# chlhnu/DOT-SOCP

Measured on AMD Instinct MI355X. Metric: ADMM iters/sec on NxNxT dot2d staggered grid at 1/2/4/8 MI355X, higher is better.
Workload: dtype f64

## Files before the change

### dot-socp_amd/capi.py

```python
import ctypes
import os

import numpy as np

_HERE = os.path.dirname(os.path.abspath(__file__))
LIB_PATH = os.path.join(_HERE, "lib", "libdotsocp.so")

i64 = ctypes.c_longlong
dbl = ctypes.c_double
vp = ctypes.c_void_p


class DotsocpError(RuntimeError):
    def __init__(self, code, msg):
        super().__init__(f"libdotsocp error {code}: {msg}")
        self.code = code


class Problem(ctypes.Structure):
    _fields_ = [("dim", ctypes.c_int), ("weighted", ctypes.c_int),
                ("ny", i64), ("nx", i64), ("nt", i64),
                ("D", dbl), ("E", dbl), ("cScale", dbl), ("dScale", dbl),
                ("normc", dbl), ("normd", dbl)]


class Opts(ctypes.Structure):
    _fields_ = [("tau", dbl), ("sigma", dbl), ("tol", dbl), ("maxit", i64),
                ("ifCheckStepByStep", ctypes.c_int), ("checkPrimDualFeas", ctypes.c_int),
                ("scaling", ctypes.c_int), ("time_limit", dbl)]


class Result(ctypes.Structure):
    _fields_ = [("sigma", dbl), ("sigma_internal", dbl), ("cScale", dbl), ("dScale", dbl),
                ("times", dbl * 7), ("iters", i64), ("hist_len", i64), ("stopped", ctypes.c_int),
                ("time_extra", dbl)]


class AccOpts(ctypes.Structure):
    _fields_ = [("restart", i64), ("rho", dbl), ("theta", dbl)]


REPORT_BINS = 49
REPORT_RHO_FLOOR = 1e-8


class Report(ctypes.Structure):
    _fields_ = [("n_nodes", i64), ("n_cells", i64), ("mass_err", dbl), ("neg_err", dbl),
                ("rho_min", dbl), ("rho_neg", i64), ("rho_hist", i64 * REPORT_BINS),
                ("fq_max", dbl), ("fq_pos", i64), ("fq_hist", i64 * REPORT_BINS),
                ("cost", dbl), ("nonfinite", i64)]


class AdvectOpts(ctypes.Structure):
    _fields_ = [("n", i64), ("nsub", ctypes.c_int), ("direction", ctypes.c_int), ("rho_floor", dbl)]


class PushOpts(ctypes.Structure):
    _fields_ = [("n", i64), ("nsub", ctypes.c_int), ("direction", ctypes.c_int), ("rho_floor", dbl), ("nf", i64)]


class MapReport(ctypes.Structure):
    _fields_ = [("n", i64), ("n_clamped", i64), ("n_still", i64), ("mass", dbl),
                ("cost_map", dbl), ("cost_length", dbl), ("cost_action", dbl), ("disp_mean", dbl), ("len_mean", dbl),
                ("disp_max", dbl), ("len_max", dbl), ("detour_max", dbl),
                ("detour_hist", i64 * REPORT_BINS), ("detour_over", i64)]


class RenderOpts(ctypes.Structure):
    _fields_ = [("mode", ctypes.c_int), ("channels", ctypes.c_int), ("nf", i64), ("nlevels", ctypes.c_int),
                ("barrier_index", ctypes.c_int), ("vmax", dbl), ("skip_y", i64), ("skip_x", i64), ("mask_frac", dbl)]


class RenderInfo(ctypes.Structure):
    _fields_ = [("vmax", dbl), ("rho_min", dbl), ("nonfinite", i64), ("masked", i64), ("my", i64), ("mx", i64)]


RENDER_LINEAR, RENDER_INVERTED, RENDER_LEVELS = 0, 1, 2
METHOD_INPALM, METHOD_PALM, METHOD_ACCADMM = 0, 1, 2


F_PHI, F_Q, F_ALPHA, F_Z, F_BETA, F_C, F_WEIGHT = range(7)

SYMBOLS = {
    "dotsocp_last_error": (ctypes.c_char_p, []),
    "dotsocp_version": (ctypes.c_char_p, []),
    "dotsocp_device_count": (ctypes.c_int, []),
    "dotsocp_proj_soc": (ctypes.c_int, [vp, vp, i64, i64]),
    "dotsocp_bfd": (ctypes.c_int, [vp, vp, i64, i64, i64, dbl, dbl]),
    "dotsocp_bfd_conj": (ctypes.c_int, [vp, vp, i64, i64, i64, dbl]),
    "dotsocp_bfd1d": (ctypes.c_int, [vp, vp, i64, i64, dbl, dbl]),
    "dotsocp_bfd_conj1d": (ctypes.c_int, [vp, vp, i64, i64, dbl]),
    "dotsocp_oper_poisson": (ctypes.c_int, [vp, vp, i64, i64, i64, dbl]),
    "dotsocp_dctn": (ctypes.c_int, [vp, i64, i64, i64, ctypes.c_int]),
    "dotsocp_proj_soc_dev": (ctypes.c_int, [vp, vp, i64, i64, vp]),
    "dotsocp_bfd_dev": (ctypes.c_int, [vp, vp, i64, i64, i64, dbl, dbl, vp]),
    "dotsocp_bfd_conj_dev": (ctypes.c_int, [vp, vp, i64, i64, i64, dbl, vp]),
    "dotsocp_create": (vp, [ctypes.POINTER(Problem), ctypes.c_int, ctypes.c_int]),
    "dotsocp_create_multi": (vp, [ctypes.POINTER(Problem), ctypes.c_int, ctypes.c_int]),
    "dotsocp_destroy": (None, [vp]),
    "dotsocp_rccl_unique_id": (ctypes.c_int, [vp]),
    "dotsocp_attach_rccl": (ctypes.c_int, [vp, vp, ctypes.c_int, ctypes.c_int]),
    "dotsocp_slab_range": (ctypes.c_int, [i64, ctypes.c_int, ctypes.c_int, ctypes.POINTER(i64), ctypes.POINTER(i64)]),
    "dotsocp_field_len": (i64, [ctypes.POINTER(Problem), ctypes.c_int]),
    "dotsocp_dct_algorithm": (ctypes.c_int, [i64]),
    "dotsocp_dct_levels": (ctypes.c_int, [i64, ctypes.c_int]),
    "dotsocp_cdft_levels": (ctypes.c_int, [i64]),
    "dotsocp_tsolve_tri_safe": (ctypes.c_int, [i64, i64, i64]),
    "dotsocp_cone_writes_beta": (ctypes.c_int, [i64, dbl, i64, ctypes.c_int, ctypes.c_int, ctypes.c_int, dbl, dbl]),
    "dotsocp_rescale_due": (ctypes.c_int, [i64, ctypes.c_int, dbl, dbl]),
    "dotsocp_qcone_form": (ctypes.c_int, [i64, dbl, i64, ctypes.c_int, ctypes.c_int, ctypes.c_int, ctypes.c_int, dbl, dbl]),
    "dotsocp_release_cache": (i64, []),
    "dotsocp_upload": (ctypes.c_int, [vp, ctypes.c_int, vp]),
    "dotsocp_upload_layers": (ctypes.c_int, [vp, ctypes.c_int, vp, i64, i64]),
    "dotsocp_download": (ctypes.c_int, [vp, ctypes.c_int, vp]),
    "dotsocp_begin": (ctypes.c_int, [vp, ctypes.POINTER(Opts)]),
    "dotsocp_begin_method": (ctypes.c_int, [vp, ctypes.POINTER(Opts), ctypes.c_int, ctypes.POINTER(AccOpts)]),
    "dotsocp_run": (ctypes.c_int, [vp, i64, ctypes.POINTER(i64)]),
    "dotsocp_recover_outputs": (ctypes.c_int, [vp, vp, vp, vp, vp, vp, vp, vp, vp]),
    "dotsocp_report_edges": (ctypes.c_int, [vp]),
    "dotsocp_solution_report": (ctypes.c_int, [vp, vp, vp, ctypes.POINTER(Report), vp, vp]),
    "dotsocp_recover_velocity": (ctypes.c_int, [vp, vp, vp, dbl, vp, vp]),
    "dotsocp_advect_particles": (ctypes.c_int, [vp, vp, vp, ctypes.POINTER(AdvectOpts), vp, vp, vp, vp, ctypes.POINTER(i64)]),
    "dotsocp_push_mass": (ctypes.c_int, [vp, vp, vp, ctypes.POINTER(PushOpts), vp, vp, vp, vp, vp, ctypes.POINTER(i64),
                                         ctypes.POINTER(dbl), vp]),
    "dotsocp_map_report": (ctypes.c_int, [vp, vp, vp, ctypes.POINTER(AdvectOpts), vp, vp, vp, ctypes.POINTER(MapReport),
                                          vp, vp, vp]),
    "dotsocp_render_evolution": (ctypes.c_int, [vp, vp, vp, ctypes.POINTER(RenderOpts), vp, vp, vp, vp, vp, vp, vp,
                                                ctypes.POINTER(RenderInfo)]),
    "dotsocp_jump_next_level": (ctypes.c_int, [vp, vp]),
    "dotsocp_finish": (ctypes.c_int, [vp, ctypes.POINTER(Result)]),
    "dotsocp_get_history": (ctypes.c_int, [vp, vp, vp, vp, vp]),
    "dotsocp_set_profiling": (ctypes.c_int, [vp, ctypes.c_int]),
    "dotsocp_kernel_time": (ctypes.c_int, [vp, ctypes.c_char_p, ctypes.POINTER(dbl), ctypes.POINTER(i64)]),
    "dotsocp_canary_check": (ctypes.c_int, []),
    "dotsocp_poisson_phi": (ctypes.c_int, [vp]),
    "dotsocp_synchronize": (ctypes.c_int, [vp]),
    "dotsocp_weights_create": (vp, [ctypes.c_int, i64, i64, i64, ctypes.c_int]),
    "dotsocp_weights_destroy": (None, [vp]),
    "dotsocp_weights_len": (i64, [i64, i64, i64, ctypes.c_int, ctypes.c_int]),
    "dotsocp_weights_set": (ctypes.c_int, [vp, vp]),
    "dotsocp_weights_set_space": (ctypes.c_int, [vp, vp, vp]),
    "dotsocp_weights_restrict": (ctypes.c_int, [vp, ctypes.c_int]),
    "dotsocp_weights_log10_mean": (ctypes.c_int, [vp, ctypes.c_int, ctypes.POINTER(dbl)]),
    "dotsocp_weights_download": (ctypes.c_int, [vp, ctypes.c_int, vp]),
    "dotsocp_upload_weight_from": (ctypes.c_int, [vp, vp, ctypes.c_int]),
}

_lib = None


def _share_torchs_hip_runtime():
    import importlib.util
    import sys
    if "torch" in sys.modules or os.environ.get("DOTSOCP_SYSTEM_HIP"):
        return
    try:
        spec = importlib.util.find_spec("torch")
    except (ImportError, ValueError):
        return
    if not spec or not spec.submodule_search_locations:
        return
    for name in ("libamdhip64.so", "libamdhip64.so.7"):
        path = os.path.join(list(spec.submodule_search_locations)[0], "lib", name)
        if os.path.exists(path):
            try:
                ctypes.CDLL(path, mode=ctypes.RTLD_GLOBAL)
            except OSError:
                pass
            return


def lib():
    global _lib
    if _lib is None:
        _share_torchs_hip_runtime()
        if not os.path.exists(LIB_PATH):
            raise ImportError(
                f"{LIB_PATH} is missing: build the HIP extension first "
                "(python -c 'import __graft_entry__ as g; g.build()'); there is no CPU fallback")
        L = ctypes.CDLL(LIB_PATH)
        for name, (res, args) in SYMBOLS.items():
            f = getattr(L, name)
            f.restype = res
            f.argtypes = args
        _lib = L
    return _lib


def check(code):
    if code != 0:
        raise DotsocpError(code, lib().dotsocp_last_error().decode())


def fptr(a):
    if not isinstance(a, np.ndarray) or a.dtype != np.float64 or not (a.flags.f_contiguous or a.flags.c_contiguous):
        raise ValueError("expected a contiguous float64 numpy array")
    return a.ctypes.data


def slab_range(nt, world, rank):
    t0, t1 = i64(), i64()
    check(lib().dotsocp_slab_range(nt, world, rank, ctypes.byref(t0), ctypes.byref(t1)))
    return t0.value, t1.value


def rccl_unique_id():
    buf = (ctypes.c_ubyte * 128)()
    check(lib().dotsocp_rccl_unique_id(buf))
    return bytes(buf)


DCT_ALGORITHMS = ("none", "fft", "pfa", "rader", "bluestein", "dense")


def dct_algorithm(n):
    return DCT_ALGORITHMS[lib().dotsocp_dct_algorithm(int(n))]


def dct_levels(n, axis):
    return int(lib().dotsocp_dct_levels(int(n), int(axis)))


def cdft_levels(n):
    return int(lib().dotsocp_cdft_levels(int(n)))
```

### dot-socp_amd/csrc/capi.hip

```cpp
#include <cstring>
#include <new>

#include "comm.h"
#include "solver.h"
#include "weights.h"

using namespace dotsocp;

namespace dotsocp {
extern thread_local std::string g_last_error;
int dotsocp_slab_range_impl(i64 nt, int world, int rank, i64 *t0, i64 *t1);
}

struct dotsocp_ctx {
    Solver s;
};

struct dotsocp_weights {
    Weights w;
};

static int require_device() {
    int n = 0;
    if (hipGetDeviceCount(&n) != hipSuccess || n <= 0) {
// ... 119 lines not shown
    Grid g;
    DS_CHECK(make_grid(g, nt, 1, nx));
    DS_ARG(z && q, "NULL pointer");
    DS_CHECK(require_device());
    DevBuf dz, dq;
    DS_CHECK(dz.alloc(10 * g.Nz));
    DS_CHECK(dq.alloc(g.NqAlloc));
    DS_HIP(hipMemset(dz.p, 0, sizeof(double) * 10 * g.Nz));
    for (int j = 0; j < 6; ++j)
        DS_HIP(hipMemcpy(dz.p + k1dCols[j] * g.Nz, z + j * g.Nz, sizeof(double) * g.Nz, hipMemcpyHostToDevice));
    DS_CHECK(launch_bfd_conj(g, dq.p, dz.p, scale, nullptr));
    DS_HIP(hipDeviceSynchronize());
    DS_HIP(hipMemcpy(q, dq.p, sizeof(double) * g.NqAlloc, hipMemcpyDeviceToHost));
    return 0;
}

static int dctn_dev(double *a, double *b, i64 ny, i64 nx, i64 nt, int inverse, DctPlan *py, DctPlan *px, DctPlan *pt) {
    if (!inverse) {
        DS_CHECK(launch_dct_axis(py, a, b, ny, nx, nt, 0, 0, nullptr));
        DS_CHECK(launch_dct_axis(px, b, a, ny, nx, nt, 1, 0, nullptr));
        DS_CHECK(launch_dct_axis(pt, a, b, ny, nx, nt, 2, 0, nullptr));
    } else {
        DS_CHECK(launch_dct_axis(pt, a, b, ny, nx, nt, 2, 1, nullptr));
        DS_CHECK(launch_dct_axis(px, b, a, ny, nx, nt, 1, 1, nullptr));
        DS_CHECK(launch_dct_axis(py, a, b, ny, nx, nt, 0, 1, nullptr));
    }
    return 0;
}

struct Plans {
    DctPlan *py = nullptr, *px = nullptr, *pt = nullptr;
    ~Plans() { dct_plan_destroy(py); dct_plan_destroy(px); dct_plan_destroy(pt); }
    int make(i64 ny, i64 nx, i64 nt) {
        DS_CHECK(dct_length_check(ny)); DS_CHECK(dct_length_check(nx)); DS_CHECK(dct_length_check(nt));
        py = dct_plan_create(ny); px = dct_plan_create(nx); pt = dct_plan_create(nt);
        if (!py || !px || !pt) { set_error("DCT plan allocation failed"); return DOTSOCP_EHIP; }
        return 0;
    }
};

int dotsocp_dctn(double *a, dotsocp_i64 ny, dotsocp_i64 nx, dotsocp_i64 nt, int inverse) {
    DS_ARG(a && ny >= 1 && nx >= 1 && nt >= 1, "bad array");
    DS_CHECK(dct_length_check(ny)); DS_CHECK(dct_length_check(nx)); DS_CHECK(dct_length_check(nt));
    DS_CHECK(require_device());
    const i64 n = ny * nx * nt;
    DevBuf da, db;
    Plans pl;
    DS_CHECK(da.alloc(n));
    DS_CHECK(db.alloc(n));
    DS_CHECK(pl.make(ny, nx, nt));
    DS_HIP(hipMemcpy(da.p, a, sizeof(double) * n, hipMemcpyHostToDevice));
    DS_CHECK(dctn_dev(da.p, db.p, ny, nx, nt, inverse, pl.py, pl.px, pl.pt));
    DS_HIP(hipDeviceSynchronize());
    DS_HIP(hipMemcpy(a, db.p, sizeof(double) * n, hipMemcpyDeviceToHost));
    return 0;
}

int dotsocp_oper_poisson(double *res, const double *rhs, dotsocp_i64 ny, dotsocp_i64 nx, dotsocp_i64 nt,
                         double kernelScale) {
    DS_ARG(res && rhs && ny >= 1 && nx >= 1 && nt >= 1, "bad array");
    DS_CHECK(dct_length_check(ny)); DS_CHECK(dct_length_check(nx)); DS_CHECK(dct_length_check(nt));
    DS_CHECK(require_device());
    const i64 n = ny * nx * nt;
    DevBuf da, db, cy, cx, ct;
    Plans pl;
    DS_CHECK(da.alloc(n));
    DS_CHECK(db.alloc(n));
    DS_CHECK(pl.make(ny, nx, nt));
    const double pi = 3.14159265358979323846;
    auto table = [&](DevBuf &d, i64 m) -> int {
        std::vector<double> t((size_t)m);
        for (i64 k = 0; k < m; ++k) t[k] = (2.0 * (double)(m - 1) * (double)(m - 1)) * (1.0 - cos(pi * (double)k / (double)m));
        DS_CHECK(d.alloc(m));
        DS_HIP(hipMemcpy(d.p, t.data(), sizeof(double) * m, hipMemcpyHostToDevice));
        return 0;
    };
    DS_CHECK(table(cy, ny));
    DS_CHECK(table(cx, nx));
    DS_CHECK(table(ct, nt));
    DS_HIP(hipMemcpy(da.p, rhs, sizeof(double) * n, hipMemcpyHostToDevice));
    Grid g;
    g.set(ny, nx, nt, 0, nt);
    DS_CHECK(launch_dct_axis(pl.py, da.p, db.p, ny, nx, nt, 0, 0, nullptr));
    DS_CHECK(launch_dct_axis(pl.px, db.p, da.p, ny, nx, nt, 1, 0, nullptr));
    DS_CHECK(launch_poisson_t_single(pl.pt, g, kernelScale, cy.p, cx.p, ct.p, da.p, db.p, 0, nullptr, tsolve_tri_allowed()));
    DS_CHECK(launch_dct_axis(pl.px, da.p, db.p, ny, nx, nt, 1, 1, nullptr));
    DS_CHECK(launch_dct_axis(pl.py, db.p, da.p, ny, nx, nt, 0, 1, nullptr));
    DS_HIP(hipDeviceSynchronize());
    DS_HIP(hipMemcpy(res, da.p, sizeof(double) * n, hipMemcpyDeviceToHost));
    return 0;
}

dotsocp_ctx *dotsocp_create(const dotsocp_problem *prob, int device, int nslabs) {
    dotsocp_ctx *c = new (std::nothrow) dotsocp_ctx();
    if (!c) { set_error("out of host memory"); return nullptr; }
    if (c->s.init(prob, device, nslabs) != 0) {
        delete c;
        return nullptr;
    }
    return c;
}

dotsocp_ctx *dotsocp_create_multi(const dotsocp_problem *prob, int first_device, int ngpu) {
    dotsocp_ctx *c = new (std::nothrow) dotsocp_ctx();
    if (!c) { set_error("out of host memory"); return nullptr; }
    if (c->s.init(prob, first_device, ngpu, true) != 0) {
        delete c;
        return nullptr;
    }
    return c;
}

void dotsocp_destroy(dotsocp_ctx *ctx) { delete ctx; }

int dotsocp_slab_range(dotsocp_i64 nt, int world, int rank, dotsocp_i64 *t0, dotsocp_i64 *t1) {
    DS_ARG(t0 && t1 && world >= 1 && rank >= 0 && rank < world && nt >= 2 * world, "bad slab request");
    return dotsocp_slab_range_impl(nt, world, rank, t0, t1);
}

int dotsocp_rccl_unique_id(unsigned char id[128]) {
    DS_ARG(id != nullptr, "id is NULL");
    Rccl &api = rccl_api();
    DS_CHECK(api.load());
    ncclUniqueId uid;
    static_assert(sizeof(uid) == 128, "ncclUniqueId is expected to be 128 bytes");
    DS_NCCL(api.GetUniqueId(&uid));
    memcpy(id, &uid, sizeof uid);
    return 0;
}

int dotsocp_attach_rccl(dotsocp_ctx *ctx, const unsigned char id[128], int rank, int world) {
    if (!ctx) { set_error("ctx is NULL"); return DOTSOCP_EINVAL; }
    return ctx->s.attach_rccl(id, rank, world);
}

#define CTX_OR_FAIL()                                      \
    do {                                                   \
        if (!ctx) { set_error("ctx is NULL"); return DOTSOCP_EINVAL; } \
        (void)hipGetLastError();    \
    } while (0)

int dotsocp_dct_algorithm(dotsocp_i64 n) { return dct_choose_algorithm(n); }
int dotsocp_dct_levels(dotsocp_i64 n, int axis) { return dct_levels(n, axis); }
int dotsocp_cdft_levels(dotsocp_i64 n) { return cdft_levels(n); }
int dotsocp_tsolve_tri_safe(dotsocp_i64 ny, dotsocp_i64 nx, dotsocp_i64 nt) { return tsolve_tri_safe(ny, nx, nt) ? 1 : 0; }

int dotsocp_cone_writes_beta(dotsocp_i64 it, double last_sigma_it, dotsocp_i64 maxit, int check_step_by_step,
                             int last_of_run, int rescale, double maxFeas, double relGap) {
    return cone_writes_beta(it, last_sigma_it, maxit, check_step_by_step != 0, last_of_run != 0, rescale, maxFeas, relGap) ? 1 : 0;
}
int dotsocp_rescale_due(dotsocp_i64 it, int rescale, double maxFeas, double relGap) {
    return rescale_due(it, rescale, maxFeas, relGap) ? 1 : 0;
}
int dotsocp_qcone_form(dotsocp_i64 it, double last_sigma_it, dotsocp_i64 maxit, int check_step_by_step, int last_of_run,
                       int next_last_of_run, int rescale, double maxFeas, double relGap) {
    return qcone_form(it, last_sigma_it, maxit, check_step_by_step != 0, last_of_run != 0, next_last_of_run != 0, rescale,
                      maxFeas, relGap);
}

dotsocp_i64 dotsocp_field_len(const dotsocp_problem *p, int field) {
    if (!p || (p->dim != 1 && p->dim != 2) || p->nt < 2 || p->nx < 1 || (p->dim == 2 && p->ny < 1)) return -1;
    const i64 ny = p->dim == 1 ? p->nx : p->ny, nx = p->dim == 1 ? 1 : p->nx, nt = p->nt;
    const i64 Nphi = ny * nx * nt, Nz = ny * nx * (nt - 1);
    const i64 Nq = Nz + ny * (nx - 1) * nt + (ny - 1) * nx * nt;
    switch (field) {
        case DOTSOCP_F_PHI: case DOTSOCP_F_C: return Nphi;
        case DOTSOCP_F_Q: case DOTSOCP_F_ALPHA: case DOTSOCP_F_WEIGHT: return Nq;
        case DOTSOCP_F_Z: case DOTSOCP_F_BETA: return Nz * (p->dim == 1 ? 6 : 10);
        default: return -1;
    }
}

int dotsocp_upload(dotsocp_ctx *ctx, int field, const double *host) { CTX_OR_FAIL(); return ctx->s.upload(field, host); }
dotsocp_i64 dotsocp_release_cache(void) { return (dotsocp_i64)device_cache_release(); }

int dotsocp_upload_layers(dotsocp_ctx *ctx, int field, const double *host, dotsocp_i64 t0, dotsocp_i64 n) {
    CTX_OR_FAIL();
    return ctx->s.upload_layers(field, host, t0, n);
}
int dotsocp_download(dotsocp_ctx *ctx, int field, double *host) { CTX_OR_FAIL(); return ctx->s.download(field, host); }
int dotsocp_begin(dotsocp_ctx *ctx, const dotsocp_opts *opts) { CTX_OR_FAIL(); return ctx->s.begin(opts); }
int dotsocp_begin_method(dotsocp_ctx *ctx, const dotsocp_opts *opts, int method, const dotsocp_acc_opts *acc) {
    CTX_OR_FAIL();
    return ctx->s.begin_method(opts, method, acc);
}
int dotsocp_recover_outputs(dotsocp_ctx *ctx, const double *rho0, const double *rho1, double *rho, double *Ex,
                            double *Ey, double *q0, double *bx, double *by) {
    CTX_OR_FAIL();
    if (ctx->s.prob.dim == 1)
        return ctx->s.recover_outputs(rho0, rho1, rho, nullptr, Ex, q0, nullptr, bx);
    return ctx->s.recover_outputs(rho0, rho1, rho, Ex, Ey, q0, bx, by);
}

int dotsocp_report_edges(double edges[DOTSOCP_REPORT_BINS + 1]) {
    if (!edges) { set_error("invalid argument: report_edges() needs an array of %d doubles", DOTSOCP_REPORT_BINS + 1); return DOTSOCP_EINVAL; }
    report_edges_host(edges);
    return 0;
}

int dotsocp_solution_report(dotsocp_ctx *ctx, const double *rho0, const double *rho1, dotsocp_report *rep, double *layer_mass,
                            double *layer_neg) {
    CTX_OR_FAIL();
    return ctx->s.solution_report(rho0, rho1, rep, layer_mass, layer_neg);
}

int dotsocp_recover_velocity(dotsocp_ctx *ctx, const double *rho0, const double *rho1, double rho_floor, double *vx, double *vy) {
    CTX_OR_FAIL();
    if (ctx->s.prob.dim == 1)
        return ctx->s.recover_velocity(rho0, rho1, rho_floor, nullptr, vx);
    return ctx->s.recover_velocity(rho0, rho1, rho_floor, vx, vy);
}

int dotsocp_advect_particles(dotsocp_ctx *ctx, const double *rho0, const double *rho1, const dotsocp_advect_opts *o, double *x,
                             double *y, double *traj_x, double *traj_y, dotsocp_i64 *n_clamped) {
    CTX_OR_FAIL();
    if (ctx->s.prob.dim == 1)
        return ctx->s.advect_particles(rho0, rho1, o, nullptr, x, nullptr, traj_x, n_clamped);
    return ctx->s.advect_particles(rho0, rho1, o, x, y, traj_x, traj_y, n_clamped);
}

int dotsocp_push_mass(dotsocp_ctx *ctx, const double *rho0, const double *rho1, const dotsocp_push_opts *o, double *x, double *y,
                      const double *mass, const dotsocp_i64 *frame_nodes, double *frames, dotsocp_i64 *n_clamped, double *unit,
                      double *l1) {
    CTX_OR_FAIL();
    if (ctx->s.prob.dim == 1)
        return ctx->s.push_mass(rho0, rho1, o, nullptr, x, mass, frame_nodes, frames, n_clamped, unit, l1);
    return ctx->s.push_mass(rho0, rho1, o, x, y, mass, frame_nodes, frames, n_clamped, unit, l1);
}

int dotsocp_map_report(dotsocp_ctx *ctx, const double *rho0, const double *rho1, const dotsocp_advect_opts *o, double *x, double *y,
                       const double *mass, dotsocp_map_report_t *rep, double *disp, double *len, double *action) {
    CTX_OR_FAIL();
    if (ctx->s.prob.dim == 1)
        return ctx->s.map_report(rho0, rho1, o, nullptr, x, mass, rep, disp, len, action);
    return ctx->s.map_report(rho0, rho1, o, x, y, mass, rep, disp, len, action);
}

int dotsocp_render_evolution(dotsocp_ctx *ctx, const double *rho0, const double *rho1, const dotsocp_render_opts *opts,
                             const dotsocp_i64 *frame_nodes, const double *levels, const unsigned char *lut,
                             const unsigned char *barrier, unsigned char *image, double *mvx, double *mvy,
                             dotsocp_render_info *info) {
    CTX_OR_FAIL();
    if (ctx->s.prob.dim != 1 || !opts)
        return ctx->s.render_evolution(rho0, rho1, opts, frame_nodes, levels, lut, barrier, image, mvx, mvy, info);
    dotsocp_render_opts o = *opts;
    if (o.skip_y >= 1 && o.skip_x >= 1) { o.skip_y = o.skip_x; o.skip_x = 1; }
    dotsocp_render_info got{};
    const int rc = ctx->s.render_evolution(rho0, rho1, &o, frame_nodes, levels, lut, barrier, image, nullptr, mvx, &got);
    if (rc == 0 && info) {
        *info = got;
        info->mx = got.my;
        info->my = got.my > 0 ? 1 : 0;
    }
    return rc;
}

int dotsocp_jump_next_level(dotsocp_ctx *coarse, dotsocp_ctx *fine) {
    if (!coarse || !fine) { set_error("context is NULL"); return DOTSOCP_EINVAL; }
    return fine->s.jump_from(coarse->s);
}

int dotsocp_run(dotsocp_ctx *ctx, dotsocp_i64 n_iters, dotsocp_i64 *done) { CTX_OR_FAIL(); return ctx->s.run(n_iters, done); }
int dotsocp_finish(dotsocp_ctx *ctx, dotsocp_result *res) { CTX_OR_FAIL(); return ctx->s.finish(res); }

int dotsocp_get_history(dotsocp_ctx *ctx, double *kkt, double *time, double *iter, double *pdGap) {
    CTX_OR_FAIL();
    const Solver &s = ctx->s;
    const size_t n = s.hist_iter.size();
    for (size_t i = 0; i < n; ++i) {
        if (kkt) for (int j = 0; j < 7; ++j) kkt[j * n + i] = s.hist_kkt[i * 7 + j];
        if (time) time[i] = s.hist_time[i];
        if (iter) iter[i] = s.hist_iter[i];
        if (pdGap) pdGap[i] = s.hist_gap[i];
    }
    return 0;
}

int dotsocp_set_profiling(dotsocp_ctx *ctx, int on) {
    CTX_OR_FAIL();
    ctx->s.profiling = on != 0;
    return 0;
}

int dotsocp_kernel_time(dotsocp_ctx *ctx, const char *name, double *avg_ms, dotsocp_i64 *launches) {
    CTX_OR_FAIL();
    DS_ARG(name != nullptr, "name is NULL");
    static const char *names[PH_COUNT] = {"rhs", "poisson", "cone_proj", "qstep", "beta", "kkt",
                                          "cone_fused_a", "cone_fused_b", "materialise", "comm",
                                          "interp", "acc_cone", "acc_gather", "qstep_first", "transpose", "cone_carry", "qcone",
                                          "velocity_layer", "advect", "deposit", "frame_l1", "advect_path", "map_final"};
    for (int i = 0; i < PH_COUNT; ++i)
        if (strcmp(name, names[i]) == 0) {
            const i64 n = ctx->s.phase_launches[i];
            if (avg_ms) *avg_ms = n ? ctx->s.phase_ms[i] / (double)n : 0.0;
            if (launches) *launches = n;
            return 0;
        }
    set_error("unknown kernel family '%s'", name);
    return DOTSOCP_EINVAL;
}

int dotsocp_canary_check(void) {
    std::string rep;
    const int bad = canary_check(&rep);
    if (bad) set_error("canary: %d device buffer(s) written out of bounds: %s", bad, rep.c_str());
    return bad;
}

#define WEIGHTS_OR_FAIL()                                  \
    do {                                                   \
        if (!w) { set_error("weight pyramid is NULL"); return DOTSOCP_EINVAL; } \
        (void)hipGetLastError();                           \
    } while (0)

dotsocp_weights *dotsocp_weights_create(int device, dotsocp_i64 ny, dotsocp_i64 nx, dotsocp_i64 nt, int levels) {
    dotsocp_weights *w = new (std::nothrow) dotsocp_weights();
    if (!w) { set_error("out of host memory"); return nullptr; }
    if (w->w.init(device, ny, nx, nt, levels) != 0) {
        delete w;
        return nullptr;
    }
    return w;
}

void dotsocp_weights_destroy(dotsocp_weights *w) { delete w; }

dotsocp_i64 dotsocp_weights_len(dotsocp_i64 ny, dotsocp_i64 nx, dotsocp_i64 nt, int levels, int level) {
    return weights_level_len(ny, nx, nt, levels, level);
}

int dotsocp_weights_set(dotsocp_weights *w, const double *weight) { WEIGHTS_OR_FAIL(); return w->w.set(weight); }
int dotsocp_weights_set_space(dotsocp_weights *w, const double *weightX, const double *weightY) {
    WEIGHTS_OR_FAIL();
    return w->w.set_space(weightX, weightY);
}
int dotsocp_weights_restrict(dotsocp_weights *w, int log_mean) { WEIGHTS_OR_FAIL(); return w->w.restrict_all(log_mean); }
int dotsocp_weights_log10_mean(dotsocp_weights *w, int level, double *mean) { WEIGHTS_OR_FAIL(); return w->w.log10_mean(level, mean); }
int dotsocp_weights_download(dotsocp_weights *w, int level, double *host) { WEIGHTS_OR_FAIL(); return w->w.download(level, host); }

int dotsocp_upload_weight_from(dotsocp_ctx *ctx, dotsocp_weights *w, int level) {
    CTX_OR_FAIL();
    WEIGHTS_OR_FAIL();
    const Weights::Level *L = nullptr;
    DS_CHECK(w->w.level_for_upload(level, &L));
    return ctx->s.upload_weight_from(L->w, w->w.device, L->ny, L->nx, L->nt);
}

int dotsocp_poisson_phi(dotsocp_ctx *ctx) { CTX_OR_FAIL(); return ctx->s.poisson_phi(); }

int dotsocp_synchronize(dotsocp_ctx *ctx) {
    CTX_OR_FAIL();
    ctx->s.cur_dev = -1;
    return ctx->s.sync_all();
}

}
```

### dot-socp_amd/csrc/fused.hip

```cpp
#include "device_utils.h"
#include "gather_tile.h"
#include "kernels.h"

#include <cstdlib>

namespace dotsocp {

template <int MODE, int XB, bool NT = false, bool GIN = false, bool GOUT = false>
__global__ void __launch_bounds__(64 * XB) k_cone_fused(Grid g, LoopCoef c, FusedArgs a) {
    static_assert(MODE == 1 || !(GIN || GOUT), "the gamma form exists between two MODE_B passes only");
    constexpr bool DUAL = (MODE >= 5);
    constexpr bool UPD = (MODE != 0 && MODE != 6);
    constexpr bool PROJ = (MODE < 2 || MODE >= 5);
    __shared__ double2 xch[2][XB][64];
    __shared__ double2 xchp[DUAL ? 2 : 1][DUAL ? XB : 1][DUAL ? 64 : 1];
    const int lane = threadIdx.x, xl = threadIdx.y;
    const BlockId blk = block_id(a.xcd != 0);
    const i64 y = (i64)blk.x * 64 + lane;
    const i64 x = (i64)blk.y * XB + xl;
    const bool inb = (y < g.ny) && (x < g.nx);
    const i64 yc = inb ? y : 0, xc = inb ? x : 0;
    const i64 t0 = ((i64)blk.z + a.z0) * a.TC;
    const i64 t1 = (t0 + a.TC < g.ncl) ? t0 + a.TC : g.ncl;
    const bool lastChunk = (t1 == g.ncl);
    constexpr bool GATHER = (PROJ || MODE == 4);
    const bool carried = GATHER && !DUAL && t0 > 0 && a.carry_in != nullptr;
    const i64 tstart = (GATHER && t0 > 0 && !carried) ? t0 - 1 : t0;
    const i64 nxblk = gridDim.y, nyblk = gridDim.x;

    EdgeQuad cur = load_edges(g, a.q, yc, xc, tstart, c.sf), curo, cur3;
    if (UPD && !GIN) curo = load_edges(g, a.q_old, yc, xc, tstart, c.sf);
    if (MODE == 5) cur3 = load_edges(g, a.q3, yc, xc, tstart, c.sf);
    GatherCarry gc, gcp;
    if (carried) {
        const i64 ci = yc + g.py * xc;
        gc.p3 = a.carry_in[ci]; gc.p4 = a.carry_in[g.plane + ci];
        gc.p7 = a.carry_in[2 * g.plane + ci]; gc.p8 = a.carry_in[3 * g.plane + ci];
    }
    const i64 tstop = (GATHER && lastChunk) ? t1 + 1 : t1;
    for (i64 tl = tstart; tl < tstop; ++tl) {
        const bool hasCell = tl < g.ncl;
        const bool own = tl >= t0;
        double w[10], wp[10];
        if (hasCell) {
            const i64 i = yc + g.py * (xc + g.nx * tl);
            const EdgeQuad nxt = load_edges(g, a.q, yc, xc, tl + 1, c.sf);
            double b[10], v[10];
#pragma unroll
            for (int j = 0; j < 10; ++j) b[j] = ld_stream<NT>(a.beta_in + j * g.Nc + i);
            if (!GIN) apply_scale_ops(b, a.bops);
            build_z2(v, a.q[i], cur, nxt, c.s, c.dF);
            if constexpr (GIN) {
#pragma unroll
                for (int j = 0; j < 10; ++j) b[j] = mult_finish(b[j], v[j], c.tau);
                if (!GOUT && own && inb) {
#pragma unroll
                    for (int j = 0; j < 10; ++j) st_stream<NT>(a.beta_out + j * g.Nc + i, b[j]);
                }
            } else if constexpr (UPD) {
                const EdgeQuad nxto = load_edges(g, a.q_old, yc, xc, tl + 1, c.sf);
                double zo[10];
                build_z2(zo, a.q_old[i], curo, nxto, c.s, c.dF);
#pragma unroll
                for (int j = 0; j < 10; ++j) zo[j] = zo[j] - b[j];
                proj_row<10>(zo);
#pragma unroll
                for (int j = 0; j < 10; ++j) b[j] = mult_finish(mult_carry(b[j], zo[j], c.tau), v[j], c.tau);
                if (own && inb) {
                    if (MODE != 3 && !GOUT) {
#pragma unroll
                        for (int j = 0; j < 10; ++j) st_stream<NT>(a.beta_out + j * g.Nc + i, b[j]);
                    }
                    if (MODE == 2 || MODE == 3) {
#pragma unroll
                        for (int j = 0; j < 10; ++j) st_stream<NT>(a.z_out + j * g.Nc + i, zo[j]);
                    }
                }
                curo = nxto;
                if (MODE == 4) {
#pragma unroll
                    for (int j = 0; j < 10; ++j) w[j] = zo[j] + b[j];
                    if (own && inb) a.q2[i] = c.s * (w[9] - w[0]);
                }
            }
            cur = nxt;
            if (PROJ) {
                if (MODE == 5) {
                    const EdgeQuad nxt3 = load_edges(g, a.q3, yc, xc, tl + 1, c.sf);
                    build_z2(v, a.q3[i], cur3, nxt3, c.s, c.dF);
                    cur3 = nxt3;
                }
#pragma unroll
                for (int j = 0; j < 10; ++j) v[j] = v[j] - b[j];
                proj_row<10>(v);
                if (GOUT && own && inb) {
#pragma unroll
                    for (int j = 0; j < 10; ++j) st_stream<NT>(a.beta_out + j * g.Nc + i, mult_carry(b[j], v[j], c.tau));
                }
#pragma unroll
                for (int j = 0; j < 10; ++j) w[j] = v[j] + b[j];
                if (own && inb) a.q2[i] = c.s * (w[9] - w[0]);
                if (DUAL) {
#pragma unroll
                    for (int j = 0; j < 10; ++j) wp[j] = w[j] + c.tau * v[j];
                    if (own && inb) a.p2[i] = c.s * (wp[9] - wp[0]);
                }
            }
        } else {
#pragma unroll
            for (int j = 0; j < 10; ++j) w[j] = 0.0;
            if (DUAL) {
#pragma unroll
                for (int j = 0; j < 10; ++j) wp[j] = 0.0;
            }
        }
        if constexpr (GATHER && !DUAL)
            gather_emit<XB>(g, c.sf, xch, gc, w, tl, own && inb, x, y, xl, lane, nxblk, nyblk, blk.y, blk.x,
                            a.q2, a.sx, a.sy);
        if constexpr (DUAL) {
            gather_post<XB>(xch, gc, w, xl, lane);
            gather_post<XB>(xchp, gcp, wp, xl, lane);
            __syncthreads();
            gather_finish<XB>(g, c.sf, xch, gc, w, tl, own && inb, x, y, xl, lane, nxblk, nyblk, blk.y, blk.x,
                              a.q2, a.sx, a.sy);
            gather_finish<XB>(g, c.sf, xchp, gcp, wp, tl, own && inb, x, y, xl, lane, nxblk, nyblk, blk.y, blk.x,
                              a.p2, a.sxp, a.syp);
        }
    }
    if (GATHER && !DUAL && !lastChunk && a.carry_out != nullptr && inb) {
        const i64 ci = y + g.py * x;
        a.carry_out[ci] = gc.p3; a.carry_out[g.plane + ci] = gc.p4;
        a.carry_out[2 * g.plane + ci] = gc.p7; a.carry_out[3 * g.plane + ci] = gc.p8;
    }
}

bool stream_nt_enabled() {
    const char *e = getenv("DOTSOCP_NT");
    return !(e && atoi(e) == 0);
}

bool tile_xcd_remap(const Grid &g) {
    return (g.py % 16) != 0;
}

bool cone_split_enabled() { return true; }

int fused_geometry(const Grid &g, FusedGeom &fg) {
    fg.XB = 4;
    fg.nyblk = (g.ny + 63) / 64;
    fg.nxblk = (g.nx + fg.XB - 1) / fg.XB;
    const i64 tiles = fg.nyblk * fg.nxblk;
    const i64 target = 2048;
    i64 chunks = (target + tiles - 1) / tiles;
    if (chunks < 1) chunks = 1;
    if (!(g.first && g.last) && cone_split_enabled() && chunks < 2 && g.ncl >= 12) chunks = 2;
    i64 TC = (g.ncl + chunks - 1) / chunks;
    if (TC < 8) TC = 8;
    if (TC > g.ncl) TC = g.ncl;
    if (TC < 1) TC = 1;
    fg.TC = TC;
    fg.chunks = (g.ncl + TC - 1) / TC;
    fg.sx_len = (g.ncl + 1) * fg.nxblk * g.ny;
    fg.sy_len = (g.ncl + 1) * g.nx * fg.nyblk;
    return 0;
}

int launch_cone_fused(int mode, const Grid &g, const LoopCoef &c, const FusedGeom &fg, FusedArgs a,
                      hipStream_t st, i64 z0, i64 zcount, int flavour) {
    if (g.Nz <= 0) return 0;
    if (zcount < 0) zcount = fg.chunks - z0;
    if (z0 < 0 || zcount <= 0 || z0 + zcount > fg.chunks) return 0;
    a.TC = fg.TC;
    a.z0 = (int)z0;
    a.xcd = tile_xcd_remap(g) ? 1 : 0;
    dim3 grid((unsigned)fg.nyblk, (unsigned)fg.nxblk, (unsigned)zcount);
    dim3 blk(64, 4);
    const bool nt = stream_nt_enabled();
#define CONE_MODE(M)                                                                     \
    case M:                                                                              \
        if (nt) DS_KLAUNCH((k_cone_fused<M, 4, true>), grid, blk, 0, st, g, c, a);       \
        else DS_KLAUNCH((k_cone_fused<M, 4>), grid, blk, 0, st, g, c, a);                \
        break;
    if (flavour != 0) {
        if (mode != 1 || (flavour & ~(CONE_GIN | CONE_GOUT))) { set_error("bad fused flavour"); return DOTSOCP_EINVAL; }
        if ((flavour & CONE_GIN) && !a.bops.empty()) { set_error("internal: gamma with a pending scaling"); return DOTSOCP_ESTATE; }
#define CONE_FLAV(GI, GO)                                                                          \
        if (nt) DS_KLAUNCH((k_cone_fused<1, 4, true, GI, GO>), grid, blk, 0, st, g, c, a);         \
        else DS_KLAUNCH((k_cone_fused<1, 4, false, GI, GO>), grid, blk, 0, st, g, c, a);
        if (flavour == CONE_GOUT) { CONE_FLAV(false, true) }
        else if (flavour == CONE_GIN) { CONE_FLAV(true, false) }
        else { CONE_FLAV(true, true) }
#undef CONE_FLAV
        DS_HIP(hipGetLastError());
        return 0;
    }
    switch (mode) {
        CONE_MODE(0) CONE_MODE(1) CONE_MODE(2) CONE_MODE(3) CONE_MODE(4) CONE_MODE(5) CONE_MODE(6)
#undef CONE_MODE
        default: set_error("bad fused mode"); return DOTSOCP_EINVAL;
    }
    DS_HIP(hipGetLastError());
    return 0;
}

}
```

### dot-socp_amd/csrc/kernels.h

```cpp
#pragma once
#include "common.h"
#include "defer.h"
#include "particle_block.h"

namespace dotsocp {

struct LoopCoef {
    double s;
    double sf;
    double dF;
    double at, ax, ay;
    double tau;
    double c1, c2;
    double dinv1, dinv2;
};

enum {
    S_Q2 = 0, S_Z2, S_APHI2, S_ALPHA2, S_BETA2, S_FBBETA2, S_PRIM1, S_PRIM2, S_DUAL1, S_DUAL2,
    S_COMPLEM, S_DOTCOMP, S_RHO2, S_RHOFQ2, S_MRHOB, S_M2, S_RHOB2, S_QALPHA, S_CPHI, S_PHI2,
    S_COUNT
};

struct KktCoef {
    double sigma;
    double kappa;
    double dsD;
    double dsE;
};

struct ScaleOps {
    int n;
    double mul, div;
    double mul2, div2;
    bool empty() const { return n == 0; }
    void clear() { n = 0; }
    bool push(double m, double d) {
        if (n >= 2) return false;
        if (n == 0) { mul = m; div = d; } else { mul2 = m; div2 = d; }
        n += 1;
        return true;
    }
};

int launch_proj_soc(double *out, const double *in, i64 M, i64 K, hipStream_t st);
int launch_bfd(const Grid &g, double *z, const double *q, double s, double dF, hipStream_t st);
int launch_bfd_conj(const Grid &g, double *q, const double *w, double s, hipStream_t st, const double *tail_bx = nullptr,
                    const double *tail_by = nullptr);
int launch_cone_proj(const Grid &g, const LoopCoef &c, const double *q, const double *beta, double *z,
                     hipStream_t st);
int launch_beta_update(const Grid &g, const LoopCoef &c, const double *q, const double *z, double *beta,
                       hipStream_t st);
int launch_gather_tail(const Grid &g, const double *z, const double *beta, double *tail_bx, double *tail_by,
                       hipStream_t st);

struct FusedGeom {
    int XB;
    i64 nyblk, nxblk;
    i64 TC, chunks;
    i64 sx_len, sy_len;
};
struct FusedArgs {
    const double *q_old;
    const double *q;
    const double *beta_in;
    double *beta_out;
    double *z_out;
    double *q2;
    double *sx, *sy;
    const double *q3;
    double *p2, *sxp, *syp;
    i64 TC;
    ScaleOps bops;
    int xcd;
    int z0;
    const double *carry_in;
    double *carry_out;
};
bool tile_xcd_remap(const Grid &g);
int fused_geometry(const Grid &g, FusedGeom &fg);
enum { CONE_GIN = 1, CONE_GOUT = 2 };
int launch_cone_fused(int mode, const Grid &g, const LoopCoef &c, const FusedGeom &fg, FusedArgs a,
                      hipStream_t st, i64 z0 = 0, i64 zcount = -1, int flavour = 0);
bool cone_split_enabled();

struct KktWork;
struct AccArgs {
    const double *q;
    const double *z_in, *beta_in;
    const double *z0, *beta0;
    double *z0_out, *beta0_out;
    double bdiv;
    KktCoef kk;
    const double *alpha_p, *weight;
    double *partials;
    int nostore;
    double *z_out, *beta_out;
    double *q2, *sx, *sy;
    i64 TC;
    double c1, c2, om_rho, rho;
};
struct AccCoef {
    double c1, c2, om_rho, rho;
    double om_c1, c1c2;
};
int launch_acc_cone(int mode, const Grid &g, const LoopCoef &c, const FusedGeom &fg, AccArgs a, hipStream_t st);
int launch_acc_cone_kkt(const Grid &g, const LoopCoef &c, const FusedGeom &fg, AccArgs a, const KktWork &w, hipStream_t st);
int launch_acc_restart(double *x, const double *xp, double *anchor, i64 n, const AccCoef &k, double div, hipStream_t st);
int launch_acc_interp(double *x, const double *xp, double *aux, i64 n, const AccCoef &k, int mode, int write_aux,
                      hipStream_t st);

int launch_prolong_phi(const Grid &gf, const Grid &gc, const double *phic, double *phif, double sc_in, double sc_out,
                       hipStream_t st, i64 tc0 = 0);
int launch_prolong_beta(const Grid &gf, const Grid &gc, const double *betac, double *betaf, double *neg, double sc_in0,
                        double sc_in1, double sc_out, hipStream_t st, i64 tc0 = 0, i64 Nzc = -1);
int launch_scale_div(double *x, const double *w, i64 n, double sc, hipStream_t st);
int launch_fill(double *x, i64 n, double v, hipStream_t st);
int launch_outputs(const Grid &g, const double *q, const double *alpha, const double *weight, const double *rho0,
                   const double *rho1, const double *a_prev, double sig, double cD, double dD, int which, double *out,
                   hipStream_t st);
int launch_out_tail(const Grid &g, const double *alpha, const double *weight, double sig, double cD, double *out,
                    hipStream_t st);

int launch_velocity_layer(const Grid &g, const double *alpha, const double *weight, const double *rho0, const double *rho1,
                          const double *a_prev, double sig, double cD, bool dim1, i64 tl, double floor, double *vX, double *vY,
                          hipStream_t st);
int launch_advect_seed(bool dim1, i64 n, double *px, double *py, unsigned int *flag, hipStream_t st);
int launch_advect(bool dim1, i64 ny, i64 nx, i64 py, const double *vX0, const double *vY0, const double *vX1,
                  const double *vY1, i64 n, int nsub, int dir, double dt, double *px, double *py_, unsigned int *flag,
                  hipStream_t st, double *sq = nullptr, double *len = nullptr);
int launch_advect_count(const unsigned int *flag, i64 n, unsigned long long *count, hipStream_t st);
int launch_deposit(bool dim1, i64 ny, i64 nx, i64 py, i64 n, const double *px, const double *py_, const i64 *units,
                   unsigned long long *cnt, hipStream_t st);
int launch_frame_l1(const Grid &g, const double *alpha, const double *weight, const double *rho0, const double *rho1,
                    const double *a_prev, double sig, double cD, i64 tl, double unit, double *frame, double *partials,
                    double *sum, hipStream_t st);
i64 map_blocks(i64 n);
int launch_map_final(bool dim1, i64 n, const double *px, const double *py_, const double *sq, const double *len, const double *sx,
                     const double *sy, const double *mass, const double *edges, double steps, double *disp, double *action,
                     double *partials, double *sums, unsigned long long *counts, hipStream_t st);

enum { RC_RHO_HIST = 0, RC_FQ_HIST = DOTSOCP_REPORT_BINS, RC_RHO_NEG = 2 * DOTSOCP_REPORT_BINS, RC_FQ_POS, RC_NONFINITE,
       RC_RHO_MIN, RC_FQ_MAX, RC_COUNT };
void report_edges_host(double edges[DOTSOCP_REPORT_BINS + 1]);
double report_key_decode(unsigned long long key, bool inverted, double none);
i64 report_tiles(const Grid &g);
int launch_report_rows(const double *partials, i64 tiles, i64 rows, double *sums, hipStream_t st);
int launch_report(const Grid &g, const double *q, const double *alpha, const double *weight, const double *rho0,
                  const double *rho1, const double *a_prev, double sig, double cD, double dD, bool dim1, const double *edges,
                  double *partials, double *sums, unsigned long long *counts, hipStream_t st);

enum { RR_MAX = 0, RR_MIN, RR_NONFINITE, RR_MASKED, RR_COUNT };
#define RND_LEVELS 255
int launch_rho_range(const Grid &g, const double *alpha, const double *weight, const double *rho0, const double *rho1,
                     const double *a_prev, double sig, double cD, const unsigned char *barrier, unsigned long long *counts,
                     hipStream_t st);
int launch_render(const Grid &g, const double *alpha, const double *weight, const double *rho0, const double *rho1,
                  const double *a_prev, double sig, double cD, i64 tl, int mode, int channels, const unsigned char *barrier,
                  const double *levels, int nlevels, const unsigned char *lut, int barrier_index, double vmax,
                  unsigned char *image, hipStream_t st);
int launch_movement(const Grid &g, const double *alpha, const double *weight, const double *rho0, const double *rho1,
                    const double *a_prev, double sig, double cD, i64 tl, i64 skip_y, i64 skip_x, i64 my, i64 mx, double thr,
                    double *mvX, double *mvY, hipStream_t st);

struct QStepExtra {
    ScaleOps aops;
    double *partials, *resid;
    double kappa, dsD;
    double *u0_tail;
    int c_ends;
};
int launch_qstep_rhs(const Grid &g, const LoopCoef &c, const FusedGeom &fg, const double *phi, const double *q2,
                     const double *sx, const double *sy, const double *weight, const double *tail_bx,
                     const double *tail_by, const double *cvec, double *q_out, const double *alpha_in, double *alpha_out,
                     double *rhs, hipStream_t st, i64 z0 = 0, i64 zcount = -1, i64 zstride = 1,
                     const QStepExtra *ex = nullptr);
i64 qstep_rhs_blocks(const Grid &g, const FusedGeom &fg);
struct QConeArgs {
    const double *phi, *q2v, *sx, *sy, *cvec, *alpha_in, *gamma_in;
    double *alpha_out, *rhs, *q_out, *beta_out, *q2_out, *sx_out, *sy_out;
    i64 TC;
    int ap_on;
    double ap_mul, ap_div;
    int c_ends;
};
int launch_qcone(const Grid &g, const LoopCoef &c, const FusedGeom &fg, QConeArgs a, bool gout, hipStream_t st);
i64 qcone_chunk_len(const Grid &g);
i64 qstep_rhs_chunks(const Grid &g, const FusedGeom &fg, i64 *TC = nullptr);
int launch_qstep_rhs_acc(int var, const Grid &g, const LoopCoef &c, const FusedGeom &fg, const double *phi,
                         const double *q2, const double *sx, const double *sy, const double *weight, const double *cvec,
                         double *q_raw, const double *alpha_in, double *alpha_out, double *rhs, double *q_state,
                         const double *q_anchor, const double *alpha_anchor, const AccCoef &k, hipStream_t st,
                         const double *tail_bx = nullptr, const double *tail_by = nullptr, double *u0_tail = nullptr);
int launch_qstep_palm_first(const Grid &g, const LoopCoef &c, const FusedGeom &fg, const double *phi, const double *q2,
                            const double *sx, const double *sy, const double *cvec, double *q_out, const double *alpha,
                            double *rhs, hipStream_t st, const double *tail_bx = nullptr, const double *tail_by = nullptr,
                            const double *qk = nullptr);

int launch_qstep_fused(const Grid &g, const LoopCoef &c, const FusedGeom &fg, const double *phi,
                       const double *q2, const double *sx, const double *sy, const double *weight,
                       const double *tail_bx, const double *tail_by, double *q_out, double *alpha,
                       hipStream_t st);
int launch_rhs_sigma_fix(const Grid &g, double *rhs, const double *r, double *cvec, double factor, hipStream_t st,
                         bool c_ends = false);
int launch_c_interior_test(const Grid &g, const double *cvec, int *flag, hipStream_t st);
int launch_rhs_fixup(const Grid &g, const LoopCoef &c, const double *u0_prev, double *rhs, hipStream_t st);
int launch_grad(const Grid &g, const LoopCoef &c, const double *phi, double *out, hipStream_t st);
int launch_tail_finalize(const Grid &g, const LoopCoef &c, const FusedGeom &fg, const double *q2, const double *sx,
                         const double *sy, double *tail_bx, double *tail_by, hipStream_t st);
int launch_kkt_tail(const Grid &g, const double *alpha, const double *beta, const double *weight, double *a0,
                    double *a0w, double *bt_bx, double *bt_by, hipStream_t st);
int launch_rhs(const Grid &g, const LoopCoef &c, const double *q, const double *alpha, const double *cvec,
               const double *weight, const double *u0_prev, double *rhs, hipStream_t st, bool c_ends = false);
int launch_qstep(const Grid &g, const LoopCoef &c, const double *phi, const double *z, const double *beta,
                 const double *weight, const double *tail_bx, const double *tail_by, double *q,
                 double *alpha, hipStream_t st);
int launch_u0_tail(const Grid &g, const double *q, const double *alpha, const double *weight, double *out,
                   hipStream_t st);
int launch_scale(double *x, i64 n, double mul, double div, hipStream_t st);
#define DS_MAX_WORLD 64
struct PencilCuts {
    int world;
    i64 cut[DS_MAX_WORLD + 1];
};
int launch_pencil_pack(bool pack, const PencilCuts &pc, i64 plane, i64 ntl, double *slab, double *stage, hipStream_t st);

#define TRI_EXTRA 256
int launch_tri_local(const Grid &g, i64 nt, double kscale, const double *cy, const double *cx, const PencilCuts &pc,
                     const double *r, double *send, hipStream_t st);
int launch_tri_reduced(const Grid &g, i64 nt, double kscale, const double *cy, const double *cx, const PencilCuts &pc,
                       int rank, i64 l0, i64 nl, const i64 *slab_n, const double *recv, double *back, double *zero_work,
                       hipStream_t st, const double *own_recv = nullptr, double *own_back = nullptr);
int launch_tri_final(const Grid &g, i64 nt, double kscale, const double *cy, const double *cx, const PencilCuts &pc,
                     const double *back, double *x, hipStream_t st);
bool tsolve_tri_supported(i64 nt);
bool tsolve_tri_preferred(i64 nt, bool pow2, i64 plane);
bool tsolve_tri_safe(i64 ny, i64 nx, i64 nt);
int launch_tsolve_tri(const Grid &g, i64 nt, double kscale, const double *cy, const double *cx, double *x, hipStream_t st);
int device_cus();
struct GatherMsgs {
    const double *src[DS_MAX_WORLD];
    double *dst[DS_MAX_WORLD];
    i64 count[DS_MAX_WORLD];
    int n;
};
int launch_gather_msgs(const GatherMsgs &m, hipStream_t st);

#define KKT_SLICES 64
struct KktWork {
    double *partials;
    i64 maxBlocks;
    double *sums;
};
struct KktHalo {
    const double *a0_prev, *a0w_prev, *btail_bx, *btail_by;
};
i64 kkt_partials_needed(const Grid &g);
int launch_kkt(const Grid &g, const LoopCoef &c, const KktCoef &k, const double *phi, const double *q,
               const double *alpha, const double *z, const double *beta, const double *cvec,
               const double *weight, const KktHalo &halo, const KktWork &w, int parts, hipStream_t st,
               bool layer0 = false, double *resid = nullptr);
int launch_kkt_nodual(const Grid &g, const LoopCoef &c, const KktCoef &k, const double *phi, const double *q,
                      const double *alpha, const double *cvec, const double *weight, const KktWork &w, hipStream_t st);
int launch_kkt_bnd_dual(const Grid &g, const LoopCoef &c, const KktCoef &k, const FusedGeom &fg, const double *q,
                        const double *alpha, const double *weight, const double *q2, const double *sx, const double *sy,
                        const KktWork &w, hipStream_t st);
int launch_kkt_cells_update(const Grid &g, const LoopCoef &c, const KktCoef &k, const FusedGeom &fg, FusedArgs a,
                            const double *phi, const double *alpha, const double *weight, const KktWork &w,
                            hipStream_t st, bool edges = false, const double *q_new = nullptr);
int launch_norms(const Grid &g, const LoopCoef &c, const KktCoef &k, const FusedGeom &fg, FusedArgs a, const double *phi,
                 const double *alpha, const double *weight, const KktWork &w, hipStream_t st);
double *kkt_qstep_partials(const Grid &g, const KktWork &w);
int launch_kkt_final(const Grid &g, const KktWork &w, hipStream_t st);

enum { DCT_ALG_NONE = 0, DCT_ALG_FFT = 1, DCT_ALG_PFA = 2, DCT_ALG_RADER = 3, DCT_ALG_BLUESTEIN = 4, DCT_ALG_DENSE = 5 };
int dct_choose_algorithm(i64 n);
struct DctPlan;
int dct_levels(i64 n, int axis);
int dct_length_check(i64 n);
int cdft_levels(i64 n);
DctPlan *dct_plan_create(i64 n);
void dct_plan_destroy(DctPlan *p);
int launch_dct_axis(const DctPlan *p, const double *src, double *dst, i64 n0, i64 n1, i64 n2, int axis,
                    int inverse, hipStream_t st, i64 pitch0 = 0);
bool dct_plan_is_pow2(const DctPlan *p);
bool dct_plan_has_tsolve(const DctPlan *p);
int launch_dct_t_solve(const DctPlan *p, const double *src, double *dst, i64 ny, i64 nplane, i64 line0, i64 nl,
                       i64 nt, double kscale, const double *cy, const double *cx, const double *ct, hipStream_t st,
                       i64 pitch0 = 0);
int launch_spectral_divide_pencil(double *data, i64 ny, i64 line0, i64 nl, i64 nt, double kscale, const double *cy,
                                  const double *cx, const double *ct, hipStream_t st);
int launch_spectral_divide(double *data, i64 ny, i64 nt, i64 x0, i64 nxl, double kscale, const double *cy,
                           const double *cx, const double *ct, hipStream_t st, i64 pitch0 = 0);
bool tsolve_tri_allowed();
int launch_poisson_t_single(const DctPlan *pt, const Grid &g, double kscale, const double *cy, const double *cx,
                            const double *ct, double *p, double *p2, i64 pitch0, hipStream_t st, bool allow_tri);

}
```

### dot-socp_amd/csrc/kkt.hip

```cpp
#include "device_utils.h"
#include "gather_tile.h"
#include "kernels.h"

#include <cstdlib>

namespace dotsocp {

struct WBeta {
    const double *b;
    i64 Nz;
    __device__ __forceinline__ double operator()(int j, i64 cell) const { return b[j * Nz + cell]; }
};

template <bool WEIGHTED, int PART, bool NODUAL = false>
__global__ void __launch_bounds__(TILE_Y *TILE_X) k_kkt(Grid g, LoopCoef c, KktCoef k, i64 chunk,
                                                         const double *__restrict__ phi, const double *__restrict__ q,
                                                         const double *__restrict__ alpha, const double *__restrict__ z,
                                                         const double *__restrict__ beta,
                                                         const double *__restrict__ cvec,
                                                         const double *__restrict__ weight,
                                                         KktHalo halo, double *__restrict__ partials,
                                                         double *__restrict__ resid) {
    const i64 y = (i64)blockIdx.x * TILE_Y + threadIdx.x;
    const i64 x = (i64)blockIdx.y * TILE_X + threadIdx.y;
// ... 2 lines not shown
    const i64 tend = (tbeg + chunk < g.ntl) ? tbeg + chunk : g.ntl;
    double S[S_COUNT];
#pragma unroll
    for (int i = 0; i < S_COUNT; ++i) S[i] = 0.0;
    WBeta WB{beta, g.Nc};
    auto wgt = [&](i64 idx) { return WEIGHTED ? weight[idx] : 1.0; };
    auto rhoT_at = [&](i64 yy, i64 xx, i64 tl) -> double {
        if (tl >= g.ncl) return 0.0;
        if (tl < 0) {
            if (g.first) return 0.0;
            return k.kappa * halo.a0w_prev[yy + g.py * xx];
        }
        const i64 cidx = yy + g.py * (xx + g.nx * tl);
        return k.kappa * (wgt(cidx) * alpha[cidx]);
    };
    auto rho_node = [&](i64 yy, i64 xx, i64 tl) { return (rhoT_at(yy, xx, tl - 1) + rhoT_at(yy, xx, tl)) / 2.0; };
    auto edge_sums = [&](i64 idx, double tmp, double q2b) {
        const double w = wgt(idx);
        const double qv = q[idx], av = alpha[idx];
        const double wq = w * qv, wa = w * av;
        S[S_Q2] += qv * qv;
        S[S_ALPHA2] += av * av;
        S[S_APHI2] += tmp * tmp;
        const double r1 = tmp - wq;
        S[S_PRIM1] += r1 * r1;
        if (!NODUAL) {
            S[S_FBBETA2] += q2b * q2b;
            const double r2 = q2b + wa;
            S[S_DUAL2] += r2 * r2;
        }
        S[S_QALPHA] += wq * av;
    };
    if (inb) {
        for (i64 tl = tbeg; tl < tend; ++tl) {
            const i64 node = y + g.py * (x + g.nx * tl);
            const i64 bxo = g.offBx + g.bxLayer * tl, byo = g.offBy + g.byLayer * tl;
            if (PART & 1) {
                double r = 0.0;
                if (tl >= 1)
                    r += c.at * alpha[node - g.plane];
                else if (!g.first)
                    r += c.at * halo.a0_prev[y + g.py * x];
                if (tl < g.ncl) r += (-c.at) * alpha[node];
                if (x >= 1) r += c.ax * alpha[bxo + y + g.py * (x - 1)];
                if (x <= g.nx - 2) r += (-c.ax) * alpha[bxo + y + g.py * x];
                if (y >= 1) r += c.ay * alpha[byo + (y - 1) + g.pyb * x];
                if (y <= g.ny - 2) r += (-c.ay) * alpha[byo + y + g.pyb * x];
                const double cv = cvec[node], pv = phi[node];
                r = r - cv;
                if (resid) resid[node] = (tl == 0 && !g.first) ? r - c.at * halo.a0_prev[y + g.py * x] : r;
                S[S_DUAL1] += r * r;
                S[S_CPHI] += cv * pv;
                S[S_PHI2] += pv * pv;
            }
            if ((PART & 2) && tl < g.ncl) {
                const EdgeQuad ea = load_edges(g, q, y, x, tl, c.sf);
                const EdgeQuad eb = load_edges(g, q, y, x, tl + 1, c.sf);
                const double q0 = q[node];
                double z2[10], zz[10], p[10];
                build_z2(z2, q0, ea, eb, c.s, c.dF);
                double zs = 0.0, bs = 0.0, rs = 0.0;
#pragma unroll
                for (int j = 0; j < 10; ++j) {
                    const double zv = z[j * g.Nc + node], bv = beta[j * g.Nc + node];
                    zz[j] = zv;
                    p[j] = zv - k.sigma * bv;
                    zs += zv * zv;
                    bs += bv * bv;
                    const double d = zv - z2[j];
                    rs += d * d;
                }
                proj_row<10>(p);
                double cs = 0.0;
#pragma unroll
                for (int j = 0; j < 10; ++j) {
                    const double d = zz[j] - p[j];
                    cs += d * d;
                }
                S[S_Z2] += zs;
                S[S_BETA2] += bs;
                S[S_PRIM2] += rs;
                S[S_COMPLEM] += cs;
                const double rhoT = rhoT_at(y, x, tl);
                double sq = 0.0;
#pragma unroll
                for (int j = 1; j < 9; ++j) {
                    const double e = k.dsE * z2[j];
                    sq += e * e;
                }
                double rhoFq = rhoT + k.dsD * q0 + sq / 4.0;
                rhoFq = (rhoFq < 0.0) ? 0.0 : rhoFq;
                const double dd = rhoT - rhoFq;
                S[S_DOTCOMP] += dd * dd;
                S[S_RHO2] += rhoT * rhoT;
                S[S_RHOFQ2] += rhoFq * rhoFq;
                double tmp = (-c.at) * phi[node];
                tmp += c.at * phi[node + g.plane];
                edge_sums(node, tmp, c.s * (WB(9, node) - WB(0, node)));
            }
            if ((PART & 16) && tl < g.ncl) {
                double tmp = (-c.at) * phi[node];
                tmp += c.at * phi[node + g.plane];
                edge_sums(node, tmp, 0.0);
            }
            if ((PART & 4) && x < g.nx - 1) {
                const i64 idx = bxo + y + g.py * x;
                double tmp = (-c.ax) * phi[node];
                tmp += c.ax * phi[node + g.py];
                const double q2b = NODUAL ? 0.0 : c.sf * gather_bx(g, WB, y, x, tl, halo.btail_bx);
                edge_sums(idx, tmp, q2b);
                const double rm = (rho_node(y, x, tl) + rho_node(y, x + 1, tl)) / 2.0;
                const double rb = k.dsD * (rm * q[idx]);
                const double m = k.kappa * (wgt(idx) * alpha[idx]);
                const double d = m - rb;
                S[S_MRHOB] += d * d;
                S[S_M2] += m * m;
                S[S_RHOB2] += rb * rb;
            }
            if ((PART & 8) && y < g.ny - 1) {
                const i64 idx = byo + y + g.pyb * x;
                double tmp = (-c.ay) * phi[node];
                tmp += c.ay * phi[node + 1];
                const double q2b = NODUAL ? 0.0 : c.sf * gather_by(g, WB, y, x, tl, halo.btail_by);
                edge_sums(idx, tmp, q2b);
                const double rm = (rho_node(y, x, tl) + rho_node(y + 1, x, tl)) / 2.0;
                const double rb = k.dsD * (rm * q[idx]);
                const double m = k.kappa * (wgt(idx) * alpha[idx]);
                const double d = m - rb;
                S[S_MRHOB] += d * d;
                S[S_M2] += m * m;
                S[S_RHOB2] += rb * rb;
            }
        }
    }
    __shared__ double red[TILE_X][S_COUNT];
    const int lane = threadIdx.x;
#pragma unroll
    for (int i = 0; i < S_COUNT; ++i) {
        double v = S[i];
#pragma unroll
        for (int off = 32; off >= 1; off >>= 1) v += __shfl_down(v, off, 64);
        if (lane == 0) red[threadIdx.y][i] = v;
    }
    __syncthreads();
    if (threadIdx.y == 0 && lane < S_COUNT) {
        double v = red[0][lane];
#pragma unroll
        for (int wv = 1; wv < TILE_X; ++wv) v += red[wv][lane];
        const i64 b = blockIdx.x + (i64)gridDim.x * (blockIdx.y + (i64)gridDim.y * blockIdx.z);
        partials[b * S_COUNT + lane] = v;
    }
}

template <bool WEIGHTED, bool EDGES, bool NORMS = false, bool NT = false>
__global__ void __launch_bounds__(TILE_Y *TILE_X) k_kkt_cells(Grid g, LoopCoef c, KktCoef k, FusedArgs a,
                                                               const double *__restrict__ phi,
                                                               const double *__restrict__ alpha,
                                                               const double *__restrict__ weight,
                                                               double *__restrict__ partials) {
    __shared__ double2 xch[EDGES ? 2 : 1][EDGES ? TILE_X : 1][EDGES ? 64 : 1];
    const int lane = threadIdx.x, xl = threadIdx.y;
    const i64 y = (i64)blockIdx.x * TILE_Y + lane;
    const i64 x = (i64)blockIdx.y * TILE_X + xl;
    const bool inb = (y < g.ny) && (x < g.nx);
    const i64 yc = inb ? y : 0, xc = inb ? x : 0;
    const i64 t0 = (i64)blockIdx.z * a.TC;
    const i64 t1 = (t0 + a.TC < g.ncl) ? t0 + a.TC : g.ncl;
    const bool lastChunk = (t1 == g.ncl);
    const i64 tstart = (EDGES && t0 > 0) ? t0 - 1 : t0;
    const i64 tstop = (EDGES && lastChunk) ? t1 + 1 : t1;
    const i64 nxblk = gridDim.y, nyblk = gridDim.x;
    double S[S_COUNT];
#pragma unroll
    for (int i = 0; i < S_COUNT; ++i) S[i] = 0.0;
    auto wgt = [&](i64 idx) { return WEIGHTED ? weight[idx] : 1.0; };
    double p3 = 0.0, p4 = 0.0, p7 = 0.0, p8 = 0.0;
    int par = 0;
    if (inb || EDGES) {
        EdgeQuad cur = load_edges(g, a.q, yc, xc, tstart, c.sf);
        EdgeQuad curo = load_edges(g, a.q_old, yc, xc, tstart, c.sf);
        for (i64 tl = tstart; tl < tstop; ++tl) {
            const bool hasCell = tl < g.ncl;
            const bool own = (tl >= t0) && inb;
            double b[10];
            if (hasCell) {
                const i64 i = yc + g.py * (xc + g.nx * tl);
                const EdgeQuad nxt = load_edges(g, a.q, yc, xc, tl + 1, c.sf);
                const EdgeQuad nxto = load_edges(g, a.q_old, yc, xc, tl + 1, c.sf);
                const double q0 = a.q[i];
                double v[10], zo[10];
#pragma unroll
                for (int j = 0; j < 10; ++j) b[j] = ld_stream<NT>(a.beta_in + j * g.Nc + i);
                apply_scale_ops(b, a.bops);
                build_z2(v, q0, cur, nxt, c.s, c.dF);
                build_z2(zo, a.q_old[i], curo, nxto, c.s, c.dF);
#pragma unroll
                for (int j = 0; j < 10; ++j) zo[j] = zo[j] - b[j];
                proj_row<10>(zo);
                double zs = 0.0, bs = 0.0, rs = 0.0;
#pragma unroll
                for (int j = 0; j < 10; ++j) {
                    const double r = zo[j] - v[j];
                    b[j] = mult_finish(mult_carry(b[j], zo[j], c.tau), v[j], c.tau);
                    zs += zo[j] * zo[j];
                    bs += b[j] * b[j];
                    rs += r * r;
                }
                cur = nxt;
                curo = nxto;
                if (own && NORMS) {
                    S[S_Z2] += zs;
                    S[S_BETA2] += bs;
                }
                if (own && !NORMS) {
#pragma unroll
                    for (int j = 0; j < 10; ++j) st_stream<NT>(a.beta_out + j * g.Nc + i, b[j]);
                    auto xj = [&](int j) { return zo[j] - k.sigma * b[j]; };
                    const double n = sqrt(soc_norm2(xj, 10)), x0 = xj(0);
                    double cf = (x0 / n + 1.0) * 0.5;
                    cf = (cf > 1.0) ? 1.0 : cf;
                    cf = (cf < 0.0) ? 0.0 : cf;
                    const double p0 = (cf >= 1.0) ? x0 : cf * n;
                    double cs = (zo[0] - p0) * (zo[0] - p0);
#pragma unroll
                    for (int j = 1; j < 10; ++j) {
                        const double d = zo[j] - cf * xj(j);
                        cs += d * d;
                    }
                    S[S_Z2] += zs;
                    S[S_BETA2] += bs;
                    S[S_PRIM2] += rs;
                    S[S_COMPLEM] += cs;
                    const double w = wgt(i);
                    const double av = alpha[i];
                    const double rhoT = k.kappa * (w * av);
                    double sq = 0.0;
#pragma unroll
                    for (int j = 1; j < 9; ++j) {
                        const double e = k.dsE * v[j];
                        sq += e * e;
                    }
                    double rhoFq = rhoT + k.dsD * q0 + sq / 4.0;
                    rhoFq = (rhoFq < 0.0) ? 0.0 : rhoFq;
                    const double dd = rhoT - rhoFq;
                    S[S_DOTCOMP] += dd * dd;
                    S[S_RHO2] += rhoT * rhoT;
                    S[S_RHOFQ2] += rhoFq * rhoFq;
                    const double q2b = c.s * (b[9] - b[0]);
                    const double wa = w * av;
                    S[S_FBBETA2] += q2b * q2b;
                    const double r2 = q2b + wa;
                    S[S_DUAL2] += r2 * r2;
                    if (!EDGES) {
                        double tmp = (-c.at) * phi[i];
                        tmp += c.at * phi[i + g.plane];
                        const double wq = w * q0;
                        S[S_Q2] += q0 * q0;
                        S[S_ALPHA2] += av * av;
                        S[S_APHI2] += tmp * tmp;
                        const double r1 = tmp - wq;
                        S[S_PRIM1] += r1 * r1;
                        S[S_QALPHA] += wq * av;
                    }
                }
            } else {
#pragma unroll
                for (int j = 0; j < 10; ++j) b[j] = 0.0;
            }
            if (EDGES) {
                auto dual = [&](i64 e, double acc) {
                    const double gb = c.sf * acc;
                    S[S_FBBETA2] += gb * gb;
                    const double r2 = gb + wgt(e) * alpha[e];
                    S[S_DUAL2] += r2 * r2;
                };
                xch[par][xl][lane] = make_double2(b[1], p3);
                __syncthreads();
                const bool sumLayer = (tl < g.ntl) && !(tl == 0 && !g.first);
                if (own) {
                    if (x < g.nx - 1) {
                        const i64 e = g.offBx + g.bxLayer * tl + y + g.py * x;
                        if (xl < TILE_X - 1) {
                            if (sumLayer) {
                            const double2 r = xch[par][xl + 1][lane];
                            double acc = r.x + b[2];
                            acc += r.y;
                            acc += p4;
                            dual(e, acc);
                            }
                        } else {
                            a.q2[e] = b[2] + p4;
                        }
                    }
                    if (xl == 0 && x > 0) a.sx[(tl * nxblk + blockIdx.y) * g.ny + y] = b[1] + p3;
                }
                const double u5 = __shfl_down(b[5], 1, 64), u7 = __shfl_down(p7, 1, 64);
                if (own) {
                    if (y < g.ny - 1) {
                        const i64 e = g.offBy + g.byLayer * tl + y + g.pyb * x;
                        if (lane < 63) {
                            if (sumLayer) {
                                double acc = u5 + b[6];
                                acc += u7;
                                acc += p8;
                                dual(e, acc);
                            }
                        } else {
                            a.q2[e] = b[6] + p8;
                        }
                    }
                    if (lane == 0 && y > 0) a.sy[(tl * g.nx + x) * nyblk + blockIdx.x] = b[5] + p7;
                }
                p3 = b[3]; p4 = b[4]; p7 = b[7]; p8 = b[8];
                par ^= 1;
            }
        }
    }
    __shared__ double red[TILE_X][S_COUNT];
#pragma unroll
    for (int i = 0; i < S_COUNT; ++i) {
        double v = S[i];
#pragma unroll
        for (int off = 32; off >= 1; off >>= 1) v += __shfl_down(v, off, 64);
        if (lane == 0) red[threadIdx.y][i] = v;
    }
    __syncthreads();
    if (threadIdx.y == 0 && lane < S_COUNT) {
        double v = red[0][lane];
#pragma unroll
        for (int wv = 1; wv < TILE_X; ++wv) v += red[wv][lane];
        const i64 bb = blockIdx.x + (i64)gridDim.x * (blockIdx.y + (i64)gridDim.y * blockIdx.z);
        partials[bb * S_COUNT + lane] = v;
    }
}

__global__ void __launch_bounds__(256) k_sumsq(const double *__restrict__ x, i64 n, int slot, double *__restrict__ partials) {
    double v = 0.0;
    for (i64 i = (i64)blockIdx.x * 256 + threadIdx.x; i < n; i += (i64)gridDim.x * 256) v += x[i] * x[i];
    __shared__ double red[4];
#pragma unroll
    for (int off = 32; off >= 1; off >>= 1) v += __shfl_down(v, off, 64);
    if ((threadIdx.x & 63) == 0) red[threadIdx.x >> 6] = v;
    __syncthreads();
    if (threadIdx.x < S_COUNT)
        partials[(i64)blockIdx.x * S_COUNT + threadIdx.x] = ((int)threadIdx.x == slot) ? ((red[0] + red[1]) + red[2]) + red[3] : 0.0;
}

#define BND_TC 8
// ... 46 lines not shown
            const double gb = c.sf * (q2[e] + sy[(tl * g.nx + x) * fg.nyblk + (y / 64 + 1)]);
            sF += gb * gb;
            const double r2 = gb + wgt(e) * alpha[e];
            sD += r2 * r2;
        }
    }
    }
    __shared__ double red[4][4];
    double v4[4] = {sM, sR, sF, sD};
    const int lane = threadIdx.x & 63, wv = threadIdx.x >> 6;
#pragma unroll
    for (int i = 0; i < 4; ++i) {
        double v = v4[i];
#pragma unroll
        for (int off = 32; off >= 1; off >>= 1) v += __shfl_down(v, off, 64);
        if (lane == 0) red[wv][i] = v;
    }
    __syncthreads();
    if (threadIdx.x < S_COUNT) {
        const int s = threadIdx.x;
        const int i = (s == S_MRHOB) ? 0 : (s == S_RHOB2) ? 1 : (s == S_FBBETA2) ? 2 : (s == S_DUAL2) ? 3 : -1;
        double v = 0.0;
        if (i >= 0) v = ((red[0][i] + red[1][i]) + red[2][i]) + red[3][i];
        const i64 bb = blockIdx.x + (i64)gridDim.x * (blockIdx.y + (i64)gridDim.y * blockIdx.z);
        partials[bb * S_COUNT + s] = v;
    }
}

__global__ void __launch_bounds__(256) k_kkt_final(const double *__restrict__ partials, i64 nblocks,
                                                    double *__restrict__ sums) {
    const int s = blockIdx.x;
    const i64 per = (nblocks + gridDim.y - 1) / gridDim.y;
    const i64 b0 = (i64)blockIdx.y * per, b1 = (b0 + per < nblocks) ? b0 + per : nblocks;
    double v = 0.0;
    for (i64 b = b0 + threadIdx.x; b < b1; b += 256) v += partials[b * S_COUNT + s];
    __shared__ double red[256];
    red[threadIdx.x] = v;
    __syncthreads();
    for (int off = 128; off >= 1; off >>= 1) {
        if ((int)threadIdx.x < off) red[threadIdx.x] += red[threadIdx.x + off];
        __syncthreads();
    }
    if (threadIdx.x == 0) sums[(i64)blockIdx.y * S_COUNT + s] = red[0];
}

__global__ void __launch_bounds__(64) k_kkt_final2(const double *__restrict__ slices, int nslices, double *__restrict__ sums) {
    const int s = threadIdx.x;
    if (s >= S_COUNT) return;
    double v = 0.0;
    for (int j = 0; j < nslices; ++j) v += slices[(i64)j * S_COUNT + s];
    sums[s] = v;
}

static void kkt_geometry(const Grid &g, dim3 &grid, i64 &chunk) {
    const i64 tiles = ((g.ny + TILE_Y - 1) / TILE_Y) * ((g.nx + TILE_X - 1) / TILE_X);
    i64 chunks = (4096 + tiles - 1) / tiles;
    if (chunks < 1) chunks = 1;
    if (chunks > g.ntl) chunks = g.ntl;
    chunk = (g.ntl + chunks - 1) / chunks;
    chunks = (g.ntl + chunk - 1) / chunk;
    grid = dim3((unsigned)((g.ny + TILE_Y - 1) / TILE_Y), (unsigned)((g.nx + TILE_X - 1) / TILE_X), (unsigned)chunks);
}

static i64 bnd_blocks(const Grid &g, const FusedGeom &fg, int dir) {
    const i64 tch = (g.ntl + BND_TC - 1) / BND_TC;
    if (dir == 0) return ((g.ny + 255) / 256) * fg.nxblk * tch;
    return ((g.nx + 255) / 256) * fg.nyblk * tch;
}

static i64 kkt_region_blocks(const Grid &g) {
    dim3 grid;
    i64 chunk;
    kkt_geometry(g, grid, chunk);
    FusedGeom fg;
    fused_geometry(g, fg);
    i64 m = (i64)grid.x * grid.y * grid.z;
    const i64 cand[] = {fg.nyblk * fg.nxblk * fg.chunks, qstep_rhs_blocks(g, fg), bnd_blocks(g, fg, 0), bnd_blocks(g, fg, 1)};
    for (i64 v : cand) m = v > m ? v : m;
    return m;
}

#define KKT_REGIONS 8
i64 kkt_partials_needed(const Grid &g) { return KKT_REGIONS * kkt_region_blocks(g); }

int launch_kkt(const Grid &g, const LoopCoef &c, const KktCoef &k, const double *phi, const double *q,
               const double *alpha, const double *z, const double *beta, const double *cvec, const double *weight,
               const KktHalo &halo, const KktWork &w, int parts, hipStream_t st, bool layer0, double *resid) {
    dim3 grid;
    i64 chunk;
    kkt_geometry(g, grid, chunk);
    const i64 region = kkt_region_blocks(g);
    if (KKT_REGIONS * region > w.maxBlocks) {
        set_error("kkt workspace too small");
        return DOTSOCP_EINVAL;
    }
    const int base = layer0 ? 4 : 0;
    if (layer0) { chunk = 1; grid.z = 1; }
    const dim3 blk(TILE_Y, TILE_X);
#define KKT_PART(W, P, slot)                                                                                     \
    if (parts & P)                                                                                               \
    DS_KLAUNCH((k_kkt<W, P>), grid, blk, 0, st, g, c, k, chunk, phi, q, alpha, z, beta, cvec, weight, halo, \
                       w.partials + ((layer0 && (slot) > 0 ? (slot) - 1 : (slot)) + base) * region * S_COUNT,    \
                       (P == 1) ? resid : nullptr)
    if (weight) { KKT_PART(true, 1, 0); KKT_PART(true, 2, 1); KKT_PART(true, 4, 2); KKT_PART(true, 8, 3); }
    else { KKT_PART(false, 1, 0); KKT_PART(false, 2, 1); KKT_PART(false, 4, 2); KKT_PART(false, 8, 3); }
#undef KKT_PART
    DS_HIP(hipGetLastError());
    return 0;
}

int launch_kkt_nodual(const Grid &g, const LoopCoef &c, const KktCoef &k, const double *phi, const double *q,
                      const double *alpha, const double *cvec, const double *weight, const KktWork &w, hipStream_t st) {
    dim3 grid;
    i64 chunk;
    kkt_geometry(g, grid, chunk);
    const i64 region = kkt_region_blocks(g);
    if (KKT_REGIONS * region > w.maxBlocks) {
        set_error("kkt workspace too small");
        return DOTSOCP_EINVAL;
    }
    const dim3 blk(TILE_Y, TILE_X);
    const KktHalo halo{nullptr, nullptr, nullptr, nullptr};
    const double *none = nullptr;
#define KKT_ND(W, P, reg)                                                                                                 \
    DS_KLAUNCH((k_kkt<W, P, true>), grid, blk, 0, st, g, c, k, chunk, phi, q, alpha, none, none, cvec, weight, halo, \
               w.partials + (i64)(reg) * region * S_COUNT, (double *)nullptr)
    if (weight) { KKT_ND(true, 1, 0); KKT_ND(true, 16, 4); KKT_ND(true, 4, 5); KKT_ND(true, 8, 6); }
    else { KKT_ND(false, 1, 0); KKT_ND(false, 16, 4); KKT_ND(false, 4, 5); KKT_ND(false, 8, 6); }
#undef KKT_ND
    DS_HIP(hipGetLastError());
    return 0;
}

int launch_kkt_bnd_dual(const Grid &g, const LoopCoef &c, const KktCoef &k, const FusedGeom &fg, const double *q,
                        const double *alpha, const double *weight, const double *q2, const double *sx, const double *sy,
                        const KktWork &w, hipStream_t st) {
    const i64 region = kkt_region_blocks(g);
    for (int dir = 0; dir < 2; ++dir) {
        const i64 len = dir == 0 ? g.ny : g.nx, lines = dir == 0 ? fg.nxblk : fg.nyblk;
        if (len <= 0 || lines <= 0) continue;
        dim3 gb((unsigned)((len + 255) / 256), (unsigned)lines, (unsigned)((g.ntl + BND_TC - 1) / BND_TC));
        double *pb = w.partials + (2 + dir) * region * S_COUNT;
#define BND(W, D) DS_KLAUNCH((k_kkt_bnd<W, D, true>), gb, dim3(256), 0, st, g, c, k, fg, q, alpha, weight, q2, sx, sy, pb)
        if (weight) { if (dir == 0) BND(true, 0); else BND(true, 1); }
        else { if (dir == 0) BND(false, 0); else BND(false, 1); }
#undef BND
        DS_HIP(hipGetLastError());
    }
    return 0;
}

int launch_kkt_cells_update(const Grid &g, const LoopCoef &c, const KktCoef &k, const FusedGeom &fg, FusedArgs a,
                            const double *phi, const double *alpha, const double *weight, const KktWork &w,
                            hipStream_t st, bool edges, const double *q_new) {
    if (g.Nz <= 0) return 0;
    const i64 region = kkt_region_blocks(g);
    a.TC = fg.TC;
    dim3 grid((unsigned)fg.nyblk, (unsigned)fg.nxblk, (unsigned)fg.chunks);
    double *part = w.partials + 1 * region * S_COUNT;
    const dim3 blk(TILE_Y, TILE_X);
    if (!edges) {
        if (weight) DS_KLAUNCH((k_kkt_cells<true, false>), grid, blk, 0, st, g, c, k, a, phi, alpha, weight, part);
        else DS_KLAUNCH((k_kkt_cells<false, false>), grid, blk, 0, st, g, c, k, a, phi, alpha, weight, part);
        DS_HIP(hipGetLastError());
        return 0;
    }
    const bool nt = stream_nt_enabled();
    if (weight) {
        if (nt) DS_KLAUNCH((k_kkt_cells<true, true, false, true>), grid, blk, 0, st, g, c, k, a, phi, alpha, weight, part);
        else DS_KLAUNCH((k_kkt_cells<true, true>), grid, blk, 0, st, g, c, k, a, phi, alpha, weight, part);
    } else {
        if (nt) DS_KLAUNCH((k_kkt_cells<false, true, false, true>), grid, blk, 0, st, g, c, k, a, phi, alpha, weight, part);
        else DS_KLAUNCH((k_kkt_cells<false, true>), grid, blk, 0, st, g, c, k, a, phi, alpha, weight, part);
    }
    DS_HIP(hipGetLastError());
    for (int dir = 0; dir < 2; ++dir) {
        const i64 len = dir == 0 ? g.ny : g.nx, lines = dir == 0 ? fg.nxblk : fg.nyblk;
        if (len <= 0 || lines <= 0) continue;
        dim3 gb((unsigned)((len + 255) / 256), (unsigned)lines, (unsigned)((g.ntl + BND_TC - 1) / BND_TC));
        double *pb = w.partials + (2 + dir) * region * S_COUNT;
#define BND(W, D) DS_KLAUNCH((k_kkt_bnd<W, D>), gb, dim3(256), 0, st, g, c, k, fg, q_new, alpha, weight, a.q2, a.sx, a.sy, pb)
        if (weight) { if (dir == 0) BND(true, 0); else BND(true, 1); }
        else { if (dir == 0) BND(false, 0); else BND(false, 1); }
#undef BND
        DS_HIP(hipGetLastError());
    }
    return 0;
}

int launch_norms(const Grid &g, const LoopCoef &c, const KktCoef &k, const FusedGeom &fg, FusedArgs a, const double *phi,
                 const double *alpha, const double *weight, const KktWork &w, hipStream_t st) {
    const i64 region = kkt_region_blocks(g);
    a.TC = fg.TC;
    if (g.Nz > 0) {
        dim3 grid((unsigned)fg.nyblk, (unsigned)fg.nxblk, (unsigned)fg.chunks);
        double *part = w.partials + 1 * region * S_COUNT;
        if (weight) DS_KLAUNCH((k_kkt_cells<true, false, true>), grid, dim3(TILE_Y, TILE_X), 0, st, g, c, k, a, phi, alpha, weight, part);
        else DS_KLAUNCH((k_kkt_cells<false, false, true>), grid, dim3(TILE_Y, TILE_X), 0, st, g, c, k, a, phi, alpha, weight, part);
    }
    struct R { const double *x; i64 n; int slot, reg; };
    const R rs[] = {{phi, g.Nphi, S_PHI2, 0},
                    {a.q, g.Nz, S_Q2, 2}, {a.q + g.offBx, g.bxLayer * g.ntl, S_Q2, 3}, {a.q + g.offBy, g.byLayer * g.ntl, S_Q2, 4},
                    {alpha, g.Nz, S_ALPHA2, 5}, {alpha + g.offBx, g.bxLayer * g.ntl, S_ALPHA2, 6},
                    {alpha + g.offBy, g.byLayer * g.ntl, S_ALPHA2, 7}};
    for (const R &r : rs) {
        if (r.n <= 0) continue;
        i64 blocks = (r.n + 256 * 64 - 1) / (256 * 64);
        if (blocks > region) blocks = region;
        double *part = w.partials + r.reg * region * S_COUNT;
        DS_KLAUNCH(k_sumsq, dim3((unsigned)blocks), dim3(256), 0, st, r.x, r.n, r.slot, part);
    }
    DS_HIP(hipGetLastError());
    return 0;
}

double *kkt_qstep_partials(const Grid &g, const KktWork &w) {
    (void)g;
    return w.partials;
}

int launch_kkt_final(const Grid &g, const KktWork &w, hipStream_t st) {
    DS_KLAUNCH(k_kkt_final, dim3(S_COUNT, KKT_SLICES), dim3(256), 0, st, w.partials,
                       KKT_REGIONS * kkt_region_blocks(g), w.sums + S_COUNT);
    DS_KLAUNCH(k_kkt_final2, dim3(1), dim3(64), 0, st, w.sums + S_COUNT, KKT_SLICES, w.sums);
    DS_HIP(hipGetLastError());
    return 0;
}

}
```

### dot-socp_amd/csrc/qstep_march.hip

```cpp
#include "device_utils.h"
#include "gather_tile.h"
#include "kernels.h"
#include "qstep_tile.h"

#include <cstdlib>

namespace dotsocp {


struct QRhsArgs {
    const double *phi, *q2v, *sx, *sy, *weight, *tail_bx, *tail_by, *cvec, *alpha_in;
    double *q_out, *alpha_out, *rhs;
    double *u0_tail;
    i64 TC, z0, zstride;
    double *q_state;
    const double *q_anchor, *alpha_anchor;
    double c1, c2, om_rho, rho;
    APend ap;
    int xcd;
    const double *qk;
    double *partials, *resid;
    double kappa, dsD;
    int c_ends;
};
// ... 114 lines not shown
            if (KKT && !lay0) {
                const double abx_m = from_left(t, xcha[par], o.aL, 0.0);
                const double aby_m = from_below(t, aby_s, o.aB);
                double ra = adjoint_sum(g, c, t, tl, a0prev, o.a0n, abx_m, o.aXn, aby_m, o.aYn);
                ra = ra - in.cv;
                a.resid[in.node] = ra;
                S[Q_DUAL1] += ra * ra;
                S[Q_CPHI] += in.cv * p0;
                S[Q_PHI2] += p0 * p0;
                if (x < g.nx - 1 && xl < QTX - 1) {
                    const double rm = (rhoN + xchr[par][xl + 1][lane]) / 2.0;
                    const double rb = a.dsD * (rm * o.qXn);
                    const double d = mbx - rb;
                    S[Q_MRHOB] += d * d;
                    S[Q_RHOB2] += rb * rb;
                }
                if (y < g.ny - 1 && lane < TILE_Y - 1) {
                    const double rm = (rhoN + rhoU) / 2.0;
                    const double rb = a.dsD * (rm * o.qYn);
                    const double d = mby - rb;
                    S[Q_MRHOB] += d * d;
                    S[Q_RHOB2] += rb * rb;
                }
            }
        }
        u0prev = o.u0;
        if (KKT) {
            a0prev = o.a0n;
            rhoTprev = rhoT;
        }
        p0 = o.pT;
        par ^= 1;
    }
    if (KKT) {
        __shared__ double red[QTX][Q_COUNT];
        static const int slot[Q_COUNT] = {S_Q2, S_ALPHA2, S_APHI2, S_PRIM1, S_QALPHA, S_CPHI, S_PHI2, S_DUAL1, S_MRHOB, S_M2, S_RHOB2};
#pragma unroll
        for (int i = 0; i < Q_COUNT; ++i) {
            double v = S[i];
#pragma unroll
            for (int off = 32; off >= 1; off >>= 1) v += __shfl_down(v, off, 64);
            if (lane == 0) red[xl][i] = v;
        }
        __syncthreads();
        if (xl == 0 && lane < S_COUNT) {
            double v = 0.0;
#pragma unroll
            for (int i = 0; i < Q_COUNT; ++i)
                if (slot[i] == lane) {
                    v = red[0][i];
#pragma unroll
                    for (int wv = 1; wv < QTX; ++wv) v += red[wv][i];
                }
            const i64 b = blk.x + (i64)gridDim.x * (blk.y + (i64)gridDim.y * ((i64)blk.z * a.zstride + a.z0));
            a.partials[b * S_COUNT + lane] = v;
        }
    }
}

static int launch_qstep_rhs_var(int var, const Grid &g, const LoopCoef &c, const FusedGeom &fg, QRhsArgs a, hipStream_t st,
                                i64 z0 = 0, i64 zcount = -1, i64 zstride = 1);

int launch_qstep_rhs(const Grid &g, const LoopCoef &c, const FusedGeom &fg, const double *phi, const double *q2,
                     const double *sx, const double *sy, const double *weight, const double *tail_bx,
                     const double *tail_by, const double *cvec, double *q_out, const double *alpha_in, double *alpha_out,
                     double *rhs, hipStream_t st, i64 z0, i64 zcount, i64 zstride, const QStepExtra *ex) {
    QRhsArgs a{};
    a.phi = phi; a.q2v = q2; a.sx = sx; a.sy = sy; a.weight = weight; a.tail_bx = tail_bx; a.tail_by = tail_by;
    a.cvec = cvec; a.alpha_in = alpha_in; a.q_out = q_out; a.alpha_out = alpha_out; a.rhs = rhs;
    a.ap = APend{0, 1.0, 1.0};
    if (ex) {
        a.ap = APend{ex->aops.n, ex->aops.mul, ex->aops.div};
        a.partials = ex->partials;
        a.resid = ex->resid;
        a.u0_tail = ex->u0_tail;
        a.kappa = ex->kappa;
        a.dsD = ex->dsD;
        a.c_ends = ex->c_ends;
    }
    return launch_qstep_rhs_var(0, g, c, fg, a, st, z0, zcount, zstride);
}

i64 qstep_rhs_blocks(const Grid &g, const FusedGeom &fg) { return fg.nyblk * fg.nxblk * qstep_rhs_chunks(g, fg); }

int launch_qstep_rhs_acc(int var, const Grid &g, const LoopCoef &c, const FusedGeom &fg, const double *phi,
                         const double *q2, const double *sx, const double *sy, const double *weight, const double *cvec,
                         double *q_raw, const double *alpha_in, double *alpha_out, double *rhs, double *q_state,
                         const double *q_anchor, const double *alpha_anchor, const AccCoef &k, hipStream_t st,
                         const double *tail_bx, const double *tail_by, double *u0_tail) {
    QRhsArgs a{};
    a.phi = phi; a.q2v = q2; a.sx = sx; a.sy = sy; a.weight = weight; a.cvec = cvec;
    a.tail_bx = tail_bx; a.tail_by = tail_by; a.u0_tail = u0_tail;
    a.alpha_in = alpha_in; a.q_out = q_raw; a.alpha_out = alpha_out; a.rhs = rhs;
    a.q_state = q_state; a.q_anchor = q_anchor; a.alpha_anchor = alpha_anchor;
    a.c1 = k.c1; a.c2 = k.c2; a.om_rho = k.om_rho; a.rho = k.rho;
    return launch_qstep_rhs_var(var, g, c, fg, a, st);
}

i64 qstep_rhs_chunks(const Grid &g, const FusedGeom &fg, i64 *TCout) {
    const i64 tiles = fg.nyblk * fg.nxblk;
    const i64 target = 32768;
    i64 chunks = (target + tiles - 1) / tiles;
    i64 TC = (g.ntl + chunks - 1) / chunks;
    if (TC < 8) TC = 8;
    if (!(g.first && g.last) && cone_split_enabled() && g.ntl >= 12) {
        const i64 tail = (g.ntl / 4 < 4) ? 4 : g.ntl / 4;
        const i64 body = g.ntl - tail, nb = (body + 7) / 8;
        TC = (body + nb - 1) / nb;
    }
    if (TC > g.ntl) TC = g.ntl;
    if (TC < 1) TC = 1;
    if (TCout) *TCout = TC;
    return (g.ntl + TC - 1) / TC;
}

static int launch_qstep_rhs_var(int var, const Grid &g, const LoopCoef &c, const FusedGeom &fg, QRhsArgs a, hipStream_t st,
                                i64 z0, i64 zcount, i64 zstride) {
    i64 TC = 1;
    const i64 chunks = qstep_rhs_chunks(g, fg, &TC);
    if (zcount < 0) zcount = chunks - z0;
    if (z0 < 0 || zcount <= 0 || zstride < 1 || z0 + (zcount - 1) * zstride >= chunks) return 0;
    a.TC = TC;
    a.z0 = z0;
    a.zstride = zstride;
    a.xcd = 1;
    dim3 grid((unsigned)fg.nyblk, (unsigned)fg.nxblk, (unsigned)zcount);
    dim3 blk(TILE_Y, TILE_X);
    const char *qe = getenv("DOTSOCP_QTX");
    const int qtx_env = qe ? atoi(qe) : 0;
    const int qtx = qtx_env ? qtx_env : ((fg.nyblk * fg.nxblk * zcount >= 8192 && !a.weight) ? 2 * TILE_X : TILE_X);
    if (var == 0 && !a.partials && qtx == 2 * TILE_X) {
        dim3 grid2((unsigned)fg.nyblk, (unsigned)((g.nx + 2 * TILE_X - 1) / (2 * TILE_X)), (unsigned)zcount);
        dim3 blk2(TILE_Y, 2 * TILE_X);
        if (a.weight) DS_KLAUNCH((k_qstep_rhs<true, 0, false, 2 * TILE_X>), grid2, blk2, 0, st, g, c, fg, a);
        else DS_KLAUNCH((k_qstep_rhs<false, 0, false, 2 * TILE_X>), grid2, blk2, 0, st, g, c, fg, a);
        DS_HIP(hipGetLastError());
        return 0;
    }
#define QRHS_LAUNCH(W, V) DS_KLAUNCH((k_qstep_rhs<W, V>), grid, blk, 0, st, g, c, fg, a)
    if (var == 0 && a.partials) {
        if (a.weight) DS_KLAUNCH((k_qstep_rhs<true, 0, true>), grid, blk, 0, st, g, c, fg, a);
        else DS_KLAUNCH((k_qstep_rhs<false, 0, true>), grid, blk, 0, st, g, c, fg, a);
    } else if (a.weight) {
        if (var == 0) QRHS_LAUNCH(true, 0); else if (var == 1) QRHS_LAUNCH(true, 1); else QRHS_LAUNCH(true, 2);
    } else {
        if (var == 0) QRHS_LAUNCH(false, 0); else if (var == 1) QRHS_LAUNCH(false, 1);
        else if (var == 2) QRHS_LAUNCH(false, 2); else QRHS_LAUNCH(false, 3);
    }
#undef QRHS_LAUNCH
    DS_HIP(hipGetLastError());
    return 0;
}

template <bool NT, bool GOUT>
__global__ void __launch_bounds__(TILE_Y *TILE_X, 3) k_qcone(Grid g, LoopCoef c, FusedGeom fg, QConeArgs a) {
    constexpr int XB = TILE_X;
    __shared__ double2 xch[2][XB][TILE_Y];
    __shared__ double ph[2][XB + 2][TILE_Y + 2];
    __shared__ double2 gch[2][XB][64];
    const APend ap{a.ap_on, a.ap_mul, a.ap_div};
    const BlockId blk = block_id(true);
    const QTile<XB> t = q_tile<XB>(g, fg, blk);
    const int lane = t.lane, xl = t.xl;
    const i64 y = t.y, x = t.x;
    const bool inb = t.inb;
    const i64 t0 = (i64)blk.z * a.TC;
    const i64 t1 = (t0 + a.TC < g.ntl) ? t0 + a.TC : g.ntl;
    const i64 tstart = (t0 >= 2) ? t0 - 2 : 0;
    const i64 tstop = (t1 == g.ntl) ? t1 + 1 : t1;
    const i64 nxblk = gridDim.y, nyblk = gridDim.x;
    const QSrc src{a.phi, a.q2v, a.sx, a.sy, nullptr, nullptr, nullptr, a.cvec, a.alpha_in, nullptr, a.c_ends};
    double p0 = 0.0;
    if (inb) {
        const i64 node0 = y + g.py * (x + g.nx * tstart);
        p0 = a.phi[node0];
        store_phi_layer<XB>(ph[0], t, p0, load_phi_halo(g, t, a.phi, node0));
    }
    double u0prev = 0.0;
    double q0c = 0.0;
    EdgeQuad eprev{0.0, 0.0, 0.0, 0.0};
    GatherCarry gc;
    int par = 0;
    __syncthreads();
    for (i64 tl = tstart; tl < tstop; ++tl) {
        const bool own = tl >= t0;
        const bool hasC = (tl > tstart) && (tl - 1 < g.ncl);
        const i64 ci = t.yc + g.py * (t.xc + g.nx * (hasC ? tl - 1 : 0));
        double b[10];
        if (hasC) {
#pragma unroll
            for (int j = 0; j < 10; ++j) b[j] = ld_stream<NT>(a.gamma_in + j * g.Nc + ci);
        }
        EdgeQuad ecur{0.0, 0.0, 0.0, 0.0};
        double q0n = 0.0;
        if (tl < g.ntl) {
            const QLayerIn in = q_layer_load<false, XB>(g, c, fg, t, src, ph[par], tl, false, false);
            const QLayerOut o = q_layer_calc<false, 0, XB>(c, t, in, ap, p0, false, false);
            q0n = o.q0n;
            if (own) {
                if (in.hasCell) {
                    a.alpha_out[in.node] = o.a0n;
                    if (!GOUT) a.q_out[in.node] = o.q0n;
                }
                if (t.hasBx) {
                    a.alpha_out[in.eX] = o.aXn;
                    if (!GOUT) a.q_out[in.eX] = o.qXn;
                }
                if (t.hasBy) {
                    a.alpha_out[in.eY] = o.aYn;
                    if (!GOUT) a.q_out[in.eY] = o.qYn;
                }
            }
            xch[par][xl][lane] = make_double2(o.ubx, o.qXn);
            store_phi_layer<XB>(ph[par ^ 1], t, in.pTl, in.h);
            __syncthreads();
            const double uby_s = __shfl_up(o.uby, 1, 64);
            const double qY_s = __shfl_up(o.qYn, 1, 64);
            if (inb) {
                const double2 r = from_left(t, xch[par], make_double2(o.ubx_l, o.qL),
                                            make_double2(0.0, 0.0));
                const double uby_m = from_below(t, uby_s, o.uby_b), qY_m = from_below(t, qY_s, o.qB);
                if (own) a.rhs[in.node] = adjoint_sum(g, c, t, tl, u0prev, o.u0, r.x, o.ubx, uby_m, o.uby) + in.cv;
                ecur.xm = (x >= 1) ? c.sf * r.y : 0.0;
                ecur.xp = (x <= g.nx - 2) ? c.sf * o.qXn : 0.0;
                ecur.ym = (y >= 1) ? c.sf * qY_m : 0.0;
                ecur.yp = (y <= g.ny - 2) ? c.sf * o.qYn : 0.0;
            }
            u0prev = o.u0;
            p0 = o.pT;
            par ^= 1;
        }
        if (tl > tstart) {
            double w[10];
            if (hasC) {
                double v[10];
                build_z2(v, q0c, eprev, ecur, c.s, c.dF);
#pragma unroll
                for (int j = 0; j < 10; ++j) b[j] = mult_finish(b[j], v[j], c.tau);
                if (!GOUT && own && inb) {
#pragma unroll
                    for (int j = 0; j < 10; ++j) st_stream<NT>(a.beta_out + j * g.Nc + ci, b[j]);
                }
#pragma unroll
                for (int j = 0; j < 10; ++j) v[j] = v[j] - b[j];
                proj_row<10>(v);
                if (GOUT && own && inb) {
#pragma unroll
                    for (int j = 0; j < 10; ++j) st_stream<NT>(a.beta_out + j * g.Nc + ci, mult_carry(b[j], v[j], c.tau));
                }
#pragma unroll
                for (int j = 0; j < 10; ++j) w[j] = v[j] + b[j];
                if (own && inb) a.q2_out[ci] = c.s * (w[9] - w[0]);
            } else {
#pragma unroll
                for (int j = 0; j < 10; ++j) w[j] = 0.0;
            }
            gather_emit<XB>(g, c.sf, gch, gc, w, tl - 1, own && inb, x, y, xl, lane, nxblk, nyblk, blk.y, blk.x, a.q2_out,
                            a.sx_out, a.sy_out);
        }
        eprev = ecur;
        q0c = q0n;
    }
}

i64 qcone_chunk_len(const Grid &g) {
    i64 TC = g.ntl;
    if (const char *e = getenv("DOTSOCP_QCONE_TC")) {
        const i64 n = atoll(e);
        if (n >= 1) TC = n;
    }
    return TC < g.ntl ? TC : g.ntl;
}

int launch_qcone(const Grid &g, const LoopCoef &c, const FusedGeom &fg, QConeArgs a, bool gout, hipStream_t st) {
    if (fg.XB != TILE_X || !(g.first && g.last) || g.ncl < 1) { set_error("internal: k_qcone on a grid it does not serve"); return DOTSOCP_ESTATE; }
    a.TC = qcone_chunk_len(g);
    const i64 chunks = (g.ntl + a.TC - 1) / a.TC;
    dim3 grid((unsigned)fg.nyblk, (unsigned)fg.nxblk, (unsigned)chunks);
    dim3 blk(TILE_Y, TILE_X);
    const bool nt = stream_nt_enabled();
    if (gout) {
        if (nt) DS_KLAUNCH((k_qcone<true, true>), grid, blk, 0, st, g, c, fg, a);
        else DS_KLAUNCH((k_qcone<false, true>), grid, blk, 0, st, g, c, fg, a);
    } else {
        if (nt) DS_KLAUNCH((k_qcone<true, false>), grid, blk, 0, st, g, c, fg, a);
        else DS_KLAUNCH((k_qcone<false, false>), grid, blk, 0, st, g, c, fg, a);
    }
    DS_HIP(hipGetLastError());
    return 0;
}

int launch_qstep_palm_first(const Grid &g, const LoopCoef &c, const FusedGeom &fg, const double *phi, const double *q2,
                            const double *sx, const double *sy, const double *cvec, double *q_out, const double *alpha,
                            double *rhs, hipStream_t st, const double *tail_bx, const double *tail_by, const double *qk) {
    QRhsArgs a{};
    a.phi = phi; a.q2v = q2; a.sx = sx; a.sy = sy; a.cvec = cvec; a.tail_bx = tail_bx; a.tail_by = tail_by;
    a.alpha_in = alpha; a.q_out = q_out; a.rhs = rhs; a.qk = qk;
    return launch_qstep_rhs_var(3, g, c, fg, a, st);
}

}
```

### dot-socp_amd/csrc/solver.h

```cpp
#pragma once
#include <chrono>
#include <functional>
#include <memory>
#include <string>
#include <vector>

#include "hostmem.h"
#include "kernels.h"

namespace dotsocp {

int guarded_malloc(void **p, size_t bytes);
void guarded_free(void *p);
long long device_cache_release();
int canary_check(std::string *report);
bool canary_enabled();
bool stream_stress_enabled();
void stream_stress(hipStream_t st);

template <class T>
inline int dmalloc(T **p, i64 n) {
    *p = nullptr;
    if (n <= 0) n = 1;
    return guarded_malloc((void **)p, sizeof(T) * (size_t)n);
}

inline void dfree(void *p) {
    if (p) guarded_free(p);
}

struct DevRes {
    int dev = 0;
    DctPlan *py = nullptr, *px = nullptr, *pt = nullptr;
    double *cy = nullptr, *cx = nullptr, *ct = nullptr;
};

#define DS_XEV 8
enum SlabEvent { EV_FORK = 0, EV_JOIN, EV_HALO, EV_CJOIN, EV_TRI, EV_MSG, EV_GOT, EV_X0 };
struct Slab {
    int index = 0;
    int dev = 0;
    hipStream_t st = nullptr;
    hipStream_t st_z = nullptr;
    hipEvent_t ev[EV_X0 + DS_XEV] = {nullptr};
    int xev_next = 0;
    DevRes *res = nullptr;
    double *h_sums = nullptr;
    Grid g;
    std::vector<void *> owned;
    template <class T> int alloc(T **p, i64 n) {
        DS_CHECK(dmalloc(p, n));
        owned.push_back(*p);
        return 0;
    }
    int zalloc(double **p, i64 n) {
        DS_CHECK(alloc(p, n));
        DS_HIP(hipMemsetAsync(*p, 0, sizeof(double) * (size_t)(n > 0 ? n : 1), st));
        return 0;
    }
    double *phi = nullptr;
    double *q = nullptr;
    double *alpha = nullptr;
    double *z = nullptr;
    double *beta = nullptr;
    double *c = nullptr;
    bool c_ends = false;
    double *weight = nullptr;
    double *w0 = nullptr, *w1 = nullptr;
    i64 l0 = 0, nl = 0;
    double *pencil = nullptr, *pencil2 = nullptr;
    double *stage = nullptr;
    double *u0_prev = nullptr, *tail_bx = nullptr, *tail_by = nullptr;
    double *a0_prev = nullptr, *a0w_prev = nullptr, *btail_bx = nullptr, *btail_by = nullptr;
    double *send_plane = nullptr, *send_plane2 = nullptr, *send_bx = nullptr, *send_by = nullptr;
    KktWork kw{};
    double *q_old = nullptr, *q2 = nullptr, *beta2 = nullptr, *sx = nullptr, *sy = nullptr;
    double *q3 = nullptr, *p2 = nullptr, *sxp = nullptr, *syp = nullptr;
    double *send_pbx = nullptr, *send_pby = nullptr, *ptail_bx = nullptr, *ptail_by = nullptr;
    double *alpha2 = nullptr;
    double *sx2 = nullptr, *sy2 = nullptr;
    double *tri_send = nullptr, *tri_recv = nullptr, *tri_bsend = nullptr, *tri_brecv = nullptr, *tri_zero = nullptr;
    double *carry = nullptr;
    FusedGeom fg{};
    double *phi_p = nullptr, *alpha_p = nullptr, *z_p = nullptr;
    double *phi_a = nullptr, *q_a = nullptr, *alpha_a = nullptr, *z_a = nullptr, *beta_a = nullptr;
    double *rep_edges = nullptr, *rep_part = nullptr, *rep_sums = nullptr;
    unsigned long long *rep_counts = nullptr;
    double *adv_vel = nullptr;
    i64 adv_have[2] = {-1, -1};
};

#define FOR_SLABS(s) for (auto &s : slabs) if (int rc_use__ = use(s)) return rc_use__; else

int dotsocp_slab_range_impl(i64 nt, int world, int rank, i64 *t0, i64 *t1);
void pencil_range(i64 plane, int world, int j, i64 *l0, i64 *l1);

bool if_adjust_sigma(double iter, double last_iter);

enum Phase { PH_RHS = 0, PH_POISSON, PH_PROJ, PH_QSTEP, PH_BETA, PH_KKT, PH_FUSED_A, PH_FUSED_B, PH_MATERIALISE,
             PH_COMM, PH_INTERP, PH_ACC_CONE, PH_ACC_GATHER, PH_QSTEP0, PH_TRANSPOSE, PH_CONE_CARRY, PH_QCONE, PH_VELOCITY, PH_ADVECT,
             PH_DEPOSIT, PH_FRAME_L1, PH_ADVECT_PATH, PH_MAP_FINAL, PH_COUNT };

bool rescale_due(i64 it, int rescale, double maxFeas, double relGap);
bool cone_writes_beta(i64 it, double lastSigmaIt, i64 maxit, bool checkStepByStep, bool last_of_run, int rescale,
                      double maxFeas, double relGap);

enum { QCONE_NONE = 0, QCONE_STEADY = 1, QCONE_EXIT = 2 };
int qcone_form(i64 it, double lastSigmaIt, i64 maxit, bool checkStepByStep, bool last_of_run, bool next_last_of_run,
               int rescale, double maxFeas, double relGap);

struct Solver {
    dotsocp_problem prob{};
    int device = 0;
    i64 ny = 0, nx = 0, nt = 0;
    hipStream_t stream = nullptr;
    hipStream_t stream_z = nullptr;
    bool multi_device = false;
    int ndev_visible = 1;
    std::vector<DevRes *> devres;
    int cur_dev = -1;
    std::vector<Slab> slabs;
    std::unique_ptr<DeferCtx> defer;
    int world = 1;
    int rank = 0;
    void *nccl = nullptr;
    double *h_sums = nullptr;
    double *d_red = nullptr;
    bool fused = true;
    bool overlap = false;
    bool tri_tsolve = true;
    bool peer_ok = true;
    bool cross_device = false;
    ~Solver();
    int init(const dotsocp_problem *p, int device, int nslabs, bool multi_dev = false);
    int attach_rccl(const unsigned char *id, int rank, int world);
    int use(const Slab &s);
    int use_dev(int d);
    int sync_all();
    DevRes *res_for(int dev);
    i64 column_pad() const;
    i64 row_pitch() const;
    int alloc_slabs(int first, int count);
    int ensure_alloc();
    void free_slabs();
    bool multi() const { return world > 1; }
    bool remote() const { return nccl != nullptr; }

    int xcopy(Slab &from, const double *src, Slab &to, double *dst, i64 count);
    int xcopy2d(Slab &from, const double *src, size_t spitch, Slab &to, double *dst, size_t dpitch, size_t width,
                size_t height);
    bool comm_z = false;
    bool comm_async = false;
    int comm_depth = 0;
    hipStream_t cst(const Slab &s) const { return comm_z ? s.st_z : s.st; }
    int comm_enter();
    int comm_leave();
    int comm_fork();
    int comm_mark(SlabEvent ev);
    int comm_wait(SlabEvent ev);
    int open_groups = 0;
    typedef std::function<double *(Slab &)> Sel;
    int shift(int dir, const Sel &src, const Sel &dst, i64 count);
    int shift_edge_halo(const Sel &base);
    int group_begin();
    int group_end();
    struct Msg { int from, to; const double *src; double *dst; i64 count; };
    std::vector<Msg> msgs;
    int msg_depth = 0;
    bool pull_default(const char *env_var) const;
    bool msg_batching() const;
    int flush_msgs();
    bool halo_pending = false;
    bool u0_fresh = false;
    bool u0_made = false;
    int make_u0_tail();
    int exchange_u0_tail();
    int exchange_q_halo(bool with_u0);
    int ensure_halo();
    int make_tails();
    int send_tails();
    int send_phi_head();
    int ship_tails();
    int transpose(bool forward);
    struct PhiHooks { std::function<int()> fill, behind; };
    int tri_alloc();
    int tri_exchange(bool back);
    int poisson_t_tridiag(const PhiHooks *hooks);

    i64 field_len(int field) const;
    enum { ROWS_DOWN = 0, ROWS_UP = 1, ROWS_FROM_DEV = 2 };
    int copy_rows(double *dev, double *host, i64 rowlen, i64 pitch, i64 nrows, int dir, hipStream_t st, int src_dev = -1);
    int upload(int field, const double *host);
    int upload_layers(int field, const double *host, i64 t0, i64 n);
    int download(int field, double *host);
    int upload_weight_from(const double *src, int src_dev, i64 src_ny, i64 src_nx, i64 src_nt);
    bool c_ends_on = true;
    int detect_c_ends();
    int stage_left_tail();
    int stage_rho_ends(Slab &s, const double *rho0, const double *rho1);
    int canary_after();
    int recover_outputs(const double *rho0, const double *rho1, double *rho, double *Ex, double *Ey, double *q0,
                        double *bx, double *by);
    int jump_from(Solver &coarse);
    int solution_report(const double *rho0, const double *rho1, dotsocp_report *rep, double *layer_mass, double *layer_neg);
    int render_evolution(const double *rho0, const double *rho1, const dotsocp_render_opts *o, const i64 *frame_nodes,
                         const double *levels, const unsigned char *lut, const unsigned char *barrier, unsigned char *image,
                         double *mvX, double *mvY, dotsocp_render_info *info);

    int velocity_stage(const double *rho0, const double *rho1);
    int velocity_layer(Slab &s, i64 tg, double floor);
    int recover_velocity(const double *rho0, const double *rho1, double floor, double *vX, double *vY);
    int advect_particles(const double *rho0, const double *rho1, const dotsocp_advect_opts *o, double *x, double *y,
                         double *traj_x, double *traj_y, i64 *n_clamped);
    int push_mass(const double *rho0, const double *rho1, const dotsocp_push_opts *o, double *x, double *y, const double *mass,
                  const i64 *frame_nodes, double *frames, i64 *n_clamped, double *unit, double *l1);
    int map_report(const double *rho0, const double *rho1, const dotsocp_advect_opts *o, double *x, double *y, const double *mass,
                   dotsocp_map_report_t *rep, double *disp, double *len, double *action);

    bool begun = false, finished = false, stopped = false;
    dotsocp_opts opts{};
    bool checkPrimDualFeas = true;
    double time_limit = 3600.0;
    double sigma = 1.0, sigmaScale = 1.0;
    double cScale = 1.0, dScale = 1.0, D = 1.0, E = 1.0;
    double norm_c = 0.0, norm_d = 0.0;
    double h = 1.0;
    int rescale = 0, use_feasOrg = 0;
    double maxFeas = 0.0, relGap = 0.0, tol_feasOrg = 0.0;
    double lastSigmaIt = 0.0;
    i64 it = 0;
    LoopCoef lc{};
    std::vector<double> hist_kkt, hist_time, hist_iter, hist_gap;
    std::chrono::steady_clock::time_point t_begin;
    double elapsed_prev = 0.0;
    double elapsed_agreed = 0.0;
    bool deferred = false;
    bool z_valid = true;
    bool z_prev_ok = false;
    bool rhs_valid = false;
    bool cone_carry = true;
    bool beta_gamma = false;
    bool cone_gout = false;
    bool last_of_run = false;
    int qcone = -1;
    bool q_valid = true;
    bool early_pass = false;
    bool early_gout = false;
    bool next_last_of_run = false;
    int need_q(const char *who) const;
    int qcone_decide() const;
    bool time_limit_passed() const;
    i64 timeout_at = -1;
    bool timeout_pending = false;
    int need_beta_form(const char *who) const;
    ScaleOps bops{0, 1.0, 1.0, 1.0, 1.0};
    ScaleOps zp_ops{0, 1.0, 1.0, 1.0, 1.0};
    int push_beta_op(double mul, double div);
    int flush_beta();
    ScaleOps aops{0, 1.0, 1.0, 1.0, 1.0};
    int flush_alpha();
    int sigma_scale_folded(double factor);
    FusedArgs pending_step_args(const Slab &s) const;
    double last_S[S_COUNT] = {0};
    double last_S_sigma = 1.0;
    i64 last_S_it = -1;
    bool norm_cache = true;
    bool kkt_fold = true;
    KktCoef kkt_coef() const;
    int clear_partials(Slab &s);
    int begin(const dotsocp_opts *o);
    int begin_method(const dotsocp_opts *o, int method, const dotsocp_acc_opts *acc);
    int run(i64 n_iters, i64 *done);
    int finish(dotsocp_result *res);
    int step(bool *brk);
    int rescale_block();
    int poisson_all(const PhiHooks *hooks = nullptr);
    int poisson_phi();
    int phase_phi(const PhiHooks *hooks = nullptr);
    int phase_z(int part = 0);
    int phase_q(int part = 0, bool kkt = false, int early = QCONE_NONE);
    int phase_mult();
    int materialise();
    int ensure_z();
    int kkt_sums(double *S, bool folded = false);
    int reduce_sums(double *S);
    int norms_light(double *S);
    int kkt_block(bool adjustSigmaYes, bool timed_out, bool *brk, bool folded = false);
    int scale_state(double a_mul, double a_div, double q_div, bool with_c);
    void update_coef();
    double elapsed() const;
    bool profiling = false;
    struct Pending { hipEvent_t a, b; int phase; };
    std::vector<Pending> pending;
    std::vector<hipEvent_t> event_pool;
    double phase_ms[PH_COUNT] = {0};
    i64 phase_launches[PH_COUNT] = {0};
    void prof_begin(int phase, bool on_z = false);
    void prof_end(int phase, bool on_z = false);
    int prof_flush();

    int method = DOTSOCP_METHOD_INPALM;
    i64 acc_restart = 100, acc_k = 0;
    double acc_rho = 2.0, acc_theta = 2.0;
    bool acc_halpern = true;
    bool acc_gather_valid = false;
    bool acc_swapped = false;
    bool acc_post = true;
    bool acc_light = false;
    double acc_factor = 1.0;
    int acc_alloc();
    int acc_begin(const dotsocp_acc_opts *acc);
    int acc_step(bool *brk);
    int acc_rescale_block();
    int acc_set_anchors();
    void acc_swap_state();
    int acc_on_sigma_factor(double factor);
    AccCoef acc_coef() const;
    bool palm_fast = true;
    bool palm_p_valid = false;
    int palm_begin();
    int palm_step(bool *brk);
};

struct DeviceScratch {
    Solver &S;
    std::vector<double *> bufs;
    explicit DeviceScratch(Solver &s) : S(s) {}
    int alloc(double **p, i64 n) { DS_CHECK(dmalloc(p, n)); bufs.push_back(*p); return 0; }
    ~DeviceScratch() {
        if (bufs.empty()) return;
        S.cur_dev = -1;
        (void)S.sync_all();
        for (double *b : bufs) dfree(b);
    }
};

}
```

### dot-socp_amd/csrc/solver.hip

```cpp
#include "solver.h"

#include <algorithm>
#include <cmath>
#include <cstring>

#include "comm.h"

namespace dotsocp {

void Solver::update_coef() {
    lc.s = E / D;
    lc.sf = edge_factor(lc.s);
    lc.dF = E / dScale;
    const double ht = 1.0 / (double)(nt - 1);
    lc.at = D * (1.0 / ht);
    lc.ax = (nx > 1) ? D * (1.0 / (1.0 / (double)(nx - 1))) : 0.0;
    lc.ay = (ny > 1) ? D * (1.0 / (1.0 / (double)(ny - 1))) : 0.0;
    lc.tau = opts.tau;
    const double tmp = (E / D) * (E / D);
    if (prob.weighted) { lc.c1 = 2.0 * tmp; lc.c2 = tmp; }
    else { lc.c1 = 1.0 + 2.0 * tmp; lc.c2 = 1.0 + tmp; }
    lc.dinv1 = 1.0 / lc.c1;
    lc.dinv2 = 1.0 / lc.c2;
}

int Solver::need_beta_form(const char *who) const {
    if (!beta_gamma) return 0;
    set_error("internal: %s met the gamma form of beta", who);
    return DOTSOCP_ESTATE;
}

int Solver::need_q(const char *who) const {
    if (q_valid) return 0;
    set_error("internal: %s met a q that was never stored", who);
    return DOTSOCP_ESTATE;
}

int Solver::flush_beta() {
    DS_CHECK(need_beta_form("flush_beta"));
    if (bops.empty()) return 0;
    FOR_SLABS(s) {
        DS_CHECK(launch_scale(s.beta, 10 * s.g.Nc, bops.mul, bops.div, s.st));
        if (bops.n > 1) DS_CHECK(launch_scale(s.beta, 10 * s.g.Nc, bops.mul2, bops.div2, s.st));
    }
    bops.clear();
    return 0;
}

int Solver::push_beta_op(double mul, double div) {
    if (bops.push(mul, div)) return 0;
    DS_CHECK(flush_beta());
    bops.push(mul, div);
    return 0;
}

FusedArgs Solver::pending_step_args(const Slab &s) const {
    FusedArgs a{};
    a.q_old = s.q_old;
    a.q = s.q;
    a.beta_in = s.beta;
    a.bops = bops;
    return a;
}

int Solver::clear_partials(Slab &s) {
    DS_HIP(ds_memset_async(s.kw.partials, 0, sizeof(double) * s.kw.maxBlocks * S_COUNT, s.st));
    return 0;
}

int Solver::flush_alpha() {
    if (aops.empty()) return 0;
    FOR_SLABS(s) DS_CHECK(launch_scale(s.alpha, s.g.NqAlloc, aops.mul, aops.div, s.st));
    aops.clear();
    return 0;
}

int Solver::sigma_scale_folded(double factor) {
    DS_CHECK(flush_alpha());
    DS_CHECK(ensure_halo());
    u0_made = false;
    DS_CHECK(push_beta_op(1.0, factor));
    if (multi()) {
        FOR_SLABS(s) DS_CHECK(launch_scale(s.alpha, s.g.NqAlloc, 1.0, factor, s.st));
    } else {
        aops.push(1.0, factor);
    }
    u0_fresh = false;
    FOR_SLABS(s) DS_CHECK(launch_rhs_sigma_fix(s.g, s.w0, s.w1, s.c, factor, s.st, c_ends_on && s.c_ends));
    return 0;
}

int Solver::scale_state(double a_mul, double a_div, double q_div, bool with_c) {
    DS_CHECK(need_beta_form("scale_state"));
    DS_CHECK(need_q("scale_state"));
    DS_CHECK(flush_alpha());
    if (begun) DS_CHECK(ensure_halo());
    u0_made = false;
    u0_fresh = false;
    rhs_valid = false;
    if (fused && begun) {
        DS_CHECK(push_beta_op(a_mul, a_div));
    }
    FOR_SLABS(s) {
        const Grid &g = s.g;
        if (with_c) DS_CHECK(launch_scale(s.c, g.Nphi, a_mul, a_div, s.st));
        if (!acc_light) DS_CHECK(launch_scale(s.alpha, g.NqAlloc, a_mul, a_div, s.st));
        if (!(fused && begun) && !acc_light) DS_CHECK(launch_scale(s.beta, 10 * g.Nc, a_mul, a_div, s.st));
        if (q_div != 1.0) {
            DS_CHECK(launch_scale(s.q, g.NqAlloc, 1.0, q_div, s.st));
            if (!(fused && begun) || z_valid) DS_CHECK(launch_scale(s.z, 10 * g.Nc, 1.0, q_div, s.st));
        }
    }
    if (q_div != 1.0 && fused && begun && !z_valid) z_prev_ok = false;
    return 0;
}

int Solver::begin_method(const dotsocp_opts *o, int m, const dotsocp_acc_opts *acc) {
    if (begun) { set_error("begin() called twice"); return DOTSOCP_ESTATE; }
    if (m == DOTSOCP_METHOD_INPALM) return begin(o);
    DS_ARG(m == DOTSOCP_METHOD_ACCADMM || m == DOTSOCP_METHOD_PALM, "unknown method");
    DS_ARG(prob.dim == 2, "the reference has PALM and acc-ADMM loops for 2-D problems only");
    DS_ARG(!(m == DOTSOCP_METHOD_PALM && prob.weighted), "the reference has no weighted PALM loop");
    method = m;
    int rc = begin(o);
    if (rc != 0) { method = DOTSOCP_METHOD_INPALM; return rc; }
    return (m == DOTSOCP_METHOD_PALM) ? palm_begin() : acc_begin(acc);
}

int Solver::begin(const dotsocp_opts *o) {
    DS_ARG(o != nullptr, "opts is NULL");
    DS_ARG(o->maxit >= 0, "opts.maxit < 0");
    DS_ARG(o->sigma > 0, "opts.sigma must be positive");
    if (begun) { set_error("begin() called twice"); return DOTSOCP_ESTATE; }
    cur_dev = -1;
    DS_CHECK(use_dev(device));
    DS_CHECK(ensure_alloc());
    if (method == DOTSOCP_METHOD_ACCADMM) {
        DS_CHECK(acc_alloc());
        fused = false;
    }
    opts = *o;
    cone_carry = true;
    if (const char *e = getenv("DOTSOCP_CONE_CARRY")) cone_carry = (atoi(e) != 0);
    c_ends_on = true;
    if (const char *e = getenv("DOTSOCP_C_ENDS")) c_ends_on = (atoi(e) != 0);
    if (c_ends_on) DS_CHECK(detect_c_ends());
    timeout_at = -1;
    if (const char *e = getenv("DOTSOCP_TEST_TIMEOUT_AT")) timeout_at = atoll(e);
    qcone = -1;
    if (const char *e = getenv("DOTSOCP_QCONE")) qcone = atoi(e);
    if (qcone < -1 || qcone > 2) qcone = -1;
    q_valid = true;
    early_pass = false;
    early_gout = false;
    next_last_of_run = false;
    beta_gamma = false;
    cone_gout = false;
    last_of_run = false;
    timeout_pending = false;
    checkPrimDualFeas = (o->checkPrimDualFeas < 0) ? !prob.weighted : (o->checkPrimDualFeas != 0);
    time_limit = (o->time_limit > 0) ? o->time_limit : 3600.0;
    sigma = o->sigma;
    lastSigmaIt = -INFINITY;
    cScale = prob.cScale; dScale = prob.dScale; D = prob.D; E = prob.E;
    use_feasOrg = 0;
    tol_feasOrg = 5 * o->tol;
    rescale = o->scaling ? 1 : 0;
    maxFeas = INFINITY; relGap = INFINITY;
    h = 1.0 / ((double)nx * (double)ny * (double)nt);
    norm_c = prob.normc; norm_d = prob.normd;
    update_coef();
    DS_CHECK(scale_state(1.0, sigma, 1.0, true));
    DS_CHECK(exchange_q_halo(false));
    sigmaScale = 1.0;
    it = 0;
    stopped = false;
    deferred = false;
    z_valid = true;
    z_prev_ok = false;
    rhs_valid = false;
    last_S_it = -1;
    hist_kkt.clear(); hist_time.clear(); hist_iter.clear(); hist_gap.clear();
    for (int i = 0; i < PH_COUNT; ++i) { phase_ms[i] = 0; phase_launches[i] = 0; }
    if (canary_enabled() && getenv("DOTSOCP_CANARY_SELFTEST")) {
        Slab &s0 = slabs[0];
        DS_CHECK(use(s0));
        const double v = 1.0;
        DS_HIP(ds_memcpy_async(s0.c + s0.g.Nphi, &v, sizeof v, hipMemcpyHostToDevice, s0.st));
        DS_HIP(ds_stream_synchronize(s0.st));
    }
    begun = true;
    elapsed_prev = 0.0;
    elapsed_agreed = 0.0;
    t_begin = std::chrono::steady_clock::now();
    return 0;
}

int Solver::poisson_all(const PhiHooks *hooks) {
    const i64 plane = slabs[0].g.plane;
    const bool tp2 = dct_plan_has_tsolve(devres[0]->pt);
    FOR_SLABS(s) {
        const Grid &g = s.g;
        DS_CHECK(launch_dct_axis(s.res->py, s.w0, s.w1, g.ny, g.nx, g.ntl, 0, 0, s.st, g.py));
        DS_CHECK(launch_dct_axis(s.res->px, s.w1, s.w0, g.ny, g.nx, g.ntl, 1, 0, s.st, g.py));
    }
    bool tri = multi() && tri_tsolve && world <= DS_MAX_WORLD;
    for (auto &s : slabs) tri = tri && s.g.ntl <= TRI_EXTRA;
    if (tri) {
        DS_CHECK(poisson_t_tridiag(hooks));
    } else {
    if (hooks && hooks->fill) {
        prof_end(PH_POISSON);
        DS_CHECK(hooks->fill());
        prof_begin(PH_POISSON);
    }
    if (hooks && hooks->behind) DS_CHECK(hooks->behind());
    if (multi()) {
        prof_begin(PH_TRANSPOSE);
        DS_CHECK(transpose(true));
        prof_end(PH_TRANSPOSE);
    }
    FOR_SLABS(s) {
        double *p = multi() ? s.pencil : s.w0;
        double *p2 = multi() ? s.pencil2 : s.w1;
        if (!multi()) {
            DS_CHECK(launch_poisson_t_single(s.res->pt, s.g, D * D, s.res->cy, s.res->cx, s.res->ct, p, p2, s.g.py, s.st, tri_tsolve));
        } else if (tp2) {
            DS_CHECK(launch_dct_t_solve(s.res->pt, p, p, s.g.py, plane, s.l0, s.nl, nt, D * D, s.res->cy, s.res->cx, s.res->ct, s.st));
        } else {
            DS_CHECK(launch_dct_axis(s.res->pt, p, p2, s.nl, 1, nt, 2, 0, s.st));
            DS_CHECK(launch_spectral_divide_pencil(p2, s.g.py, s.l0, s.nl, nt, D * D, s.res->cy, s.res->cx, s.res->ct, s.st));
            DS_CHECK(launch_dct_axis(s.res->pt, p2, p, s.nl, 1, nt, 2, 1, s.st));
        }
    }
    if (multi()) {
        prof_begin(PH_TRANSPOSE);
        DS_CHECK(transpose(false));
        prof_end(PH_TRANSPOSE);
    }
    }
    FOR_SLABS(s) {
        const Grid &g = s.g;
        DS_CHECK(launch_dct_axis(s.res->px, s.w0, s.w1, g.ny, g.nx, g.ntl, 1, 1, s.st, g.py));
        DS_CHECK(launch_dct_axis(s.res->py, s.w1, s.phi, g.ny, g.nx, g.ntl, 0, 1, s.st, g.py));
    }
    return 0;
}

int Solver::poisson_phi() {
    if (begun) { set_error("poisson_phi() must precede begin()"); return DOTSOCP_ESTATE; }
    cur_dev = -1;
    DS_CHECK(use_dev(device));
    DS_CHECK(ensure_alloc());
    D = prob.D;
    FOR_SLABS(s) DS_HIP(ds_memcpy_async(s.w0, s.phi, sizeof(double) * (size_t)s.g.Nphi, hipMemcpyDeviceToDevice, s.st));
    DS_CHECK(poisson_all(nullptr));
    return sync_all();
}

int Solver::phase_phi(const PhiHooks *hooks) {
    DS_CHECK(ensure_halo());
    if (multi() && !u0_fresh) {
        DS_CHECK(make_u0_tail());
        prof_begin(PH_COMM, comm_z);
        DS_CHECK(exchange_u0_tail());
        prof_end(PH_COMM, comm_z);
    }
    prof_begin(PH_RHS);
    if (!rhs_valid) {
        DS_CHECK(need_q("phase_phi"));
        DS_CHECK(flush_alpha());
        FOR_SLABS(s) DS_CHECK(launch_rhs(s.g, lc, s.q, s.alpha, s.c, s.weight, s.u0_prev, s.w0, s.st, c_ends_on && s.c_ends));
    } else if (multi()) {
        FOR_SLABS(s)
            if (!s.g.first) DS_CHECK(launch_rhs_fixup(s.g, lc, s.u0_prev, s.w0, s.st));
    }
    rhs_valid = false;
    prof_end(PH_RHS);
    prof_begin(PH_POISSON);
    DS_CHECK(poisson_all(hooks));
    prof_end(PH_POISSON);
    return 0;
}

int Solver::phase_z(int part) {
    if (early_pass) {
        early_pass = false;
        if (part != 0 || !fused || !deferred || cone_gout != early_gout) {
            set_error("internal: the early cone pass wrote %s, the schedule asks for %s", early_gout ? "gamma" : "beta",
                      cone_gout ? "gamma" : "beta");
            return DOTSOCP_ESTATE;
        }
        return 0;
    }
    DS_CHECK(need_q("phase_z"));
    if (part != 1) DS_CHECK(ensure_halo());
    if (!fused) {
        prof_begin(PH_PROJ);
        FOR_SLABS(s) DS_CHECK(launch_cone_proj(s.g, lc, s.q, s.beta, s.z, s.st));
        prof_end(PH_PROJ);
        return 0;
    }
    const bool gin = beta_gamma, gout = deferred && cone_gout;
    if (gin && (!deferred || !bops.empty())) {
        set_error("internal: gamma form %s", deferred ? "with a pending scaling of beta" : "without a pending multiplier step");
        return DOTSOCP_ESTATE;
    }
    const int flavour = (gin ? CONE_GIN : 0) | (gout ? CONE_GOUT : 0);
    const int ph = deferred ? (gin ? PH_CONE_CARRY : PH_FUSED_B) : PH_FUSED_A;
    z_valid = false;
    z_prev_ok = false;
    prof_begin(ph);
    FOR_SLABS(s) {
        FusedArgs a{};
        a.q = s.q;
        a.q2 = s.q2;
        a.sx = s.sx;
        a.sy = s.sy;
        a.beta_in = s.beta;
        a.bops = bops;
        const i64 C = s.fg.chunks;
        const i64 z0 = (part == 2) ? C - 1 : 0;
        const i64 zc = (part == 0) ? C : ((part == 1) ? C - 1 : 1);
        if (deferred) {
            a.q_old = s.q_old;
            a.beta_out = s.beta2;
        }
        const int mode = deferred ? 1 : 0;
        if (s.carry && C > 1) {
            for (i64 z = z0; z < z0 + zc; ++z) {
                a.carry_in = (z > 0) ? s.carry : nullptr;
                a.carry_out = (z + 1 < C) ? s.carry : nullptr;
                DS_CHECK(launch_cone_fused(mode, s.g, lc, s.fg, a, s.st, z, 1, flavour));
            }
        } else {
            DS_CHECK(launch_cone_fused(mode, s.g, lc, s.fg, a, s.st, z0, zc, flavour));
        }
        if (deferred && part != 1) std::swap(s.beta, s.beta2);
    }
    prof_end(ph);
    if (part == 1) return 0;
    if (deferred) {
        bops.clear();
        beta_gamma = gout;
    }
    return 0;
}

KktCoef Solver::kkt_coef() const {
    KktCoef k;
    k.sigma = sigma;
    k.kappa = sigma * cScale * D;
    k.dsD = dScale / D;
    k.dsE = dScale / E;
    return k;
}

int Solver::phase_q(int part, bool kkt, int early) {
    if (!fused) DS_CHECK(flush_alpha());
    if (early != QCONE_NONE && (part != 0 || kkt || multi() || !fused || !deferred || !beta_gamma || !bops.empty())) {
        set_error("internal: early cone pass in a state it does not serve");
        return DOTSOCP_ESTATE;
    }
    const bool egout = (early == QCONE_STEADY);
    const int ph = (early != QCONE_NONE) ? PH_QCONE : PH_QSTEP;
    prof_begin(ph);
    FOR_SLABS(s) {
        hipStream_t st = s.st;
        if (early != QCONE_NONE && qcone != 2) {
            if (!s.sx2) {
                DS_CHECK(s.zalloc(&s.sx2, s.fg.sx_len));
                DS_CHECK(s.zalloc(&s.sy2, s.fg.sy_len));
            }
            QConeArgs a{};
            a.phi = s.phi; a.q2v = s.q2; a.sx = s.sx; a.sy = s.sy; a.cvec = s.c; a.alpha_in = s.alpha; a.gamma_in = s.beta;
            a.alpha_out = s.alpha2; a.rhs = s.w0; a.q_out = s.q_old; a.beta_out = s.beta2;
            a.q2_out = s.q; a.sx_out = s.sx2; a.sy_out = s.sy2;
            a.ap_on = aops.n; a.ap_mul = aops.mul; a.ap_div = aops.div;
            a.c_ends = (c_ends_on && s.c_ends) ? 1 : 0;
            DS_CHECK(launch_qcone(s.g, lc, s.fg, a, egout, st));
            std::swap(s.alpha, s.alpha2);
            std::swap(s.q, s.q_old);
            std::swap(s.q2, s.q_old);
            std::swap(s.sx, s.sx2);
            std::swap(s.sy, s.sy2);
            std::swap(s.beta, s.beta2);
        } else if (!fused) {
            DS_CHECK(launch_qstep(s.g, lc, s.phi, s.z, s.beta, s.weight, s.tail_bx, s.tail_by, s.q, s.alpha, s.st));
        } else {
            const i64 C = qstep_rhs_chunks(s.g, s.fg);
            i64 z0 = 0, zc = C, zs = 1;
            if (part == 1) { zc = C - 1; }
            else if (part == 2) { z0 = C - 1; zc = 1; }
            QStepExtra ex{};
            ex.aops = aops;
            ex.c_ends = (c_ends_on && s.c_ends) ? 1 : 0;
            if (multi() && !s.g.last && part != 1) ex.u0_tail = s.send_plane;
            if (kkt) {
                const KktCoef k = kkt_coef();
                ex.partials = kkt_qstep_partials(s.g, s.kw);
                ex.resid = s.w1;
                ex.kappa = k.kappa; ex.dsD = k.dsD;
            }
            DS_CHECK(launch_qstep_rhs(s.g, lc, s.fg, s.phi, s.q2, s.sx, s.sy, s.weight, s.tail_bx, s.tail_by, s.c,
                                      s.q_old, s.alpha, s.alpha2, s.w0, st, z0, zc, zs, &ex));
            if (part != 1) std::swap(s.alpha, s.alpha2);
            if (part != 1) std::swap(s.q, s.q_old);
            if (early != QCONE_NONE) {
                FusedArgs a{};
                a.q = s.q; a.q2 = s.q2; a.sx = s.sx; a.sy = s.sy;
                a.beta_in = s.beta; a.beta_out = s.beta2;
                a.bops = bops;
                DS_CHECK(launch_cone_fused(1, s.g, lc, s.fg, a, s.st, 0, s.fg.chunks, CONE_GIN | (egout ? CONE_GOUT : 0)));
                std::swap(s.beta, s.beta2);
            }
        }
    }
    prof_end(ph);
    if (part == 1) return 0;
    q_valid = true;
    if (early != QCONE_NONE) {
        q_valid = !egout || qcone == 2;
        beta_gamma = egout;
        z_valid = false;
        z_prev_ok = false;
        early_pass = true;
        early_gout = egout;
    }
    u0_made = multi() && fused;
    if (fused) aops.clear();
    rhs_valid = fused;
    if (multi() && fused && comm_z && cone_split_enabled()) halo_pending = true;
    else DS_CHECK(exchange_q_halo(true));
    return 0;
}

int Solver::phase_mult() {
    if (fused) {
        deferred = true;
        return 0;
    }
    prof_begin(PH_BETA);
    FOR_SLABS(s) DS_CHECK(launch_beta_update(s.g, lc, s.q, s.z, s.beta, s.st));
    prof_end(PH_BETA);
    return 0;
}

int Solver::materialise() {
    if (!fused || !deferred) return 0;
    DS_CHECK(need_beta_form("materialise"));
    DS_CHECK(need_q("materialise"));
    DS_CHECK(ensure_halo());
    prof_begin(PH_MATERIALISE);
    FOR_SLABS(s) {
        FusedArgs a = pending_step_args(s);
        a.beta_out = s.beta;
        a.z_out = s.z;
        DS_CHECK(launch_cone_fused(2, s.g, lc, s.fg, a, s.st));
    }
    prof_end(PH_MATERIALISE);
    bops.clear();
    deferred = false;
    z_valid = true;
    return 0;
}

int Solver::ensure_z() {
    if (!fused || z_valid) return 0;
    DS_CHECK(need_beta_form("ensure_z"));
    DS_CHECK(need_q("ensure_z"));
    if (deferred) return materialise();
    if (!z_prev_ok) {
        set_error("internal: z cannot be regenerated");
        return DOTSOCP_ESTATE;
    }
    DS_CHECK(ensure_halo());
    prof_begin(PH_MATERIALISE);
    FOR_SLABS(s) {
        FusedArgs a{};
        a.q_old = s.q_old;
        a.q = s.q;
        a.beta_in = s.beta2;
        a.z_out = s.z;
        a.bops = zp_ops;
        DS_CHECK(launch_cone_fused(3, s.g, lc, s.fg, a, s.st));
    }
    prof_end(PH_MATERIALISE);
    z_valid = true;
    return 0;
}

int Solver::kkt_sums(double *S, bool folded) {
    DS_CHECK(need_beta_form("kkt_sums"));
    DS_CHECK(need_q("kkt_sums"));
    DS_CHECK(ensure_halo());
    const KktCoef k = kkt_coef();
    if (method == DOTSOCP_METHOD_ACCADMM && folded) {
        FOR_SLABS(s) DS_CHECK(launch_kkt_nodual(s.g, lc, k, s.phi, s.q, s.alpha, s.c, s.weight, s.kw, s.st));
        return reduce_sums(S);
    }
    if (!folded) {
        DS_CHECK(flush_alpha());
        FOR_SLABS(s) DS_CHECK(clear_partials(s));
    }
    int rest = folded ? 0 : (1 | 4 | 8);
    if (fused && deferred) {
        FOR_SLABS(s) {
            FusedArgs a = pending_step_args(s);
            a.beta_out = s.beta2;
            if (folded) { a.q2 = s.q2; a.sx = s.sx; a.sy = s.sy; }
            DS_CHECK(launch_kkt_cells_update(s.g, lc, k, s.fg, a, s.phi, s.alpha, s.weight, s.kw, s.st, folded, s.q));
            std::swap(s.beta, s.beta2);
        }
        zp_ops = bops;
        bops.clear();
        deferred = false;
        z_valid = false;
        z_prev_ok = true;
    } else {
        if (folded) { set_error("internal: folded KKT sums without a pending multiplier step"); return DOTSOCP_ESTATE; }
        DS_CHECK(ensure_z());
        DS_CHECK(flush_beta());
        rest |= 2;
    }
    if (multi()) {
        const i64 plane = slabs[0].g.plane;
        u0_made = false;
        FOR_SLABS(s)
            if (!s.g.last)
                DS_CHECK(launch_kkt_tail(s.g, s.alpha, s.beta, s.weight, s.send_plane, s.send_plane2, s.send_bx, s.send_by,
                                         s.st));
        DS_CHECK(group_begin());
        DS_CHECK(shift(+1, [](Slab &s) { return s.send_plane; }, [](Slab &s) { return s.a0_prev; }, plane));
        DS_CHECK(shift(+1, [](Slab &s) { return s.send_plane2; }, [](Slab &s) { return s.a0w_prev; }, plane));
        DS_CHECK(shift(+1, [](Slab &s) { return s.send_bx; }, [](Slab &s) { return s.btail_bx; }, slabs[0].g.bxLayer));
        DS_CHECK(shift(+1, [](Slab &s) { return s.send_by; }, [](Slab &s) { return s.btail_by; }, slabs[0].g.byLayer));
        DS_CHECK(group_end());
    }
    FOR_SLABS(s) {
        KktHalo halo{s.a0_prev, s.a0w_prev, s.btail_bx, s.btail_by};
        if (rest) DS_CHECK(launch_kkt(s.g, lc, k, s.phi, s.q, s.alpha, s.z, s.beta, s.c, s.weight, halo, s.kw, rest, s.st));
        if (folded && !s.g.first)
            DS_CHECK(launch_kkt(s.g, lc, k, s.phi, s.q, s.alpha, s.z, s.beta, s.c, s.weight, halo, s.kw, 1 | 4 | 8, s.st, true,
                                s.w1));
    }
    return reduce_sums(S);
}

int Solver::reduce_sums(double *S) {
    for (int i = 0; i <= S_COUNT; ++i) S[i] = 0.0;
    FOR_SLABS(s) {
        DS_CHECK(launch_kkt_final(s.g, s.kw, s.st));
        if (remote()) break;
        DS_HIP(ds_memcpy_async(s.h_sums, s.kw.sums, sizeof(double) * S_COUNT, hipMemcpyDeviceToHost, s.st));
    }
    if (!remote()) {
        FOR_SLABS(s) {
            DS_HIP(ds_stream_synchronize(s.st));
            for (int i = 0; i < S_COUNT; ++i) S[i] += s.h_sums[i];
        }
    }
    S[S_COUNT] = elapsed();
    if (remote()) {
        Rccl &api = rccl_api();
        Slab &s = slabs[0];
        DS_CHECK(comm_enter());
        const hipStream_t cs = cst(s);
        DS_NCCL(api.AllReduce(s.kw.sums, d_red, S_COUNT, ncclDouble, ncclSum, (ncclComm_t)nccl, cs));
        h_sums[S_COUNT] = S[S_COUNT];
        DS_HIP(ds_memcpy_async(d_red + S_COUNT, h_sums + S_COUNT, sizeof(double), hipMemcpyHostToDevice, cs));
        DS_NCCL(api.AllReduce(d_red + S_COUNT, d_red + S_COUNT, 1, ncclDouble, ncclMax, (ncclComm_t)nccl, cs));
        DS_HIP(ds_memcpy_async(h_sums, d_red, sizeof(double) * (S_COUNT + 1), hipMemcpyDeviceToHost, cs));
        DS_CHECK(comm_leave());
        DS_HIP(ds_stream_synchronize(stream));
        for (int i = 0; i <= S_COUNT; ++i) S[i] = h_sums[i];
    }
    elapsed_agreed = S[S_COUNT];
    return 0;
}

int Solver::norms_light(double *S) {
    DS_CHECK(need_beta_form("norms_light"));
    DS_CHECK(need_q("norms_light"));
    DS_CHECK(ensure_halo());
    DS_CHECK(flush_alpha());
    const KktCoef k = kkt_coef();
    FOR_SLABS(s) {
        DS_CHECK(clear_partials(s));
        const FusedArgs a = pending_step_args(s);
        DS_CHECK(launch_norms(s.g, lc, k, s.fg, a, s.phi, s.alpha, s.weight, s.kw, s.st));
    }
    return reduce_sums(S);
}

int Solver::rescale_block() {
    bool scaleYes = false;
    double normPhis = 0, normAlps = 0;
    auto norms = [&](double &nPhis, double &nAlps) -> int {
        double S[S_COUNT + 1];
        double sig = sigma;
        if (method == DOTSOCP_METHOD_INPALM && fused && last_S_it == it - 1 && norm_cache) {
            for (int i = 0; i < S_COUNT; ++i) S[i] = last_S[i];
            sig = last_S_sigma;
        } else if (method == DOTSOCP_METHOD_INPALM && fused && deferred && norm_cache) {
            DS_CHECK(norms_light(S));
        } else {
            DS_CHECK(materialise());
            DS_CHECK(ensure_z());
            DS_CHECK(kkt_sums(S));
        }
        const double sh = sqrt(h);
        const double normPhi = sh * sqrt(S[S_PHI2]), normQ = sh * sqrt(S[S_Q2]), normZ = sh * sqrt(S[S_Z2]);
        const double normAlpha = sig * (sh * sqrt(S[S_ALPHA2])), normBeta = sig * (sh * sqrt(S[S_BETA2]));
        nPhis = std::max(std::max(normPhi, normQ), normZ);
        nAlps = std::max(normAlpha, normBeta);
        return 0;
    };
    if (rescale_due(it, rescale, maxFeas, relGap)) DS_CHECK(need_beta_form("rescale_block"));
    if (rescale >= 3 && (it % 100) == 0) {
        DS_CHECK(norms(normPhis, normAlps));
        const double ratio = std::max(normAlps, normPhis) / std::min(normAlps, normPhis);
        if (ratio > 1.2) scaleYes = true;
    }
    const bool first = (rescale == 1) && (maxFeas < 2e-2) && (it >= 10) && (relGap < 5e-2);
    const bool second = (rescale == 2) && (maxFeas < 5e-3) && (it >= 50) && (relGap < 1e-2);
    if (!(first || second || scaleYes)) return 0;
    if (!scaleYes) DS_CHECK(norms(normPhis, normAlps));
    DS_CHECK(materialise());
    const double dScale2 = normPhis, cScale2 = normAlps;
    sigma = sigma * (cScale2 / dScale2);
    norm_c = norm_c / cScale2;
    if (!prob.weighted) norm_d = norm_d / dScale2;
    DS_CHECK(scale_state(dScale2, cScale2 * cScale2, dScale2, true));
    if (method == DOTSOCP_METHOD_PALM) {
        FOR_SLABS(s) DS_CHECK(launch_scale(s.phi, s.g.NphiAlloc, 1.0, dScale2, s.st));
    }
    dScale = dScale2 * dScale;
    cScale = cScale2 * cScale;
    sigmaScale = sigmaScale * (cScale2 / dScale2);
    update_coef();
    rescale += 1;
    return 0;
}

bool rescale_due(i64 it, int rescale, double maxFeas, double relGap) {
    if (rescale >= 3 && (it % 100) == 0) return true;
    if (rescale == 1 && maxFeas < 2e-2 && it >= 10 && relGap < 5e-2) return true;
    if (rescale == 2 && maxFeas < 5e-3 && it >= 50 && relGap < 1e-2) return true;
    return false;
}

bool cone_writes_beta(i64 it, double lastSigmaIt, i64 maxit, bool checkStepByStep, bool last_of_run, int rescale,
                      double maxFeas, double relGap) {
    if (checkStepByStep || if_adjust_sigma((double)it, lastSigmaIt) || it >= maxit) return true;
    if (last_of_run) return true;
    return rescale_due(it + 1, rescale, maxFeas, relGap);
}

int qcone_form(i64 it, double lastSigmaIt, i64 maxit, bool checkStepByStep, bool last_of_run, bool next_last_of_run,
               int rescale, double maxFeas, double relGap) {
    if (cone_writes_beta(it, lastSigmaIt, maxit, checkStepByStep, last_of_run, rescale, maxFeas, relGap)) return QCONE_NONE;
    return cone_writes_beta(it + 1, lastSigmaIt, maxit, checkStepByStep, next_last_of_run, rescale, maxFeas, relGap)
               ? QCONE_EXIT : QCONE_STEADY;
}

bool Solver::time_limit_passed() const {
    return timeout_pending || (remote() ? false : (elapsed() > time_limit || (timeout_at > 0 && it >= timeout_at)));
}

int Solver::qcone_decide() const {
    if (qcone == 0 || !fused || multi() || prob.weighted || method != DOTSOCP_METHOD_INPALM) return QCONE_NONE;
    if (!deferred || !beta_gamma || !bops.empty()) return QCONE_NONE;
    const Slab &s = slabs[0];
    if (s.g.ncl < 1 || s.fg.XB != 4) return QCONE_NONE;
    if (qcone < 0 && s.fg.nyblk * s.fg.nxblk < 2048) return QCONE_NONE;
    if (time_limit_passed()) return QCONE_NONE;
    return qcone_form(it, lastSigmaIt, opts.maxit, opts.ifCheckStepByStep != 0, last_of_run, next_last_of_run, rescale,
                      maxFeas, relGap);
}

bool if_adjust_sigma(double iter, double last_iter) {
    const double passed = iter - last_iter;
    if (iter < 20 && passed >= 3) return true;
    if (iter < 50 && passed >= 6) return true;
    if (iter < 100 && passed >= 10) return true;
    if (iter < 200 && passed >= 15) return true;
    if (iter < 500 && passed >= 25) return true;
    return passed >= 40;
}

static const double kUpdateRule[11][2] = {
    {1.1, 1.10}, {1.2, 1.15}, {1.5, 1.20}, {2, 1.26}, {2.5, 1.28}, {3.33, 1.32},
    {5, 1.35}, {10, 1.40}, {20, 1.60}, {40, 1.80}, {50, 2.00}};

static double get_factor(double xi) {
    double factor = 1.0;
    for (int i = 0; i < 11; ++i) {
        if (xi >= kUpdateRule[i][0]) factor = kUpdateRule[i][1];
        else break;
    }
    return factor;
}

static void adjust_lagrangian_param(double &sigma, double xi, double &factor) {
    factor = 1.0;
    if (xi >= 1) factor = get_factor(xi);
    else if (xi < 1) factor = 1.0 / get_factor(1.0 / xi);
    if (factor != 1.0) {
        const double old = sigma;
        sigma = std::max(std::min(sigma * factor, 1e3), 1e-3);
        factor = sigma / old;
    }
}

int Solver::kkt_block(bool adjustSigmaYes, bool timed_out, bool *brk, bool folded) {
    double S[S_COUNT + 1];
    prof_begin(PH_KKT);
    DS_CHECK(kkt_sums(S, folded));
    prof_end(PH_KKT);
    if (remote()) timed_out = elapsed_agreed > time_limit;
    for (int i = 0; i < S_COUNT; ++i) last_S[i] = S[i];
    last_S_sigma = sigma;
    last_S_it = it;
    const double sh = sqrt(h);
    auto nrm = [&](int i) { return sh * sqrt(S[i]); };
    const double norm_q = nrm(S_Q2), norm_z = nrm(S_Z2), norm_Aphi = nrm(S_APHI2);
    const double norm_alpha = sigma * nrm(S_ALPHA2), norm_beta = sigma * nrm(S_BETA2);
    const double norm_FBbeta = sigma * nrm(S_FBBETA2);
    const double primFea1 = nrm(S_PRIM1), primFea2 = nrm(S_PRIM2);
    const double dualFea1 = sigma * nrm(S_DUAL1), dualFea2 = sigma * nrm(S_DUAL2);
    const double complem = nrm(S_COMPLEM);
    const double dotcomplem = nrm(S_DOTCOMP), normRho = nrm(S_RHO2), norm_rhoFq = nrm(S_RHOFQ2);
    const double mRhoB = nrm(S_MRHOB), normM = nrm(S_M2), normRhoB = nrm(S_RHOB2);
    const double kc = 1.0;
    const double den2 = prob.weighted ? (norm_q + norm_z) : norm_d;
    double org[7], res[5];
    org[0] = primFea1 / (kc * D / dScale + norm_Aphi + norm_q);
    org[1] = primFea2 / (kc * E / dScale + den2);
    org[2] = dualFea1 / (kc / cScale + norm_c);
    org[3] = complem / (kc * E / dScale + norm_z + norm_beta);
    org[4] = dualFea2 / (kc / cScale / D + norm_FBbeta + norm_alpha);
    org[5] = dotcomplem / (kc + normRho + norm_rhoFq);
    org[6] = mRhoB / (kc + normM + normRhoB);
    res[0] = primFea1 / (kc + norm_Aphi + norm_q);
    res[1] = primFea2 / (kc + den2);
    res[2] = dualFea1 / (kc + norm_c);
    res[3] = complem / (kc + norm_z + norm_beta);
    res[4] = dualFea2 / (kc + norm_FBbeta + norm_alpha);
    const double priVal = (sigma * cScale * dScale * h) * S[S_QALPHA];
    const double dualVal = (sigma * cScale * dScale * h) * S[S_CPHI];
    const double pdGap = fabs(priVal - dualVal) / (1 + fabs(priVal) + fabs(dualVal));
    for (int i = 0; i < 7; ++i) hist_kkt.push_back(org[i]);
    hist_time.push_back(remote() ? elapsed_agreed : elapsed());
    hist_iter.push_back((double)it);
    hist_gap.push_back(pdGap);
    double mstop = std::max(std::max(org[0], org[2]), org[5]);
    if (checkPrimDualFeas) mstop = std::max(mstop, org[6]);
    if (mstop < opts.tol || timed_out) {
        *brk = true;
        return 0;
    }
    const double maxRes = *std::max_element(res, res + 5);
    if (maxRes < tol_feasOrg) use_feasOrg = 1;
    if (adjustSigmaYes) {
        lastSigmaIt = (double)it;
        double resiPri, resiDual;
        if (use_feasOrg) { resiPri = std::max(org[0], org[1]); resiDual = std::max(org[2], org[4]); }
        else { resiPri = std::max(res[0], res[1]); resiDual = std::max(res[2], res[4]); }
        double factor;
        adjust_lagrangian_param(sigma, resiPri / resiDual, factor);
        if (factor != 1.0) {
            if (folded && rhs_valid && method != DOTSOCP_METHOD_ACCADMM) DS_CHECK(sigma_scale_folded(factor));
            else DS_CHECK(scale_state(1.0, factor, 1.0, true));
            if (method == DOTSOCP_METHOD_ACCADMM) DS_CHECK(acc_on_sigma_factor(factor));
        }
    }
    if (rescale > 0) {
        maxFeas = maxRes;
        relGap = pdGap;
    }
    return 0;
}

int Solver::step(bool *brk) {
    *brk = false;
    if (method == DOTSOCP_METHOD_ACCADMM) return acc_step(brk);
    if (method == DOTSOCP_METHOD_PALM) return palm_step(brk);
    it += 1;
    DS_CHECK(rescale_block());
    const bool adjustSigmaYes = if_adjust_sigma((double)it, lastSigmaIt);
    const bool early_steady = early_pass && early_gout;
    const bool kkt_due = opts.ifCheckStepByStep || adjustSigmaYes || it == opts.maxit || (timeout_pending && !early_steady);
    cone_gout = cone_carry && fused && deferred && !kkt_due &&
                !cone_writes_beta(it, lastSigmaIt, opts.maxit, opts.ifCheckStepByStep != 0, last_of_run, rescale, maxFeas, relGap);
    const bool fold = kkt_due && kkt_fold && fused;
    const bool inter = comm_z && multi() && fused;
    bool split = inter && cone_split_enabled();
    for (auto &s : slabs) split = split && s.fg.chunks >= 2;
    bool split_q = inter && cone_split_enabled();
    for (auto &s : slabs) split_q = split_q && qstep_rhs_chunks(s.g, s.fg) >= 2;
    auto async_comm = [&](const std::function<int()> &fn, SlabEvent ev) -> int {
        DS_CHECK(comm_fork());
        comm_async = true;
        const int rc = fn();
        comm_async = false;
        DS_CHECK(rc);
        return comm_mark(ev);
    };
    if (inter) {
        const bool pend = halo_pending;
        if (pend) {
            DS_CHECK(make_u0_tail());
            DS_CHECK(async_comm([&]() { return ensure_halo(); }, EV_HALO));
        }
        if (split) DS_CHECK(phase_z(1));
        if (pend) DS_CHECK(comm_wait(EV_HALO));
        if (!split) DS_CHECK(phase_z(0));
        PhiHooks hooks;
        hooks.fill = [&]() -> int {
            if (split) DS_CHECK(phase_z(2));
            return make_tails();
        };
        hooks.behind = [&]() -> int { return async_comm([&]() { return send_tails(); }, EV_JOIN); };
        DS_CHECK(phase_phi(&hooks));
    } else {
        DS_CHECK(phase_phi());
        DS_CHECK(phase_z(0));
    }
    if (fold) {
        FOR_SLABS(s) DS_CHECK(clear_partials(s));
    }
    if (inter) {
        DS_CHECK(async_comm([&]() { return send_phi_head(); }, EV_HALO));
        DS_CHECK(comm_wait(EV_JOIN));
        if (split_q) DS_CHECK(phase_q(1, fold));
        DS_CHECK(comm_wait(EV_HALO));
        DS_CHECK(phase_q(split_q ? 2 : 0, fold));
    } else {
        DS_CHECK(ship_tails());
        DS_CHECK(phase_q(0, fold, fold ? QCONE_NONE : qcone_decide()));
    }
    DS_CHECK(phase_mult());
    const bool timed_out = time_limit_passed();
    timeout_pending = false;
    if (timed_out && (beta_gamma || early_pass)) {
        timeout_pending = true;
        return 0;
    }
    if (kkt_due || timed_out)
        DS_CHECK(kkt_block(adjustSigmaYes, timed_out, brk, fold));
    return 0;
}

int Solver::run(i64 n_iters, i64 *done) {
    if (!begun || finished) { set_error("run() needs begin() and must precede finish()"); return DOTSOCP_ESTATE; }
    cur_dev = -1;
    DS_CHECK(use_dev(device));
    struct DeferScope {
        DeferCtx *ctx;
        int err = 0;
        explicit DeferScope(DeferCtx *c) : ctx(c) { if (ctx) { g_defer = ctx; ctx->begin(); } }
        int close() { if (ctx) { err = ctx->end(); g_defer = nullptr; ctx = nullptr; } return err; }
        ~DeferScope() { (void)close(); }
    } scope(defer.get());
    i64 n = 0;
    while (it < opts.maxit && !stopped) {
        if (n_iters >= 0 && n >= n_iters) break;
        bool brk = false;
        last_of_run = (n_iters >= 0 && n + 1 >= n_iters);
        next_last_of_run = (n_iters >= 0 && n + 2 >= n_iters);
        DS_CHECK(step(&brk));
        if (brk) stopped = true;
        ++n;
    }
    DS_CHECK(need_beta_form("the end of run()"));
    DS_CHECK(need_q("the end of run()"));
    if (early_pass) { set_error("internal: an early cone pass is pending at the end of run()"); return DOTSOCP_ESTATE; }
    DS_CHECK(ensure_halo());
    DS_CHECK(sync_all());
    DS_CHECK(prof_flush());
    if (const int derr = scope.close()) {
        set_error("a HIP call issued by a slab thread failed: %s", hipGetErrorString((hipError_t)derr));
        return DOTSOCP_EHIP;
    }
    if (done) *done = n;
    return 0;
}

int Solver::finish(dotsocp_result *res) {
    if (!begun) { set_error("finish() before begin()"); return DOTSOCP_ESTATE; }
    cur_dev = -1;
    DS_CHECK(use_dev(device));
    DS_CHECK(ensure_z());
    DS_CHECK(flush_beta());
    DS_CHECK(flush_alpha());
    DS_CHECK(sync_all());
    DS_CHECK(prof_flush());
    if (canary_enabled()) {
        std::string rep;
        const int bad = canary_check(&rep);
        cur_dev = -1;
        if (bad) {
            set_error("canary: %d device buffer(s) written out of bounds: %s", bad, rep.c_str());
            return DOTSOCP_EHIP;
        }
    }
    finished = true;
    if (res) {
        memset(res, 0, sizeof *res);
        res->sigma = sigma / sigmaScale;
        res->sigma_internal = sigma;
        res->cScale = cScale;
        res->dScale = dScale;
        res->times[0] = (phase_ms[PH_RHS] + phase_ms[PH_POISSON]) * 1e-3;
        res->times[1] = (phase_ms[PH_PROJ] + phase_ms[PH_FUSED_A] + phase_ms[PH_FUSED_B] + phase_ms[PH_CONE_CARRY]) * 1e-3;
        res->times[2] = phase_ms[PH_QSTEP] * 1e-3;
        res->times[3] = (phase_ms[PH_BETA] + phase_ms[PH_MATERIALISE]) * 1e-3;
        res->times[4] = phase_ms[PH_KKT] * 1e-3;
        res->times[5] = elapsed();
        res->times[6] = (double)it;
        res->iters = it;
        res->hist_len = (i64)hist_iter.size();
        res->stopped = stopped ? 1 : 0;
        if (method == DOTSOCP_METHOD_PALM) res->time_extra = phase_ms[PH_QSTEP0] * 1e-3;
        if (method == DOTSOCP_METHOD_ACCADMM) {
            res->times[0] = (phase_ms[PH_RHS] + phase_ms[PH_POISSON]) * 1e-3;
            res->times[1] = phase_ms[PH_ACC_CONE] * 1e-3;
            res->times[2] = (phase_ms[PH_QSTEP] + phase_ms[PH_ACC_GATHER]) * 1e-3;
            res->times[3] = 0.0;
            res->time_extra = phase_ms[PH_INTERP] * 1e-3;
        }
    }
    return 0;
}
void Solver::prof_begin(int phase, bool on_z) {
    if (!profiling) return;
    (void)use_dev(device);
    hipStream_t st = on_z ? stream_z : stream;
    Pending p;
    p.phase = phase;
    auto get = [&]() {
        hipEvent_t e;
        if (!event_pool.empty()) { e = event_pool.back(); event_pool.pop_back(); }
        else (void)hipEventCreate(&e);
        return e;
    };
    p.a = get();
    p.b = get();
    (void)ds_event_record(p.a, st);
    pending.push_back(p);
}

void Solver::prof_end(int phase, bool on_z) {
    if (!profiling) return;
    (void)use_dev(device);
    hipStream_t st = on_z ? stream_z : stream;
    for (auto it2 = pending.rbegin(); it2 != pending.rend(); ++it2)
        if (it2->phase == phase) { (void)ds_event_record(it2->b, st); break; }
}

int Solver::prof_flush() {
    if (!profiling || pending.empty()) return 0;
    DS_CHECK(use_dev(device));
    DS_HIP(ds_stream_synchronize(stream_z));
    DS_HIP(ds_stream_synchronize(stream));
    for (auto &p : pending) {
        float ms = 0.f;
        if (hipEventElapsedTime(&ms, p.a, p.b) == hipSuccess) {
            phase_ms[p.phase] += ms;
            phase_launches[p.phase] += 1;
        }
        event_pool.push_back(p.a);
        event_pool.push_back(p.b);
    }
    pending.clear();
    return 0;
}

double Solver::elapsed() const {
    return elapsed_prev + std::chrono::duration<double>(std::chrono::steady_clock::now() - t_begin).count();
}

}
```

### dot-socp_amd/solvers.py

```python
import ctypes
import time

import numpy as np

from . import capi
from .examples import SpaceWeight
from .model import (InitialScaling, ModelHandle, VarHandle, check_massConservation, initialize,
                    recover_q, recover_RhoE, recoverOrgVar)
from .weights import WeightPyramid

TIME_NAMES = ['Step_1_1_FFT', 'Step_1_2_ProjSOC', 'Step_2_Q_Step', 'Step_3_Multiplier', 'KKT',
              'Total_Time', 'Iters']
ACC_TIME_NAMES = ['Step_1_Q_Step', 'Step_2_Multiplier', 'Step_3_1_FFT', 'Step_3_2_ProjSOC', 'KKT', 'Interp',
                  'Total_Time', 'Iters']
WACC_TIME_NAMES = ['Step_1_Q_Step', 'Step_2_Multiplier', 'Step_3_1_FFT', 'Step_3_2_ProjSOC', 'Step_4_Interp', 'KKT',
                   'Total_Time', 'Iters']
PALM_TIME_NAMES = ['Step_1_Q_Step', 'Step_2_1_FFT', 'Step_2_2_ProjSOC', 'Step_3_Q_Step', 'Step_4_Multiplier', 'KKT',
                   'Total_Time', 'Iters']
METHODS = {"inPALM": capi.METHOD_INPALM, "ALG2": capi.METHOD_INPALM, "PALM": capi.METHOD_PALM,
           "acc-ADMM": capi.METHOD_ACCADMM}


def _get(opts, name, default=None):
    if isinstance(opts, dict):
        return opts.get(name, default)
    return getattr(opts, name, default)


def _has(opts, name):
    return (name in opts) if isinstance(opts, dict) else hasattr(opts, name)


def _ptr(a):
    return None if a is None else capi.fptr(a)


class InPALMContext:

    def __init__(self, var, opts, model, weighted=False, device=0, nslabs=1, profiling=False, rccl=None,
                 method="inPALM", warm_from=None, ngpu=None, z_unread=False, weight_from=None):
        L = capi.lib()
        self.method = method
        one_d = not hasattr(model, "ny")
        p = capi.Problem()
        p.dim = 1 if one_d else 2
        p.weighted = 1 if weighted else 0
        p.ny = 1 if one_d else int(model.ny)
        p.nx, p.nt = int(model.nx), int(model.nt)
        p.D, p.E, p.cScale, p.dScale = float(var.D), float(var.E), float(var.cScale), float(var.dScale)
        p.normc, p.normd = float(model.normc), float(model.normd)
        self.var, self.model, self.weighted = var, model, weighted
        if ngpu is not None and int(ngpu) > 1:
            self._ctx = L.dotsocp_create_multi(ctypes.byref(p), int(device), int(ngpu))
        else:
            self._ctx = L.dotsocp_create(ctypes.byref(p), int(device), int(nslabs))
        if not self._ctx:
            raise capi.DotsocpError(-1, L.dotsocp_last_error().decode())
        try:
            if rccl is not None:
                uid, rk, wd = rccl
                buf = (ctypes.c_ubyte * 128).from_buffer_copy(bytes(uid))
                capi.check(L.dotsocp_attach_rccl(self._ctx, buf, int(rk), int(wd)))
            skip_z = z_unread and METHODS[method] == capi.METHOD_INPALM and int(_get(opts, "maxit")) >= 1
            state = () if warm_from is not None else ((capi.F_PHI, var.phi), (capi.F_Q, var.q), (capi.F_ALPHA, var.alpha),
                                                      (capi.F_Z, None if skip_z else var.z), (capi.F_BETA, var.beta))
            for f, a in state:
                if a is not None:
                    self.upload(f, a)
            ends = getattr(model, "_c_ends", None)
            if ends is not None and model.c.size > 2 * ends and rccl is None:
                nlay = model.c.size // ends
                for t, part in ((0, model.c[:ends]), (nlay - 1, model.c[model.c.size - ends:])):
                    capi.check(L.dotsocp_upload_layers(self._ctx, capi.F_C, capi.fptr(np.ascontiguousarray(part)), t, 1))
            else:
                self.upload(capi.F_C, model.c)
            if weighted and weight_from is not None:
                weight_from[0].upload_to(self, weight_from[1])
            elif weighted:
                self.upload(capi.F_WEIGHT, model.weight)
            if warm_from is not None:
                capi.check(L.dotsocp_jump_next_level(warm_from._ctx, self._ctx))
            if profiling:
                capi.check(L.dotsocp_set_profiling(self._ctx, 1))
            o = capi.Opts()
            o.tau = float(_get(opts, "tau", 1.0) if method == "acc-ADMM" else _get(opts, "tau"))
            o.sigma, o.tol = float(_get(opts, "sigma")), float(_get(opts, "tol"))
            o.maxit = int(_get(opts, "maxit"))
            o.ifCheckStepByStep = int(bool(_get(opts, "ifCheckStepByStep", False)))
            o.checkPrimDualFeas = int(bool(_get(opts, "checkPrimDualFeas"))) if _has(opts, "checkPrimDualFeas") else -1
            o.scaling = int(bool(_get(opts, "scaling", False)))
            o.time_limit = float(_get(opts, "time_limit", 3600))
            if METHODS[method] == capi.METHOD_INPALM:
                capi.check(L.dotsocp_begin(self._ctx, ctypes.byref(o)))
            else:
                a = capi.AccOpts()
                a.restart = int(_get(opts, "restart", 0) or 0)
                a.rho = float(_get(opts, "rho", 0) or 0)
                a.theta = float(_get(opts, "theta", 0) or 0)
                capi.check(L.dotsocp_begin_method(self._ctx, ctypes.byref(o), METHODS[method], ctypes.byref(a)))
        except Exception:
            self.close()
            raise

    def upload(self, field, arr):
        a = np.asfortranarray(arr, dtype=np.float64)
        capi.check(capi.lib().dotsocp_upload(self._ctx, field, capi.fptr(a)))

    def download(self, field, like):
        out = np.empty(like.shape, dtype=np.float64, order="F")
        capi.check(capi.lib().dotsocp_download(self._ctx, field, capi.fptr(out)))
        return out

    def run(self, n_iters=-1):
        done = capi.i64()
        capi.check(capi.lib().dotsocp_run(self._ctx, int(n_iters), ctypes.byref(done)))
        return done.value

    def synchronize(self):
        capi.check(capi.lib().dotsocp_synchronize(self._ctx))

    def kernel_time(self, name):
        ms, n = capi.dbl(), capi.i64()
        capi.check(capi.lib().dotsocp_kernel_time(self._ctx, name.encode(), ctypes.byref(ms), ctypes.byref(n)))
        return ms.value, n.value

    def finish(self, download=True):
        L = capi.lib()
        res = capi.Result()
        capi.check(L.dotsocp_finish(self._ctx, ctypes.byref(res)))
        var = self.var
        var.name = {"acc-ADMM": 'Accelerated ADMM', "PALM": 'Proximal ALM'}.get(self.method, 'Inexact Proximal ALM')
        if download:
            var.phi = self.download(capi.F_PHI, var.phi)
            var.q = self.download(capi.F_Q, var.q)
            var.z = self.download(capi.F_Z, var.z)
            var.alpha = self.download(capi.F_ALPHA, var.alpha)
            var.beta = self.download(capi.F_BETA, var.beta)
        t = list(res.times)
        if self.method == "acc-ADMM":
            tm = dict(Step_1_Q_Step=t[2], Step_2_Multiplier=t[3], Step_3_1_FFT=t[0], Step_3_2_ProjSOC=t[1], KKT=t[4],
                      Interp=res.time_extra, Step_4_Interp=res.time_extra, Total_Time=t[5], Iters=t[6])
            var.time = {k: tm[k] for k in (WACC_TIME_NAMES if self.weighted else ACC_TIME_NAMES)}
        elif self.method == "PALM":
            var.time = dict(zip(PALM_TIME_NAMES, [res.time_extra] + t))
        else:
            var.time = dict(zip(TIME_NAMES, t))
        var.cScale, var.dScale = res.cScale, res.dScale
        n = int(res.hist_len)
        kkt = np.empty((n, 7), order="F")
        tm, itr, gap = np.empty(n), np.empty(n), np.empty(n)
        capi.check(L.dotsocp_get_history(self._ctx, capi.fptr(kkt) if n else None, capi.fptr(tm) if n else None,
                                         capi.fptr(itr) if n else None, capi.fptr(gap) if n else None))
        runHist = dict(kkt=kkt, time=tm, iter=itr, pdGap=gap, len=n)
        self.result = res
        return runHist, res.sigma

    def _rho_ends(self):
        if getattr(self, "_ends", None) is None:
            self._ends = (np.asfortranarray(self.model.rho0, dtype=np.float64), np.asfortranarray(self.model.rho1, dtype=np.float64))
        return self._ends

    def outputs(self):
        m = self.model
        one_d = not hasattr(m, "ny")
        nt = int(m.nt)
        shp = (int(m.nx),) if one_d else (int(m.ny), int(m.nx))
        names = ("rho", "Ex", "q0", "bx") if one_d else ("rho", "Ex", "Ey", "q0", "bx", "by")
        out = {k: np.empty(shp + ((nt - 1,) if k in ("q0", "bx", "by") else (nt,)), order="F") for k in names}
        r0, r1 = self._rho_ends()
        ptr = lambda k: capi.fptr(out[k]) if k in out else None
        capi.check(capi.lib().dotsocp_recover_outputs(self._ctx, capi.fptr(r0), capi.fptr(r1), ptr("rho"), ptr("Ex"),
                                                      ptr("Ey"), ptr("q0"), ptr("bx"), ptr("by")))
        return out

    def report(self):
        from .report import from_struct
        m = self.model
        nt = int(m.nt)
        r0, r1 = self._rho_ends()
        rep, mass, neg = capi.Report(), np.empty(nt), np.empty(nt)
        capi.check(capi.lib().dotsocp_solution_report(self._ctx, capi.fptr(r0), capi.fptr(r1), ctypes.byref(rep),
                                                      capi.fptr(mass), capi.fptr(neg)))
        return from_struct(rep, mass, neg)

    def render(self, frames=None, num_frame=6, mode="imshow", nlevels=128, lut=None, barrier=None, vmax=None, arrows=False,
               barrier_index=255, levels=None):
        from . import render as R
        m = self.model
        one_d = not hasattr(m, "ny")
        nt = int(m.nt)
        shp = (int(m.nx),) if one_d else (int(m.ny), int(m.nx))
        if mode not in R.MODES:
            raise ValueError("render(): mode must be one of %s" % sorted(R.MODES))
        nodes = R.frame_nodes(nt, num_frame) if frames is None else np.array(frames, dtype=np.int64).ravel()
        o = capi.RenderOpts()
        o.mode, o.channels, o.nf = R.MODES[mode], 1 if lut is None else 3, int(nodes.size)
        o.barrier_index, o.vmax = int(barrier_index), float(vmax) if vmax is not None else 0.0
        lv = None
        if mode == "levels":
            lv = np.ascontiguousarray(R.log_levels(nlevels) if levels is None else levels, dtype=np.float64).ravel()
            o.nlevels = int(lv.size)
        table = None if lut is None else R.check_lut(lut)
        b = R.barrier_mask(barrier, shp)
        mask = None if b is None else np.asfortranarray(b, dtype=np.uint8)
        Ex = Ey = None
        if arrows:
            a = dict(arrows) if isinstance(arrows, dict) else {}
            sy, sx = R.movement_skips(1 if one_d else shp[0], shp[-1])
            o.skip_y, o.skip_x = (1 if one_d else int(a.get("skip_y", sy))), int(a.get("skip_x", sx))
            o.mask_frac = float(a.get("mask_frac", R.MASK_FRAC))
            if o.skip_y >= 1 and o.skip_x >= 1:
                cut = tuple(-(-n // s) for n, s in zip(shp, (o.skip_x,) if one_d else (o.skip_y, o.skip_x)))
                Ex = np.empty(cut + (nodes.size,), order="F")
                Ey = None if one_d else np.empty(cut + (nodes.size,), order="F")
        image = np.empty((nodes.size,) + shp + (() if lut is None else (3,)), dtype=np.uint8)
        info = capi.RenderInfo()
        r0, r1 = self._rho_ends()
        ptr = lambda a: None if a is None else a.ctypes.data
        capi.check(capi.lib().dotsocp_render_evolution(self._ctx, capi.fptr(r0), capi.fptr(r1), ctypes.byref(o), nodes.ctypes.data,
                                                       ptr(lv), ptr(table), ptr(mask), image.ctypes.data, ptr(Ex), ptr(Ey),
                                                       ctypes.byref(info)))
        out = dict(image=image, nodes=nodes, vmax=float(info.vmax), rho_min=float(info.rho_min), nonfinite=int(info.nonfinite),
                   masked=int(info.masked))
        if Ex is not None:
            out["Ex"] = Ex
        if Ey is not None:
            out["Ey"] = Ey
        return out

    def _rho_floor(self, rho_floor):
        from .advect import default_rho_floor
        return default_rho_floor(self.model.rho0, self.model.rho1) if rho_floor is None else float(rho_floor)

    def velocity(self, rho_floor=None):
        m = self.model
        one_d = not hasattr(m, "ny")
        shp = ((int(m.nx),) if one_d else (int(m.ny), int(m.nx))) + (int(m.nt),)
        v = {k: np.empty(shp, order="F") for k in (("vx",) if one_d else ("vx", "vy"))}
        r0, r1 = self._rho_ends()
        capi.check(capi.lib().dotsocp_recover_velocity(self._ctx, capi.fptr(r0), capi.fptr(r1), self._rho_floor(rho_floor),
                                                       capi.fptr(v["vx"]), None if one_d else capi.fptr(v["vy"])))
        return v

    def _march_inputs(self, who, x, y, mass, nsub, direction, rho_floor):
        one_d = not hasattr(self.model, "ny")
        if one_d != (y is None):
            raise ValueError("%s(): y is given on a 2-D context and only there" % who)
        if who == "push_forward" and mass is None:
            raise ValueError("%s(): mass is needed" % who)
        px = np.array(x, dtype=np.float64).ravel()
        py = None if one_d else np.array(y, dtype=np.float64).ravel()
        ms = None if mass is None else np.array(mass, dtype=np.float64).ravel()
        if (py is not None and py.size != px.size) or (ms is not None and ms.size != px.size):
            raise ValueError("%s(): %s" % (who, "x and y hold the same number of seeds" if who == "advect" else
                                           "x, y and mass hold one entry per seed"))
        o = capi.PushOpts() if who == "push_forward" else capi.AdvectOpts()
        o.n, o.nsub, o.direction, o.rho_floor = int(px.size), int(nsub), int(direction), self._rho_floor(rho_floor)
        return (one_d, px, py, ms, o) + tuple(capi.fptr(r) for r in self._rho_ends())

    def advect(self, x, y=None, nsub=1, direction=+1, rho_floor=None, trajectories=False):
        one_d, px, py, _, o, r0, r1 = self._march_inputs("advect", x, y, None, nsub, direction, rho_floor)
        nt = int(self.model.nt)
        tx = np.empty((px.size, nt), order="F") if trajectories else None
        ty = np.empty((px.size, nt), order="F") if trajectories and not one_d else None
        nc = capi.i64()
        capi.check(capi.lib().dotsocp_advect_particles(self._ctx, r0, r1, ctypes.byref(o), _ptr(px), _ptr(py), _ptr(tx), _ptr(ty),
                                                       ctypes.byref(nc)))
        return dict(x=px, y=py, traj_x=tx, traj_y=ty, n_clamped=int(nc.value))

    def push_forward(self, x, y=None, mass=None, frames=None, nsub=1, direction=+1, rho_floor=None):
        one_d, px, py, ms, o, r0, r1 = self._march_inputs("push_forward", x, y, mass, nsub, direction, rho_floor)
        m = self.model
        nodes = np.arange(int(m.nt), dtype=np.int64) if frames is None else np.array(frames, dtype=np.int64).ravel()
        o.nf = int(nodes.size)
        shp = (int(m.nx),) if one_d else (int(m.ny), int(m.nx))
        fr = np.empty(shp + (nodes.size,), order="F")
        l1 = np.empty(nodes.size)
# ... 313 lines not shown
```

### include/dotsocp.h

```cpp
#ifndef DOTSOCP_H
#define DOTSOCP_H

#ifdef __cplusplus
extern "C" {
#endif

typedef long long dotsocp_i64;

enum {
    DOTSOCP_OK = 0,
    DOTSOCP_EINVAL = -1,
    DOTSOCP_ENODEVICE = -2,
    DOTSOCP_EHIP = -3,
    DOTSOCP_ESTATE = -4,
    DOTSOCP_ECOMM = -5
};

const char *dotsocp_last_error(void);
const char *dotsocp_version(void);
int dotsocp_device_count(void);
dotsocp_i64 dotsocp_release_cache(void);


int dotsocp_proj_soc(double *out, const double *in, dotsocp_i64 M, dotsocp_i64 K);

int dotsocp_bfd(double *z, const double *q, dotsocp_i64 nt, dotsocp_i64 nx, dotsocp_i64 ny,
                double scale, double dF);

int dotsocp_bfd_conj(double *q, const double *z, dotsocp_i64 nt, dotsocp_i64 nx, dotsocp_i64 ny,
                     double scale);

int dotsocp_bfd1d(double *z, const double *q, dotsocp_i64 nt, dotsocp_i64 nx, double scale, double dF);

int dotsocp_bfd_conj1d(double *q, const double *z, dotsocp_i64 nt, dotsocp_i64 nx, double scale);

int dotsocp_oper_poisson(double *res, const double *rhs, dotsocp_i64 ny, dotsocp_i64 nx,
                         dotsocp_i64 nt, double kernelScale);

int dotsocp_dctn(double *a, dotsocp_i64 ny, dotsocp_i64 nx, dotsocp_i64 nt, int inverse);

int dotsocp_proj_soc_dev(double *d_out, const double *d_in, dotsocp_i64 M, dotsocp_i64 K, void *stream);
int dotsocp_bfd_dev(double *d_z, const double *d_q, dotsocp_i64 nt, dotsocp_i64 nx, dotsocp_i64 ny,
                    double scale, double dF, void *stream);
int dotsocp_bfd_conj_dev(double *d_q, const double *d_z, dotsocp_i64 nt, dotsocp_i64 nx, dotsocp_i64 ny,
                         double scale, void *stream);


typedef struct dotsocp_ctx dotsocp_ctx;

typedef struct {
    int dim;
    int weighted;
    dotsocp_i64 ny, nx, nt;
    double D, E;
    double cScale, dScale;
    double normc, normd;
} dotsocp_problem;

typedef struct {
    double tau;
    double sigma;
    double tol;
    dotsocp_i64 maxit;
    int ifCheckStepByStep;
    int checkPrimDualFeas;
    int scaling;
    double time_limit;
} dotsocp_opts;

enum {
    DOTSOCP_METHOD_INPALM = 0,
    DOTSOCP_METHOD_PALM = 1,
    DOTSOCP_METHOD_ACCADMM = 2
};

typedef struct {
    dotsocp_i64 restart;
    double rho;
    double theta;
} dotsocp_acc_opts;

enum {
    DOTSOCP_F_PHI = 0,
    DOTSOCP_F_Q = 1,
    DOTSOCP_F_ALPHA = 2,
    DOTSOCP_F_Z = 3,
    DOTSOCP_F_BETA = 4,
    DOTSOCP_F_C = 5,
    DOTSOCP_F_WEIGHT = 6
};

typedef struct {
    double sigma;
    double sigma_internal;
    double cScale, dScale;
    double times[7];
    dotsocp_i64 iters;
    dotsocp_i64 hist_len;
    int stopped;
    double time_extra;
} dotsocp_result;

dotsocp_ctx *dotsocp_create(const dotsocp_problem *prob, int device, int nslabs);
dotsocp_ctx *dotsocp_create_multi(const dotsocp_problem *prob, int first_device, int ngpu);
void dotsocp_destroy(dotsocp_ctx *ctx);

int dotsocp_rccl_unique_id(unsigned char id[128]);
int dotsocp_attach_rccl(dotsocp_ctx *ctx, const unsigned char id[128], int rank, int world);

int dotsocp_slab_range(dotsocp_i64 nt, int world, int rank, dotsocp_i64 *t0, dotsocp_i64 *t1);

dotsocp_i64 dotsocp_field_len(const dotsocp_problem *prob, int field);

int dotsocp_dct_algorithm(dotsocp_i64 n);

int dotsocp_cdft_levels(dotsocp_i64 n);

int dotsocp_dct_levels(dotsocp_i64 n, int axis);

int dotsocp_tsolve_tri_safe(dotsocp_i64 ny, dotsocp_i64 nx, dotsocp_i64 nt);

int dotsocp_cone_writes_beta(dotsocp_i64 it, double last_sigma_it, dotsocp_i64 maxit, int check_step_by_step,
                             int last_of_run, int rescale, double maxFeas, double relGap);
int dotsocp_rescale_due(dotsocp_i64 it, int rescale, double maxFeas, double relGap);
int dotsocp_qcone_form(dotsocp_i64 it, double last_sigma_it, dotsocp_i64 maxit, int check_step_by_step, int last_of_run,
                       int next_last_of_run, int rescale, double maxFeas, double relGap);

int dotsocp_upload(dotsocp_ctx *ctx, int field, const double *host);
int dotsocp_download(dotsocp_ctx *ctx, int field, double *host);
int dotsocp_upload_layers(dotsocp_ctx *ctx, int field, const double *host, dotsocp_i64 t0, dotsocp_i64 n);

int dotsocp_begin(dotsocp_ctx *ctx, const dotsocp_opts *opts);
int dotsocp_begin_method(dotsocp_ctx *ctx, const dotsocp_opts *opts, int method, const dotsocp_acc_opts *acc);
int dotsocp_run(dotsocp_ctx *ctx, dotsocp_i64 n_iters, dotsocp_i64 *done);
int dotsocp_finish(dotsocp_ctx *ctx, dotsocp_result *res);

int dotsocp_recover_outputs(dotsocp_ctx *ctx, const double *rho0, const double *rho1, double *rho, double *Ex,
                            double *Ey, double *q0, double *bx, double *by);

#define DOTSOCP_REPORT_BINS 49
#define DOTSOCP_REPORT_RHO_FLOOR 1e-8
typedef struct {
    dotsocp_i64 n_nodes, n_cells;
    double mass_err, neg_err;
    double rho_min;  dotsocp_i64 rho_neg;
    dotsocp_i64 rho_hist[DOTSOCP_REPORT_BINS];
    double fq_max;   dotsocp_i64 fq_pos;
    dotsocp_i64 fq_hist[DOTSOCP_REPORT_BINS];
    double cost;
    dotsocp_i64 nonfinite;
} dotsocp_report;

int dotsocp_report_edges(double edges[DOTSOCP_REPORT_BINS + 1]);
int dotsocp_solution_report(dotsocp_ctx *ctx, const double *rho0, const double *rho1, dotsocp_report *rep,
                            double *layer_mass , double *layer_neg );

int dotsocp_recover_velocity(dotsocp_ctx *ctx, const double *rho0, const double *rho1, double rho_floor,
                             double *vx, double *vy);

typedef struct { dotsocp_i64 n; int nsub; int direction; double rho_floor; } dotsocp_advect_opts;
int dotsocp_advect_particles(dotsocp_ctx *ctx, const double *rho0, const double *rho1, const dotsocp_advect_opts *o,
                             double *x, double *y, double *traj_x, double *traj_y, dotsocp_i64 *n_clamped);

typedef struct { dotsocp_i64 n; int nsub; int direction; double rho_floor; dotsocp_i64 nf; } dotsocp_push_opts;
int dotsocp_push_mass(dotsocp_ctx *ctx, const double *rho0, const double *rho1, const dotsocp_push_opts *o,
                      double *x, double *y, const double *mass, const dotsocp_i64 *frame_nodes, double *frames,
                      dotsocp_i64 *n_clamped, double *unit, double *l1);

typedef struct {
    dotsocp_i64 n, n_clamped, n_still;
    double mass;
    double cost_map, cost_length, cost_action;
    double disp_mean, len_mean;
    double disp_max, len_max, detour_max;
    dotsocp_i64 detour_hist[DOTSOCP_REPORT_BINS];
    dotsocp_i64 detour_over;
} dotsocp_map_report_t;
int dotsocp_map_report(dotsocp_ctx *ctx, const double *rho0, const double *rho1, const dotsocp_advect_opts *o,
                       double *x, double *y, const double *mass, dotsocp_map_report_t *rep, double *disp, double *len,
                       double *action);

enum { DOTSOCP_RENDER_LINEAR = 0, DOTSOCP_RENDER_INVERTED = 1, DOTSOCP_RENDER_LEVELS = 2 };
typedef struct {
    int mode;
    int channels;
    dotsocp_i64 nf;
    int nlevels;
    int barrier_index;
    double vmax;
    dotsocp_i64 skip_y, skip_x;
    double mask_frac;
} dotsocp_render_opts;
typedef struct {
    double vmax, rho_min;
    dotsocp_i64 nonfinite, masked;
    dotsocp_i64 my, mx;
} dotsocp_render_info;
int dotsocp_render_evolution(dotsocp_ctx *ctx, const double *rho0, const double *rho1, const dotsocp_render_opts *opts,
                             const dotsocp_i64 *frame_nodes, const double *levels, const unsigned char *lut,
                             const unsigned char *barrier, unsigned char *image, double *mvx, double *mvy,
                             dotsocp_render_info *info);

int dotsocp_jump_next_level(dotsocp_ctx *coarse, dotsocp_ctx *fine);

typedef struct dotsocp_weights dotsocp_weights;

dotsocp_weights *dotsocp_weights_create(int device, dotsocp_i64 ny, dotsocp_i64 nx, dotsocp_i64 nt, int levels);
void dotsocp_weights_destroy(dotsocp_weights *w);

dotsocp_i64 dotsocp_weights_len(dotsocp_i64 ny, dotsocp_i64 nx, dotsocp_i64 nt, int levels, int level);

int dotsocp_weights_set(dotsocp_weights *w, const double *weight);
int dotsocp_weights_set_space(dotsocp_weights *w, const double *weightX, const double *weightY);

int dotsocp_weights_restrict(dotsocp_weights *w, int log_mean);

int dotsocp_weights_log10_mean(dotsocp_weights *w, int level, double *mean);

int dotsocp_weights_download(dotsocp_weights *w, int level, double *host);

int dotsocp_upload_weight_from(dotsocp_ctx *ctx, dotsocp_weights *w, int level);

int dotsocp_get_history(dotsocp_ctx *ctx, double *kkt, double *time, double *iter, double *pdGap);

int dotsocp_set_profiling(dotsocp_ctx *ctx, int on);
int dotsocp_kernel_time(dotsocp_ctx *ctx, const char *name, double *avg_ms, dotsocp_i64 *launches);

int dotsocp_canary_check(void);

int dotsocp_poisson_phi(dotsocp_ctx *ctx);

int dotsocp_synchronize(dotsocp_ctx *ctx);

#ifdef __cplusplus
}
#endif
#endif
```

Before: 95.16.

## Skip storing cone multipliers on passes followed by a folded KKT check

When the cone pass before a folded KKT check would only write the gamma form, it now stores nothing and leaves the multiplier finish to the KKT cell kernel, which recomputes it from q_old. This applies to the fused cone, the qcone kernel and the z materialise path through new NOST/NONE/GIN template flavours. It saves one 10-component beta store per cell on the iterations that run a check, at the cost of extra recomputation in the check kernel and more solver state to track. It is limited to single-device INPALM with carry and fold enabled.

Result: faster. 97.40, median of 6 (+2.4%).

```diff
diff --git a/dot-socp_amd/capi.py b/dot-socp_amd/capi.py
--- a/dot-socp_amd/capi.py
+++ b/dot-socp_amd/capi.py
@@ -109,6 +109,8 @@
     "dotsocp_cone_writes_beta": (ctypes.c_int, [i64, dbl, i64, ctypes.c_int, ctypes.c_int, ctypes.c_int, dbl, dbl]),
     "dotsocp_rescale_due": (ctypes.c_int, [i64, ctypes.c_int, dbl, dbl]),
     "dotsocp_qcone_form": (ctypes.c_int, [i64, dbl, i64, ctypes.c_int, ctypes.c_int, ctypes.c_int, ctypes.c_int, dbl, dbl]),
+    "dotsocp_cone_store_none": (ctypes.c_int, [i64, dbl, i64, ctypes.c_int, ctypes.c_int, ctypes.c_int, dbl, dbl]),
+    "dotsocp_cone_form_launches": (ctypes.c_int, [vp, ctypes.c_int, ctypes.POINTER(i64)]),
     "dotsocp_release_cache": (i64, []),
     "dotsocp_upload": (ctypes.c_int, [vp, ctypes.c_int, vp]),
     "dotsocp_upload_layers": (ctypes.c_int, [vp, ctypes.c_int, vp, i64, i64]),
diff --git a/dot-socp_amd/csrc/capi.hip b/dot-socp_amd/csrc/capi.hip
--- a/dot-socp_amd/csrc/capi.hip
+++ b/dot-socp_amd/csrc/capi.hip
@@ -295,6 +295,10 @@
 int dotsocp_rescale_due(dotsocp_i64 it, int rescale, double maxFeas, double relGap) {
     return rescale_due(it, rescale, maxFeas, relGap) ? 1 : 0;
 }
+int dotsocp_cone_store_none(dotsocp_i64 it, double last_sigma_it, dotsocp_i64 maxit, int check_step_by_step,
+                            int last_of_run, int rescale, double maxFeas, double relGap) {
+    return cone_store_none(it, last_sigma_it, maxit, check_step_by_step != 0, last_of_run != 0, rescale, maxFeas, relGap) ? 1 : 0;
+}
 int dotsocp_qcone_form(dotsocp_i64 it, double last_sigma_it, dotsocp_i64 maxit, int check_step_by_step, int last_of_run,
                        int next_last_of_run, int rescale, double maxFeas, double relGap) {
     return qcone_form(it, last_sigma_it, maxit, check_step_by_step != 0, last_of_run != 0, next_last_of_run != 0, rescale,
@@ -443,6 +447,13 @@
     return DOTSOCP_EINVAL;
 }
 
+int dotsocp_cone_form_launches(dotsocp_ctx *ctx, int form, dotsocp_i64 *launches) {
+    CTX_OR_FAIL();
+    DS_ARG(form >= 0 && form < 3 && launches != nullptr, "form is 0 (gamma), 1 (beta) or 2 (none); launches must not be NULL");
+    *launches = ctx->s.form_launches[form];
+    return 0;
+}
+
 int dotsocp_canary_check(void) {
     std::string rep;
     const int bad = canary_check(&rep);
diff --git a/dot-socp_amd/csrc/fused.hip b/dot-socp_amd/csrc/fused.hip
--- a/dot-socp_amd/csrc/fused.hip
+++ b/dot-socp_amd/csrc/fused.hip
@@ -6,9 +6,12 @@
 
 namespace dotsocp {
 
-template <int MODE, int XB, bool NT = false, bool GIN = false, bool GOUT = false>
+template <int MODE, int XB, bool NT = false, bool GIN = false, bool GOUT = false, bool NOST = false>
 __global__ void __launch_bounds__(64 * XB) k_cone_fused(Grid g, LoopCoef c, FusedArgs a) {
-    static_assert(MODE == 1 || !(GIN || GOUT), "the gamma form exists between two MODE_B passes only");
+    static_assert(MODE == 1 || (MODE == 3 && GIN && !GOUT) || !(GIN || GOUT),
+                  "the gamma form exists between two MODE_B passes, and in what a check behind a NOST pass keeps for MODE_Z");
+    static_assert(!NOST || (MODE == 1 && GIN && !GOUT), "only the exit flavour can leave its store to the KKT check");
+    constexpr bool ZGIN = (MODE == 3 && GIN);
     constexpr bool DUAL = (MODE >= 5);
     constexpr bool UPD = (MODE != 0 && MODE != 6);
     constexpr bool PROJ = (MODE < 2 || MODE >= 5);
@@ -29,7 +32,7 @@
     const i64 nxblk = gridDim.y, nyblk = gridDim.x;
 
     EdgeQuad cur = load_edges(g, a.q, yc, xc, tstart, c.sf), curo, cur3;
-    if (UPD && !GIN) curo = load_edges(g, a.q_old, yc, xc, tstart, c.sf);
+    if (UPD && (!GIN || ZGIN)) curo = load_edges(g, a.q_old, yc, xc, tstart, c.sf);
     if (MODE == 5) cur3 = load_edges(g, a.q3, yc, xc, tstart, c.sf);
     GatherCarry gc, gcp;
     if (carried) {
@@ -50,10 +53,24 @@
             for (int j = 0; j < 10; ++j) b[j] = ld_stream<NT>(a.beta_in + j * g.Nc + i);
             if (!GIN) apply_scale_ops(b, a.bops);
             build_z2(v, a.q[i], cur, nxt, c.s, c.dF);
-            if constexpr (GIN) {
+            if constexpr (ZGIN) {
+                const EdgeQuad nxto = load_edges(g, a.q_old, yc, xc, tl + 1, c.sf);
+                double zo[10];
+                build_z2(zo, a.q_old[i], curo, nxto, c.s, c.dF);
+#pragma unroll
+                for (int j = 0; j < 10; ++j) b[j] = mult_finish(b[j], zo[j], c.tau);
+#pragma unroll
+                for (int j = 0; j < 10; ++j) zo[j] = zo[j] - b[j];
+                proj_row<10>(zo);
+                if (own && inb) {
+#pragma unroll
+                    for (int j = 0; j < 10; ++j) st_stream<NT>(a.z_out + j * g.Nc + i, zo[j]);
+                }
+                curo = nxto;
+            } else if constexpr (GIN) {
 #pragma unroll
                 for (int j = 0; j < 10; ++j) b[j] = mult_finish(b[j], v[j], c.tau);
-                if (!GOUT && own && inb) {
+                if (!GOUT && !NOST && own && inb) {
 #pragma unroll
                     for (int j = 0; j < 10; ++j) st_stream<NT>(a.beta_out + j * g.Nc + i, b[j]);
                 }
@@ -182,8 +199,22 @@
         else DS_KLAUNCH((k_cone_fused<M, 4>), grid, blk, 0, st, g, c, a);                \
         break;
     if (flavour != 0) {
-        if (mode != 1 || (flavour & ~(CONE_GIN | CONE_GOUT))) { set_error("bad fused flavour"); return DOTSOCP_EINVAL; }
+        const bool ok = (mode == 1 && !(flavour & ~(CONE_GIN | CONE_GOUT | CONE_NOST)) &&
+                         (!(flavour & CONE_NOST) || flavour == (CONE_GIN | CONE_NOST))) || (mode == 3 && flavour == CONE_GIN);
+        if (!ok) { set_error("bad fused flavour"); return DOTSOCP_EINVAL; }
         if ((flavour & CONE_GIN) && !a.bops.empty()) { set_error("internal: gamma with a pending scaling"); return DOTSOCP_ESTATE; }
+        if (mode == 3) {
+            if (nt) DS_KLAUNCH((k_cone_fused<3, 4, true, true>), grid, blk, 0, st, g, c, a);
+            else DS_KLAUNCH((k_cone_fused<3, 4, false, true>), grid, blk, 0, st, g, c, a);
+            DS_HIP(hipGetLastError());
+            return 0;
+        }
+        if (flavour & CONE_NOST) {
+            if (nt) DS_KLAUNCH((k_cone_fused<1, 4, true, true, false, true>), grid, blk, 0, st, g, c, a);
+            else DS_KLAUNCH((k_cone_fused<1, 4, false, true, false, true>), grid, blk, 0, st, g, c, a);
+            DS_HIP(hipGetLastError());
+            return 0;
+        }
 #define CONE_FLAV(GI, GO)                                                                          \
         if (nt) DS_KLAUNCH((k_cone_fused<1, 4, true, GI, GO>), grid, blk, 0, st, g, c, a);         \
         else DS_KLAUNCH((k_cone_fused<1, 4, false, GI, GO>), grid, blk, 0, st, g, c, a);
diff --git a/dot-socp_amd/csrc/kernels.h b/dot-socp_amd/csrc/kernels.h
--- a/dot-socp_amd/csrc/kernels.h
+++ b/dot-socp_amd/csrc/kernels.h
@@ -78,7 +78,7 @@
 };
 bool tile_xcd_remap(const Grid &g);
 int fused_geometry(const Grid &g, FusedGeom &fg);
-enum { CONE_GIN = 1, CONE_GOUT = 2 };
+enum { CONE_GIN = 1, CONE_GOUT = 2, CONE_NOST = 4 };
 int launch_cone_fused(int mode, const Grid &g, const LoopCoef &c, const FusedGeom &fg, FusedArgs a,
                       hipStream_t st, i64 z0 = 0, i64 zcount = -1, int flavour = 0);
 bool cone_split_enabled();
@@ -183,7 +183,8 @@
     double ap_mul, ap_div;
     int c_ends;
 };
-int launch_qcone(const Grid &g, const LoopCoef &c, const FusedGeom &fg, QConeArgs a, bool gout, hipStream_t st);
+enum { QOUT_GAMMA = 0, QOUT_BETA = 1, QOUT_NONE = 2 };
+int launch_qcone(const Grid &g, const LoopCoef &c, const FusedGeom &fg, QConeArgs a, int out, hipStream_t st);
 i64 qcone_chunk_len(const Grid &g);
 i64 qstep_rhs_chunks(const Grid &g, const FusedGeom &fg, i64 *TC = nullptr);
 int launch_qstep_rhs_acc(int var, const Grid &g, const LoopCoef &c, const FusedGeom &fg, const double *phi,
@@ -266,7 +267,7 @@
                         const KktWork &w, hipStream_t st);
 int launch_kkt_cells_update(const Grid &g, const LoopCoef &c, const KktCoef &k, const FusedGeom &fg, FusedArgs a,
                             const double *phi, const double *alpha, const double *weight, const KktWork &w,
-                            hipStream_t st, bool edges = false, const double *q_new = nullptr);
+                            hipStream_t st, bool edges = false, const double *q_new = nullptr, bool gin = false);
 int launch_norms(const Grid &g, const LoopCoef &c, const KktCoef &k, const FusedGeom &fg, FusedArgs a, const double *phi,
                  const double *alpha, const double *weight, const KktWork &w, hipStream_t st);
 double *kkt_qstep_partials(const Grid &g, const KktWork &w);
diff --git a/dot-socp_amd/csrc/kkt.hip b/dot-socp_amd/csrc/kkt.hip
--- a/dot-socp_amd/csrc/kkt.hip
+++ b/dot-socp_amd/csrc/kkt.hip
@@ -178,12 +178,13 @@
     }
 }
 
-template <bool WEIGHTED, bool EDGES, bool NORMS = false, bool NT = false>
+template <bool WEIGHTED, bool EDGES, bool NORMS = false, bool NT = false, bool GIN = false>
 __global__ void __launch_bounds__(TILE_Y *TILE_X) k_kkt_cells(Grid g, LoopCoef c, KktCoef k, FusedArgs a,
                                                                const double *__restrict__ phi,
                                                                const double *__restrict__ alpha,
                                                                const double *__restrict__ weight,
                                                                double *__restrict__ partials) {
+    static_assert(!GIN || (EDGES && !NORMS), "only the folded check of one slab takes gamma");
     __shared__ double2 xch[EDGES ? 2 : 1][EDGES ? TILE_X : 1][EDGES ? 64 : 1];
     const int lane = threadIdx.x, xl = threadIdx.y;
     const i64 y = (i64)blockIdx.x * TILE_Y + lane;
@@ -217,9 +218,13 @@
                 double v[10], zo[10];
 #pragma unroll
                 for (int j = 0; j < 10; ++j) b[j] = ld_stream<NT>(a.beta_in + j * g.Nc + i);
-                apply_scale_ops(b, a.bops);
+                if (!GIN) apply_scale_ops(b, a.bops);
                 build_z2(v, q0, cur, nxt, c.s, c.dF);
                 build_z2(zo, a.q_old[i], curo, nxto, c.s, c.dF);
+                if constexpr (GIN) {
+#pragma unroll
+                    for (int j = 0; j < 10; ++j) b[j] = mult_finish(b[j], zo[j], c.tau);
+                }
 #pragma unroll
                 for (int j = 0; j < 10; ++j) zo[j] = zo[j] - b[j];
                 proj_row<10>(zo);
@@ -572,7 +577,9 @@
 
 int launch_kkt_cells_update(const Grid &g, const LoopCoef &c, const KktCoef &k, const FusedGeom &fg, FusedArgs a,
                             const double *phi, const double *alpha, const double *weight, const KktWork &w,
-                            hipStream_t st, bool edges, const double *q_new) {
+                            hipStream_t st, bool edges, const double *q_new, bool gin) {
+    if (gin && !edges) { set_error("internal: only the folded cell pass reads gamma"); return DOTSOCP_ESTATE; }
+    if (gin && !a.bops.empty()) { set_error("internal: gamma with a pending scaling"); return DOTSOCP_ESTATE; }
     if (g.Nz <= 0) return 0;
     const i64 region = kkt_region_blocks(g);
     a.TC = fg.TC;
@@ -586,13 +593,15 @@
         return 0;
     }
     const bool nt = stream_nt_enabled();
-    if (weight) {
-        if (nt) DS_KLAUNCH((k_kkt_cells<true, true, false, true>), grid, blk, 0, st, g, c, k, a, phi, alpha, weight, part);
-        else DS_KLAUNCH((k_kkt_cells<true, true>), grid, blk, 0, st, g, c, k, a, phi, alpha, weight, part);
+#define CELLS(W, N, G) DS_KLAUNCH((k_kkt_cells<W, true, false, N, G>), grid, blk, 0, st, g, c, k, a, phi, alpha, weight, part)
+    if (gin) {
+        if (weight) { if (nt) CELLS(true, true, true); else CELLS(true, false, true); }
+        else { if (nt) CELLS(false, true, true); else CELLS(false, false, true); }
     } else {
-        if (nt) DS_KLAUNCH((k_kkt_cells<false, true, false, true>), grid, blk, 0, st, g, c, k, a, phi, alpha, weight, part);
-        else DS_KLAUNCH((k_kkt_cells<false, true>), grid, blk, 0, st, g, c, k, a, phi, alpha, weight, part);
-    }
+        if (weight) { if (nt) CELLS(true, true, false); else CELLS(true, false, false); }
+        else { if (nt) CELLS(false, true, false); else CELLS(false, false, false); }
+    }
+#undef CELLS
     DS_HIP(hipGetLastError());
     for (int dir = 0; dir < 2; ++dir) {
         const i64 len = dir == 0 ? g.ny : g.nx, lines = dir == 0 ? fg.nxblk : fg.nyblk;
diff --git a/dot-socp_amd/csrc/qstep_march.hip b/dot-socp_amd/csrc/qstep_march.hip
--- a/dot-socp_amd/csrc/qstep_march.hip
+++ b/dot-socp_amd/csrc/qstep_march.hip
@@ -290,9 +290,10 @@
     return 0;
 }
 
-template <bool NT, bool GOUT>
+template <bool NT, int OUT>
 __global__ void __launch_bounds__(TILE_Y *TILE_X, 3) k_qcone(Grid g, LoopCoef c, FusedGeom fg, QConeArgs a) {
     constexpr int XB = TILE_X;
+    constexpr bool GOUT = (OUT == QOUT_GAMMA);
     __shared__ double2 xch[2][XB][TILE_Y];
     __shared__ double ph[2][XB + 2][TILE_Y + 2];
     __shared__ double2 gch[2][XB][64];
@@ -375,7 +376,7 @@
                 build_z2(v, q0c, eprev, ecur, c.s, c.dF);
 #pragma unroll
                 for (int j = 0; j < 10; ++j) b[j] = mult_finish(b[j], v[j], c.tau);
-                if (!GOUT && own && inb) {
+                if (OUT == QOUT_BETA && own && inb) {
 #pragma unroll
                     for (int j = 0; j < 10; ++j) st_stream<NT>(a.beta_out + j * g.Nc + ci, b[j]);
                 }
@@ -410,20 +411,21 @@
     return TC < g.ntl ? TC : g.ntl;
 }
 
-int launch_qcone(const Grid &g, const LoopCoef &c, const FusedGeom &fg, QConeArgs a, bool gout, hipStream_t st) {
+int launch_qcone(const Grid &g, const LoopCoef &c, const FusedGeom &fg, QConeArgs a, int out, hipStream_t st) {
+    if (out != QOUT_GAMMA && out != QOUT_BETA && out != QOUT_NONE) { set_error("bad output form of k_qcone"); return DOTSOCP_EINVAL; }
     if (fg.XB != TILE_X || !(g.first && g.last) || g.ncl < 1) { set_error("internal: k_qcone on a grid it does not serve"); return DOTSOCP_ESTATE; }
     a.TC = qcone_chunk_len(g);
     const i64 chunks = (g.ntl + a.TC - 1) / a.TC;
     dim3 grid((unsigned)fg.nyblk, (unsigned)fg.nxblk, (unsigned)chunks);
     dim3 blk(TILE_Y, TILE_X);
     const bool nt = stream_nt_enabled();
-    if (gout) {
-        if (nt) DS_KLAUNCH((k_qcone<true, true>), grid, blk, 0, st, g, c, fg, a);
-        else DS_KLAUNCH((k_qcone<false, true>), grid, blk, 0, st, g, c, fg, a);
-    } else {
-        if (nt) DS_KLAUNCH((k_qcone<true, false>), grid, blk, 0, st, g, c, fg, a);
-        else DS_KLAUNCH((k_qcone<false, false>), grid, blk, 0, st, g, c, fg, a);
-    }
+#define QCONE_OUT(O)                                                                   \
+    if (nt) DS_KLAUNCH((k_qcone<true, O>), grid, blk, 0, st, g, c, fg, a);             \
+    else DS_KLAUNCH((k_qcone<false, O>), grid, blk, 0, st, g, c, fg, a);
+    if (out == QOUT_GAMMA) { QCONE_OUT(QOUT_GAMMA) }
+    else if (out == QOUT_BETA) { QCONE_OUT(QOUT_BETA) }
+    else { QCONE_OUT(QOUT_NONE) }
+#undef QCONE_OUT
     DS_HIP(hipGetLastError());
     return 0;
 }
diff --git a/dot-socp_amd/csrc/solver.h b/dot-socp_amd/csrc/solver.h
--- a/dot-socp_amd/csrc/solver.h
+++ b/dot-socp_amd/csrc/solver.h
@@ -105,7 +105,10 @@
 bool cone_writes_beta(i64 it, double lastSigmaIt, i64 maxit, bool checkStepByStep, bool last_of_run, int rescale,
                       double maxFeas, double relGap);
 
-enum { QCONE_NONE = 0, QCONE_STEADY = 1, QCONE_EXIT = 2 };
+bool cone_store_none(i64 it, double lastSigmaIt, i64 maxit, bool checkStepByStep, bool last_of_run, int rescale,
+                     double maxFeas, double relGap);
+
+enum { QCONE_NONE = 0, QCONE_STEADY = 1, QCONE_EXIT = 2, QCONE_CHECK = 3 };
 int qcone_form(i64 it, double lastSigmaIt, i64 maxit, bool checkStepByStep, bool last_of_run, bool next_last_of_run,
                int rescale, double maxFeas, double relGap);
 
@@ -237,11 +240,18 @@
     bool deferred = false;
     bool z_valid = true;
     bool z_prev_ok = false;
+    bool z_prev_gamma = false;
     bool rhs_valid = false;
     bool cone_carry = true;
     bool beta_gamma = false;
     bool cone_gout = false;
     bool last_of_run = false;
+    bool check_nostore = true;
+    bool cone_none = false;
+    bool gamma_stale = false;
+    bool early_none = false;
+    bool store_none_allowed() const;
+    i64 form_launches[3] = {0, 0, 0};
     int qcone = -1;
     bool q_valid = true;
     bool early_pass = false;
diff --git a/dot-socp_amd/csrc/solver.hip b/dot-socp_amd/csrc/solver.hip
--- a/dot-socp_amd/csrc/solver.hip
+++ b/dot-socp_amd/csrc/solver.hip
@@ -26,8 +26,12 @@
 
 int Solver::need_beta_form(const char *who) const {
     if (!beta_gamma) return 0;
-    set_error("internal: %s met the gamma form of beta", who);
+    set_error("internal: %s met the gamma form of beta%s", who, gamma_stale ? " (left by a pass that stored no multipliers)" : "");
     return DOTSOCP_ESTATE;
+}
+
+bool Solver::store_none_allowed() const {
+    return check_nostore && cone_carry && kkt_fold && fused && !multi() && method == DOTSOCP_METHOD_INPALM;
 }
 
 int Solver::need_q(const char *who) const {
@@ -147,6 +151,13 @@
     if (c_ends_on) DS_CHECK(detect_c_ends());
     timeout_at = -1;
     if (const char *e = getenv("DOTSOCP_TEST_TIMEOUT_AT")) timeout_at = atoll(e);
+    check_nostore = true;
+    if (const char *e = getenv("DOTSOCP_CHECK_NOSTORE")) check_nostore = (atoi(e) != 0);
+    cone_none = false;
+    gamma_stale = false;
+    early_none = false;
+    z_prev_gamma = false;
+    for (i64 &n : form_launches) n = 0;
     qcone = -1;
     if (const char *e = getenv("DOTSOCP_QCONE")) qcone = atoi(e);
     if (qcone < -1 || qcone > 2) qcone = -1;
@@ -286,13 +297,16 @@
 int Solver::phase_z(int part) {
     if (early_pass) {
         early_pass = false;
-        if (part != 0 || !fused || !deferred || cone_gout != early_gout) {
-            set_error("internal: the early cone pass wrote %s, the schedule asks for %s", early_gout ? "gamma" : "beta",
-                      cone_gout ? "gamma" : "beta");
+        const char *form[] = {"gamma", "beta", "nothing"};
+        const int wrote = early_gout ? QOUT_GAMMA : (early_none ? QOUT_NONE : QOUT_BETA);
+        const int asked = cone_gout ? QOUT_GAMMA : (cone_none ? QOUT_NONE : QOUT_BETA);
+        if (part != 0 || !fused || !deferred || wrote != asked || gamma_stale != early_none) {
+            set_error("internal: the early cone pass wrote %s, the schedule asks for %s", form[wrote], form[asked]);
             return DOTSOCP_ESTATE;
         }
         return 0;
     }
+    if (gamma_stale) { set_error("internal: a cone pass met a gamma that is one pass old"); return DOTSOCP_ESTATE; }
     DS_CHECK(need_q("phase_z"));
     if (part != 1) DS_CHECK(ensure_halo());
     if (!fused) {
@@ -306,7 +320,10 @@
         set_error("internal: gamma form %s", deferred ? "with a pending scaling of beta" : "without a pending multiplier step");
         return DOTSOCP_ESTATE;
     }
-    const int flavour = (gin ? CONE_GIN : 0) | (gout ? CONE_GOUT : 0);
+    const bool none = gin && !gout && cone_none;
+    if (none && (part != 0 || multi())) { set_error("internal: a pass that stores nothing on time slabs"); return DOTSOCP_ESTATE; }
+    const int flavour = (gin ? CONE_GIN : 0) | (gout ? CONE_GOUT : 0) | (none ? CONE_NOST : 0);
+    if (gin && part != 1) form_launches[gout ? QOUT_GAMMA : (none ? QOUT_NONE : QOUT_BETA)] += 1;
     const int ph = deferred ? (gin ? PH_CONE_CARRY : PH_FUSED_B) : PH_FUSED_A;
     z_valid = false;
     z_prev_ok = false;
@@ -336,13 +353,14 @@
         } else {
             DS_CHECK(launch_cone_fused(mode, s.g, lc, s.fg, a, s.st, z0, zc, flavour));
         }
-        if (deferred && part != 1) std::swap(s.beta, s.beta2);
+        if (deferred && part != 1 && !none) std::swap(s.beta, s.beta2);
     }
     prof_end(ph);
     if (part == 1) return 0;
     if (deferred) {
         bops.clear();
-        beta_gamma = gout;
+        beta_gamma = gout || none;
+        gamma_stale = none;
     }
     return 0;
 }
@@ -362,7 +380,9 @@
         set_error("internal: early cone pass in a state it does not serve");
         return DOTSOCP_ESTATE;
     }
-    const bool egout = (early == QCONE_STEADY);
+    const bool egout = (early == QCONE_STEADY), enone = (early == QCONE_CHECK);
+    const int eout = egout ? QOUT_GAMMA : (enone ? QOUT_NONE : QOUT_BETA);
+    if (early != QCONE_NONE) form_launches[eout] += 1;
     const int ph = (early != QCONE_NONE) ? PH_QCONE : PH_QSTEP;
     prof_begin(ph);
     FOR_SLABS(s) {
@@ -378,13 +398,13 @@
             a.q2_out = s.q; a.sx_out = s.sx2; a.sy_out = s.sy2;
             a.ap_on = aops.n; a.ap_mul = aops.mul; a.ap_div = aops.div;
             a.c_ends = (c_ends_on && s.c_ends) ? 1 : 0;
-            DS_CHECK(launch_qcone(s.g, lc, s.fg, a, egout, st));
+            DS_CHECK(launch_qcone(s.g, lc, s.fg, a, eout, st));
             std::swap(s.alpha, s.alpha2);
             std::swap(s.q, s.q_old);
             std::swap(s.q2, s.q_old);
             std::swap(s.sx, s.sx2);
             std::swap(s.sy, s.sy2);
-            std::swap(s.beta, s.beta2);
+            if (!enone) std::swap(s.beta, s.beta2);
         } else if (!fused) {
             DS_CHECK(launch_qstep(s.g, lc, s.phi, s.z, s.beta, s.weight, s.tail_bx, s.tail_by, s.q, s.alpha, s.st));
         } else {
@@ -411,8 +431,9 @@
                 a.q = s.q; a.q2 = s.q2; a.sx = s.sx; a.sy = s.sy;
                 a.beta_in = s.beta; a.beta_out = s.beta2;
                 a.bops = bops;
-                DS_CHECK(launch_cone_fused(1, s.g, lc, s.fg, a, s.st, 0, s.fg.chunks, CONE_GIN | (egout ? CONE_GOUT : 0)));
-                std::swap(s.beta, s.beta2);
+                DS_CHECK(launch_cone_fused(1, s.g, lc, s.fg, a, s.st, 0, s.fg.chunks,
+                                           CONE_GIN | (egout ? CONE_GOUT : 0) | (enone ? CONE_NOST : 0)));
+                if (!enone) std::swap(s.beta, s.beta2);
             }
         }
     }
@@ -421,11 +442,13 @@
     q_valid = true;
     if (early != QCONE_NONE) {
         q_valid = !egout || qcone == 2;
-        beta_gamma = egout;
+        beta_gamma = egout || enone;
+        gamma_stale = enone;
         z_valid = false;
         z_prev_ok = false;
         early_pass = true;
         early_gout = egout;
+        early_none = enone;
     }
     u0_made = multi() && fused;
     if (fused) aops.clear();
@@ -483,7 +506,7 @@
         a.beta_in = s.beta2;
         a.z_out = s.z;
         a.bops = zp_ops;
-        DS_CHECK(launch_cone_fused(3, s.g, lc, s.fg, a, s.st));
+        DS_CHECK(launch_cone_fused(3, s.g, lc, s.fg, a, s.st, 0, -1, z_prev_gamma ? CONE_GIN : 0));
     }
     prof_end(PH_MATERIALISE);
     z_valid = true;
@@ -491,7 +514,12 @@
 }
 
 int Solver::kkt_sums(double *S, bool folded) {
-    DS_CHECK(need_beta_form("kkt_sums"));
+    const bool gin = gamma_stale;
+    if (gin && !(folded && fused && deferred && beta_gamma && !multi() && bops.empty() && method == DOTSOCP_METHOD_INPALM)) {
+        set_error("internal: a KKT check that cannot finish the multiplier step met a pass that stored no multipliers");
+        return DOTSOCP_ESTATE;
+    }
+    if (!gin) DS_CHECK(need_beta_form("kkt_sums"));
     DS_CHECK(need_q("kkt_sums"));
     DS_CHECK(ensure_halo());
     const KktCoef k = kkt_coef();
@@ -509,11 +537,14 @@
             FusedArgs a = pending_step_args(s);
             a.beta_out = s.beta2;
             if (folded) { a.q2 = s.q2; a.sx = s.sx; a.sy = s.sy; }
-            DS_CHECK(launch_kkt_cells_update(s.g, lc, k, s.fg, a, s.phi, s.alpha, s.weight, s.kw, s.st, folded, s.q));
+            DS_CHECK(launch_kkt_cells_update(s.g, lc, k, s.fg, a, s.phi, s.alpha, s.weight, s.kw, s.st, folded, s.q, gin));
             std::swap(s.beta, s.beta2);
         }
         zp_ops = bops;
         bops.clear();
+        beta_gamma = false;
+        gamma_stale = false;
+        z_prev_gamma = gin;
         deferred = false;
         z_valid = false;
         z_prev_ok = true;
@@ -657,6 +688,13 @@
     return rescale_due(it + 1, rescale, maxFeas, relGap);
 }
 
+bool cone_store_none(i64 it, double lastSigmaIt, i64 maxit, bool checkStepByStep, bool last_of_run, int rescale,
+                     double maxFeas, double relGap) {
+    (void)last_of_run; (void)rescale; (void)maxFeas; (void)relGap;
+    if (checkStepByStep) return false;
+    return if_adjust_sigma((double)it, lastSigmaIt) || it >= maxit;
+}
+
 int qcone_form(i64 it, double lastSigmaIt, i64 maxit, bool checkStepByStep, bool last_of_run, bool next_last_of_run,
                int rescale, double maxFeas, double relGap) {
     if (cone_writes_beta(it, lastSigmaIt, maxit, checkStepByStep, last_of_run, rescale, maxFeas, relGap)) return QCONE_NONE;
@@ -675,8 +713,12 @@
     if (s.g.ncl < 1 || s.fg.XB != 4) return QCONE_NONE;
     if (qcone < 0 && s.fg.nyblk * s.fg.nxblk < 2048) return QCONE_NONE;
     if (time_limit_passed()) return QCONE_NONE;
-    return qcone_form(it, lastSigmaIt, opts.maxit, opts.ifCheckStepByStep != 0, last_of_run, next_last_of_run, rescale,
-                      maxFeas, relGap);
+    const int form = qcone_form(it, lastSigmaIt, opts.maxit, opts.ifCheckStepByStep != 0, last_of_run, next_last_of_run,
+                                rescale, maxFeas, relGap);
+    if (form == QCONE_EXIT && store_none_allowed() &&
+        cone_store_none(it + 1, lastSigmaIt, opts.maxit, opts.ifCheckStepByStep != 0, next_last_of_run, rescale, maxFeas, relGap))
+        return QCONE_CHECK;
+    return form;
 }
 
 bool if_adjust_sigma(double iter, double last_iter) {
@@ -794,6 +836,8 @@
     cone_gout = cone_carry && fused && deferred && !kkt_due &&
                 !cone_writes_beta(it, lastSigmaIt, opts.maxit, opts.ifCheckStepByStep != 0, last_of_run, rescale, maxFeas, relGap);
     const bool fold = kkt_due && kkt_fold && fused;
+    cone_none = !cone_gout && fold && deferred && beta_gamma && store_none_allowed() &&
+                cone_store_none(it, lastSigmaIt, opts.maxit, opts.ifCheckStepByStep != 0, last_of_run, rescale, maxFeas, relGap);
     const bool inter = comm_z && multi() && fused;
     bool split = inter && cone_split_enabled();
     for (auto &s : slabs) split = split && s.fg.chunks >= 2;
@@ -843,7 +887,7 @@
     DS_CHECK(phase_mult());
     const bool timed_out = time_limit_passed();
     timeout_pending = false;
-    if (timed_out && (beta_gamma || early_pass)) {
+    if (timed_out && ((beta_gamma && !gamma_stale) || early_pass)) {
         timeout_pending = true;
         return 0;
     }
diff --git a/dot-socp_amd/solvers.py b/dot-socp_amd/solvers.py
--- a/dot-socp_amd/solvers.py
+++ b/dot-socp_amd/solvers.py
@@ -123,6 +123,14 @@
         ms, n = capi.dbl(), capi.i64()
         capi.check(capi.lib().dotsocp_kernel_time(self._ctx, name.encode(), ctypes.byref(ms), ctypes.byref(n)))
         return ms.value, n.value
+
+    def cone_form_launches(self):
+        n = capi.i64()
+        out = {}
+        for form, name in enumerate(("gamma", "beta", "none")):
+            capi.check(capi.lib().dotsocp_cone_form_launches(self._ctx, form, ctypes.byref(n)))
+            out[name] = n.value
+        return out
 
     def finish(self, download=True):
         L = capi.lib()
diff --git a/include/dotsocp.h b/include/dotsocp.h
--- a/include/dotsocp.h
+++ b/include/dotsocp.h
@@ -125,6 +125,9 @@
 int dotsocp_rescale_due(dotsocp_i64 it, int rescale, double maxFeas, double relGap);
 int dotsocp_qcone_form(dotsocp_i64 it, double last_sigma_it, dotsocp_i64 maxit, int check_step_by_step, int last_of_run,
                        int next_last_of_run, int rescale, double maxFeas, double relGap);
+int dotsocp_cone_store_none(dotsocp_i64 it, double last_sigma_it, dotsocp_i64 maxit, int check_step_by_step,
+                            int last_of_run, int rescale, double maxFeas, double relGap);
+int dotsocp_cone_form_launches(dotsocp_ctx *ctx, int form, dotsocp_i64 *launches);
 
 int dotsocp_upload(dotsocp_ctx *ctx, int field, const double *host);
 int dotsocp_download(dotsocp_ctx *ctx, int field, double *host);
```
